# googlegenomics/spark-examples

Hardware: AMD Instinct MI355X
Metric: variants/sec into N×N Gram + PCoA wall-clock, 2504 samples, 1/2/4/8 GPU (higher is better)
Workload: dtype fp4(e2m1)->f32->i32

## Files before the change

### include/pcoa.h

```cpp
#ifndef PCOA_H_
#define PCOA_H_

#include <stddef.h>
#include <stdint.h>

#ifdef __cplusplus
extern "C" {
#endif

#define PCOA_VERSION_MAJOR 0
#define PCOA_VERSION_MINOR 10

typedef struct pcoa_ctx pcoa_ctx;

typedef enum pcoa_status {
  PCOA_OK = 0,
  PCOA_ERR_INVALID_ARG = -1,
  PCOA_ERR_NO_DEVICE = -2,
  PCOA_ERR_HIP = -3,
  PCOA_ERR_OUT_OF_MEMORY = -4,
  PCOA_ERR_INDEX_RANGE = -5,
  PCOA_ERR_RCCL = -6,
  PCOA_ERR_NOT_CONVERGED = -7,
  PCOA_ERR_STATE = -8
// ... 145 lines not shown
  double king_seconds;
  int64_t king_bytes;
  int64_t king_calls;
} pcoa_king_stats;
int pcoa_get_king_stats(pcoa_ctx* plane0, pcoa_king_stats* out, size_t out_size);

#define PCOA_LOADINGS_CENTRE 1u
#define PCOA_LOADINGS_UNIT   2u
int pcoa_loadings_begin(pcoa_ctx* ctx, int32_t num_pc, const double* components ,
                        const double* eigenvalues , uint32_t flags);
int pcoa_loadings_bits(pcoa_ctx* ctx, const uint32_t* bits, int64_t n_variants, int64_t ld_words, int is_device_ptr,
                       double* out , int out_is_device);
int pcoa_loadings_plink_bed(pcoa_ctx* ctx, const uint8_t* bed_rows, int64_t n_variants, int64_t row_bytes, int ref_is_a1,
                            int is_device_ptr, double* out, int out_is_device);
int pcoa_loadings_operator(pcoa_ctx* ctx, int64_t first_variant, int64_t n_variants, double* out, int out_is_device);
int pcoa_loadings_end(pcoa_ctx* ctx);

typedef struct pcoa_loadings_stats {
  int64_t loadings_variants;
  int64_t loadings_bytes;
  double loadings_seconds;
} pcoa_loadings_stats;
int pcoa_get_loadings_stats(pcoa_ctx* ctx, pcoa_loadings_stats* out, size_t out_size);

#define PCOA_LD_MAX_WINDOW 1024
#define PCOA_LD_ACCUMULATE 1u
int pcoa_ld_begin(pcoa_ctx* ctx, int32_t window, double r2_max, uint32_t flags);
int pcoa_ld_bits(pcoa_ctx* ctx, const uint32_t* bits, int64_t n_variants, int64_t ld_words, int is_device_ptr,
                 uint8_t* keep_out , int64_t* n_kept_out );
int pcoa_ld_plink_bed(pcoa_ctx* ctx, const uint8_t* bed_rows, int64_t n_variants, int64_t row_bytes, int ref_is_a1,
                      int is_device_ptr , uint8_t* keep_out, int64_t* n_kept_out);
int pcoa_ld_break(pcoa_ctx* ctx);
int pcoa_ld_end(pcoa_ctx* ctx);

typedef struct pcoa_ld_stats {
  int64_t ld_variants;
  int64_t ld_kept;
  int64_t ld_monomorphic;
  int64_t ld_pairs;
  double ld_count_seconds;
  double ld_band_seconds;
  double ld_resolve_seconds;
  double ld_compact_seconds;
} pcoa_ld_stats;
int pcoa_get_ld_stats(pcoa_ctx* ctx, pcoa_ld_stats* out, size_t out_size);

#define PCOA_LAYOUT_AUTO   0
#define PCOA_LAYOUT_FULL   1
#define PCOA_LAYOUT_STRIPS 2
#define PCOA_LAYOUT_FREE_FRACTION 0.9

int pcoa_plan_layout(int32_t n_samples, int32_t n_engines, const int64_t* free_bytes, int32_t request, int32_t* layout_out,
                     int32_t* col0_out, int32_t* cols_out);

int pcoa_device_memory(int32_t device_ordinal, int64_t* free_out, int64_t* total_out);

int pcoa_compute_strips(pcoa_ctx* const* owners, int32_t n_owners, int32_t num_pc, double* out_components,
                        double* out_eigenvalues, int32_t* nonzero_rows_out);

void pcoa_destroy(pcoa_ctx* ctx);

const char* pcoa_last_error(const pcoa_ctx* ctx);

int pcoa_reset(pcoa_ctx* ctx);

int pcoa_n_samples(const pcoa_ctx* ctx);

int pcoa_set_stream(pcoa_ctx* ctx, void* hip_stream);

int pcoa_sync(pcoa_ctx* ctx);

int pcoa_reserve(pcoa_ctx* ctx, int64_t variants_per_call, int32_t num_pc);


int pcoa_accumulate_calls(pcoa_ctx* ctx, const int32_t* sample_idx, const int64_t* row_offsets,
                          int64_t n_variants);

#define PCOA_CALLS_DEVICE_PTR 1u
#define PCOA_CALLS_HOST_PINNED 2u
#define PCOA_CALLS_ASYNC 4u
int pcoa_accumulate_calls_ex(pcoa_ctx* ctx, const int32_t* sample_idx, const int64_t* row_offsets, int64_t n_variants,
                             uint32_t flags);

int pcoa_accumulate_dense_f32(pcoa_ctx* ctx, const float* x, int64_t n_variants, int64_t ld,
                              int is_device_ptr);

int pcoa_accumulate_dense_u8(pcoa_ctx* ctx, const uint8_t* x, int64_t n_variants, int64_t ld, int is_device_ptr);

int pcoa_accumulate_bits(pcoa_ctx* ctx, const uint32_t* bits, int64_t n_variants, int64_t ld_words,
                         int is_device_ptr);

#define PCOA_BED_HOST_ASYNC 2
int pcoa_accumulate_plink_bed(pcoa_ctx* ctx, const uint8_t* bed_rows, int64_t n_variants, int64_t row_bytes, int ref_is_a1,
                              int is_device_ptr);

int pcoa_accumulate_synthetic(pcoa_ctx* ctx, const pcoa_synth_params* params, int64_t first_variant,
                              int64_t n_variants);

int pcoa_synth_fill_f32(pcoa_ctx* ctx, const pcoa_synth_params* params, int64_t first_variant,
                        int64_t n_variants, float* x_dev, int64_t ld);

int pcoa_gram_finalize(pcoa_ctx* ctx);

int pcoa_gram_allreduce_rccl(pcoa_ctx* ctx, void* nccl_comm);

int pcoa_comm_unique_id(uint8_t out_id[128]);
int pcoa_comm_runtime(char* path_out, int32_t path_cap, int32_t* version_out);
int pcoa_comm_init(pcoa_ctx* ctx, const uint8_t id[128], int32_t rank, int32_t n_ranks,
                   void** comm_out);
int pcoa_comm_destroy(void* nccl_comm);
int pcoa_comm_count(void* nccl_comm, int32_t* count_out);

int pcoa_host_alloc_pinned(size_t bytes, void** out);
int pcoa_host_free_pinned(void* p);

int pcoa_gram_reduce_from(pcoa_ctx* dst, pcoa_ctx* src);

#define PCOA_REDUCE_MAX_ENGINES 16
int pcoa_gram_reduce_peers(pcoa_ctx* const* ctxs, int32_t k, int32_t root_only);

typedef struct pcoa_reduce_peers_stats {
  int64_t reduce_peers_calls;
  double reduce_peers_seconds;
  int64_t reduce_peers_bytes_in;
} pcoa_reduce_peers_stats;
int pcoa_get_reduce_peers_stats(pcoa_ctx* ctx, pcoa_reduce_peers_stats* out, size_t out_size);

int pcoa_gram_export_device_i64(pcoa_ctx* ctx, int64_t* dst_dev);
int pcoa_gram_import_device_i64(pcoa_ctx* ctx, const int64_t* src_dev);

int pcoa_gram_read_i64(pcoa_ctx* ctx, int64_t* out_nxn);

int pcoa_gram_read_block_i64(pcoa_ctx* ctx, int32_t row0, int32_t col0, int32_t rows, int32_t cols, int64_t* out);

int pcoa_gram_load_i64(pcoa_ctx* ctx, const int64_t* in_nxn);


int pcoa_center_read_f64(pcoa_ctx* ctx, double* out_b_nxn, double* out_row_sums, int32_t* out_nonzero_rows,
                         double* out_matrix_mean);

int pcoa_compute(pcoa_ctx* ctx, int32_t num_pc, double* out_components, double* out_eigenvalues,
                 int32_t* out_nonzero_rows);

int pcoa_project(pcoa_ctx* ref, pcoa_ctx* cross, int32_t num_pc, const double* components, const double* eigenvalues,
                 double* out_coords);


int pcoa_get_timings(pcoa_ctx* ctx, pcoa_timings* out);
int pcoa_get_timings_sized(pcoa_ctx* ctx, pcoa_timings* out, size_t out_size);
int pcoa_reset_timings(pcoa_ctx* ctx);

int pcoa_debug_alloc(int32_t device_ordinal, size_t bytes, void** out);
int pcoa_debug_centred_matvec(pcoa_ctx* ctx, const double* x, double* y, int form);
int pcoa_debug_reduce_chunk(int32_t g, int32_t k, int32_t n_samples, int64_t* first_out, int64_t* count_out);
int pcoa_debug_free(void* p);
int pcoa_debug_guard_mode(void);


int pcoa_device_info(pcoa_ctx* ctx, char* name_out, int32_t name_cap, int32_t* cu_count_out);
const char* pcoa_version(void);

#ifdef __cplusplus
}
#endif
#endif
```

### spark-examples_amd/_lib.py

```python
import ctypes
import os

_HERE = os.path.dirname(os.path.abspath(__file__))
LIB_PATH = os.environ.get("PCOA_LIB") or os.path.join(_HERE, "libpcoa_hip.so")

PCOA_OK = 0
PCOA_ERR_INVALID_ARG = -1
PCOA_ERR_NO_DEVICE = -2
PCOA_ERR_HIP = -3
PCOA_ERR_OUT_OF_MEMORY = -4
PCOA_ERR_INDEX_RANGE = -5
PCOA_ERR_RCCL = -6
PCOA_ERR_NOT_CONVERGED = -7
PCOA_ERR_STATE = -8

PCOA_FLAG_DEFAULT = 0
PCOA_FLAG_GRAM_F32_MFMA = 0x1
PCOA_FLAG_GRAM_I8_MFMA = 0x2
PCOA_FLAG_GRAM_FP4_MFMA = 0x4
PCOA_FLAG_NO_SIGN_NORM = 0x10
PCOA_FLAG_EIG_HOUSEHOLDER = 0x20
PCOA_FLAG_EIG_LANCZOS = 0x40
PCOA_FLAG_NO_PIPELINE = 0x80
PCOA_FLAG_OPERAND_FP4 = 0x100
# ... 66 lines not shown
        ("reduce_peers_seconds", ctypes.c_double),
        ("reduce_peers_bytes_in", ctypes.c_int64),
    ]


PCOA_REDUCE_MAX_ENGINES = 16


class PcoaPair(ctypes.Structure):
    _fields_ = [
        ("i", ctypes.c_int32),
        ("j", ctypes.c_int32),
        ("shared", ctypes.c_int64),
    ]


class PcoaPairsStats(ctypes.Structure):
    _fields_ = [
        ("pairs_seconds", ctypes.c_double),
        ("pairs_bytes", ctypes.c_int64),
        ("pairs_calls", ctypes.c_int64),
    ]


PCOA_KING_HET = 0
PCOA_KING_MISSING = 1
PCOA_KING_HET_OR_MISSING = 2
PCOA_KING_HOM_A1 = 3
PCOA_KING_HOM_A2 = 4
PCOA_KING_PLANES = 5


class PcoaKingPair(ctypes.Structure):
    _fields_ = [
        ("i", ctypes.c_int32),
        ("j", ctypes.c_int32),
        ("hethet", ctypes.c_int64),
        ("ibs0", ctypes.c_int64),
        ("het_sum", ctypes.c_int64),
    ]


class PcoaKingStats(ctypes.Structure):
    _fields_ = [
        ("king_seconds", ctypes.c_double),
        ("king_bytes", ctypes.c_int64),
        ("king_calls", ctypes.c_int64),
    ]


class PcoaLdStats(ctypes.Structure):
    _fields_ = [
        ("ld_variants", ctypes.c_int64),
        ("ld_kept", ctypes.c_int64),
        ("ld_monomorphic", ctypes.c_int64),
        ("ld_pairs", ctypes.c_int64),
        ("ld_count_seconds", ctypes.c_double),
        ("ld_band_seconds", ctypes.c_double),
        ("ld_resolve_seconds", ctypes.c_double),
        ("ld_compact_seconds", ctypes.c_double),
    ]


class PcoaLoadingsStats(ctypes.Structure):
    _fields_ = [
        ("loadings_variants", ctypes.c_int64),
        ("loadings_bytes", ctypes.c_int64),
        ("loadings_seconds", ctypes.c_double),
    ]


PCOA_LOADINGS_CENTRE = 1
PCOA_LOADINGS_UNIT = 2
PCOA_LD_MAX_WINDOW = 1024
PCOA_LD_ACCUMULATE = 1


class PcoaSynthParams(ctypes.Structure):
    _fields_ = [
        ("seed", ctypes.c_uint64),
        ("n_pops", ctypes.c_int32),
        ("reserved", ctypes.c_int32),
        ("pop_offsets", ctypes.POINTER(ctypes.c_int32)),
        ("thresholds", ctypes.POINTER(ctypes.c_uint32)),
    ]


_vp = ctypes.c_void_p
_i32 = ctypes.c_int32
_i64 = ctypes.c_int64
_SIGNATURES = [
    ("pcoa_version", ctypes.c_char_p, []),
    ("pcoa_create", ctypes.c_int, [ctypes.POINTER(_vp), _i32, _i32, ctypes.c_uint32]),
    ("pcoa_create_strip", ctypes.c_int, [ctypes.POINTER(_vp), _i32, _i32, _i32, _i32, ctypes.c_uint32]),
    ("pcoa_create_operator", ctypes.c_int, [ctypes.POINTER(_vp), _i32, _i32, ctypes.c_uint32]),
    ("pcoa_create_subset", ctypes.c_int, [ctypes.POINTER(_vp), _vp, _vp, _i32]),
    ("pcoa_similar_pairs", ctypes.c_int, [_vp, ctypes.c_double, _vp, _i64, ctypes.POINTER(_i64), _vp]),
    ("pcoa_get_pairs_stats", ctypes.c_int, [_vp, ctypes.POINTER(PcoaPairsStats), ctypes.c_size_t]),
    ("pcoa_set_similarity", ctypes.c_int, [_vp, _i32]),
    ("pcoa_get_similarity", ctypes.c_int, [_vp, ctypes.POINTER(_i32)]),
    ("pcoa_set_call_companion", ctypes.c_int, [_vp, _vp, _i64]),
    ("pcoa_get_call_companion", ctypes.c_int, [_vp, ctypes.POINTER(_vp), ctypes.POINTER(_i64)]),
    ("pcoa_accumulate_plink_bed_calls", ctypes.c_int, [_vp, _vp, _vp, _i64, _i64, ctypes.c_int, ctypes.c_int]),
    ("pcoa_accumulate_plink_bed_king", ctypes.c_int, [_vp, _vp, _i64, _i64, ctypes.c_int]),
    ("pcoa_king_pairs", ctypes.c_int, [_vp, ctypes.c_double, _vp, _i64, ctypes.POINTER(_i64), ctypes.POINTER(_i64), _vp]),
    ("pcoa_get_king_stats", ctypes.c_int, [_vp, ctypes.POINTER(PcoaKingStats), ctypes.c_size_t]),
    ("pcoa_loadings_begin", ctypes.c_int, [_vp, _i32, _vp, _vp, ctypes.c_uint32]),
    ("pcoa_loadings_bits", ctypes.c_int, [_vp, _vp, _i64, _i64, ctypes.c_int, _vp, ctypes.c_int]),
    ("pcoa_loadings_plink_bed", ctypes.c_int, [_vp, _vp, _i64, _i64, ctypes.c_int, ctypes.c_int, _vp, ctypes.c_int]),
    ("pcoa_loadings_operator", ctypes.c_int, [_vp, _i64, _i64, _vp, ctypes.c_int]),
    ("pcoa_loadings_end", ctypes.c_int, [_vp]),
    ("pcoa_get_loadings_stats", ctypes.c_int, [_vp, ctypes.POINTER(PcoaLoadingsStats), ctypes.c_size_t]),
    ("pcoa_ld_begin", ctypes.c_int, [_vp, _i32, ctypes.c_double, ctypes.c_uint32]),
    ("pcoa_ld_bits", ctypes.c_int, [_vp, _vp, _i64, _i64, ctypes.c_int, _vp, ctypes.POINTER(_i64)]),
    ("pcoa_ld_plink_bed", ctypes.c_int, [_vp, _vp, _i64, _i64, ctypes.c_int, ctypes.c_int, _vp, ctypes.POINTER(_i64)]),
    ("pcoa_ld_break", ctypes.c_int, [_vp]),
    ("pcoa_ld_end", ctypes.c_int, [_vp]),
    ("pcoa_get_ld_stats", ctypes.c_int, [_vp, ctypes.POINTER(PcoaLdStats), ctypes.c_size_t]),
    ("pcoa_operator_info", ctypes.c_int, [_vp, ctypes.POINTER(_i64), ctypes.POINTER(_i64)]),
    ("pcoa_operator_row_sums", ctypes.c_int, [_vp, _vp]),
    ("pcoa_operator_matvec_device", ctypes.c_int, [_vp, _vp, _vp, ctypes.c_int]),
    ("pcoa_create_grm", ctypes.c_int, [ctypes.POINTER(_vp), _i32, _i32, ctypes.c_uint32]),
    ("pcoa_grm_info", ctypes.c_int, [_vp, ctypes.POINTER(_i64), ctypes.POINTER(_i64), ctypes.POINTER(_i64)]),
    ("pcoa_grm_set_min_maf", ctypes.c_int, [_vp, ctypes.c_double]),
    ("pcoa_grm_counts", ctypes.c_int, [_vp, _i64, _i64, _vp]),
    ("pcoa_grm_matvec_device", ctypes.c_int, [_vp, _vp, _vp]),
    ("pcoa_strip_info", ctypes.c_int, [_vp, ctypes.POINTER(_i32), ctypes.POINTER(_i32)]),
    ("pcoa_strip_col_sums", ctypes.c_int, [_vp, _vp]),
    ("pcoa_strip_matvec", ctypes.c_int, [_vp, _vp, _vp, ctypes.c_double, _vp]),
    ("pcoa_strip_set_centering", ctypes.c_int, [_vp, _vp, ctypes.c_double]),
    ("pcoa_strip_matvec_device", ctypes.c_int, [_vp, _vp, _vp]),
    ("pcoa_plan_layout", ctypes.c_int, [_i32, _i32, _vp, _i32, ctypes.POINTER(_i32), _vp, _vp]),
    ("pcoa_device_memory", ctypes.c_int, [_i32, ctypes.POINTER(_i64), ctypes.POINTER(_i64)]),
    ("pcoa_compute_strips", ctypes.c_int, [_vp, _i32, _i32, _vp, _vp, ctypes.POINTER(_i32)]),
    ("pcoa_project", ctypes.c_int, [_vp, _vp, _i32, _vp, _vp, _vp]),
    ("pcoa_destroy", None, [_vp]),
    ("pcoa_last_error", ctypes.c_char_p, [_vp]),
    ("pcoa_reset", ctypes.c_int, [_vp]),
    ("pcoa_n_samples", ctypes.c_int, [_vp]),
    ("pcoa_set_stream", ctypes.c_int, [_vp, _vp]),
    ("pcoa_sync", ctypes.c_int, [_vp]),
    ("pcoa_reserve", ctypes.c_int, [_vp, _i64, _i32]),
    ("pcoa_comm_runtime", ctypes.c_int, [ctypes.c_char_p, _i32, ctypes.POINTER(_i32)]),
    ("pcoa_debug_alloc", ctypes.c_int, [_i32, ctypes.c_size_t, ctypes.POINTER(_vp)]),
    ("pcoa_debug_free", ctypes.c_int, [_vp]),
    ("pcoa_debug_reduce_chunk", ctypes.c_int, [_i32, _i32, _i32, ctypes.POINTER(_i64), ctypes.POINTER(_i64)]),
    ("pcoa_debug_guard_mode", ctypes.c_int, []),
    ("pcoa_accumulate_calls", ctypes.c_int, [_vp, _vp, _vp, _i64]),
    ("pcoa_gram_reduce_from", ctypes.c_int, [_vp, _vp]),
    ("pcoa_gram_reduce_peers", ctypes.c_int, [_vp, _i32, _i32]),
    ("pcoa_get_reduce_peers_stats", ctypes.c_int, [_vp, ctypes.POINTER(PcoaReducePeersStats), ctypes.c_size_t]),
    ("pcoa_lanczos_with_matvec", ctypes.c_int, [_vp, ctypes.c_int32, _vp, _vp, _vp, _vp, ctypes.POINTER(ctypes.c_int32)]),
    ("pcoa_debug_centred_matvec", ctypes.c_int, [_vp, _vp, _vp, ctypes.c_int]),
    ("pcoa_host_alloc_pinned", ctypes.c_int, [ctypes.c_size_t, ctypes.POINTER(ctypes.c_void_p)]),
    ("pcoa_host_free_pinned", ctypes.c_int, [_vp]),
    ("pcoa_accumulate_plink_bed", ctypes.c_int, [_vp, _vp, _i64, _i64, ctypes.c_int, ctypes.c_int]),
    ("pcoa_accumulate_calls_ex", ctypes.c_int, [_vp, _vp, _vp, _i64, ctypes.c_uint32]),
    ("pcoa_accumulate_dense_f32", ctypes.c_int, [_vp, _vp, _i64, _i64, ctypes.c_int]),
    ("pcoa_accumulate_dense_u8", ctypes.c_int, [_vp, _vp, _i64, _i64, ctypes.c_int]),
    ("pcoa_accumulate_bits", ctypes.c_int, [_vp, _vp, _i64, _i64, ctypes.c_int]),
    ("pcoa_accumulate_synthetic", ctypes.c_int, [_vp, ctypes.POINTER(PcoaSynthParams), _i64, _i64]),
    ("pcoa_synth_fill_f32", ctypes.c_int, [_vp, ctypes.POINTER(PcoaSynthParams), _i64, _i64, _vp, _i64]),
    ("pcoa_gram_finalize", ctypes.c_int, [_vp]),
    ("pcoa_gram_allreduce_rccl", ctypes.c_int, [_vp, _vp]),
    ("pcoa_comm_unique_id", ctypes.c_int, [_vp]),
    ("pcoa_comm_init", ctypes.c_int, [_vp, _vp, _i32, _i32, ctypes.POINTER(_vp)]),
    ("pcoa_comm_destroy", ctypes.c_int, [_vp]),
    ("pcoa_comm_count", ctypes.c_int, [_vp, ctypes.POINTER(_i32)]),
    ("pcoa_gram_export_device_i64", ctypes.c_int, [_vp, _vp]),
    ("pcoa_gram_import_device_i64", ctypes.c_int, [_vp, _vp]),
    ("pcoa_gram_read_i64", ctypes.c_int, [_vp, _vp]),
    ("pcoa_gram_read_block_i64", ctypes.c_int, [_vp, _i32, _i32, _i32, _i32, _vp]),
    ("pcoa_gram_load_i64", ctypes.c_int, [_vp, _vp]),
    ("pcoa_center_read_f64", ctypes.c_int, [_vp, _vp, _vp, ctypes.POINTER(_i32), ctypes.POINTER(ctypes.c_double)]),
    ("pcoa_compute", ctypes.c_int, [_vp, _i32, _vp, _vp, ctypes.POINTER(_i32)]),
    ("pcoa_get_timings", ctypes.c_int, [_vp, ctypes.POINTER(PcoaTimings)]),
    ("pcoa_get_timings_sized", ctypes.c_int, [_vp, ctypes.POINTER(PcoaTimings), ctypes.c_size_t]),
    ("pcoa_reset_timings", ctypes.c_int, [_vp]),
    ("pcoa_device_info", ctypes.c_int, [_vp, ctypes.c_char_p, _i32, ctypes.POINTER(_i32)]),
]
EXPORTED_SYMBOLS = [s[0] for s in _SIGNATURES]

_lib = None


def source_hash():
    import hashlib
    h = hashlib.sha256()
    csrc = os.path.join(_HERE, "csrc")
    files = [os.path.join(csrc, f) for f in sorted(os.listdir(csrc)) if f.endswith((".hip", ".inl", ".h"))]
    files.append(os.path.join(os.path.dirname(_HERE), "include", "pcoa.h"))
    for f in files:
        h.update(os.path.basename(f).encode())
        with open(f, "rb") as fh:
            h.update(fh.read())
    return h.hexdigest()[:16]


def load():
    global _lib
    if _lib is not None:
        return _lib
    if not os.path.exists(LIB_PATH):
        raise ImportError(
            "%s not found: build it with `python -c 'import __graft_entry__ as g; g.build()'` or "
            "`make -C spark-examples_amd/csrc`.  There is no CPU fallback." % LIB_PATH)
    try:
        import torch
    except Exception:
        pass
    lib = ctypes.CDLL(LIB_PATH, mode=ctypes.RTLD_GLOBAL)
    for name, restype, argtypes in _SIGNATURES:
        fn = getattr(lib, name)
        fn.restype = restype
        fn.argtypes = argtypes
    _lib = lib
    return lib
```

### spark-examples_amd/csrc/capi_compute.hip

```cpp
#include <algorithm>
#include <cmath>
#include <cstdio>
#include <string>

#include "pcoa_ctx.h"

using namespace pcoa;

namespace pcoa {

int ensure_workspace(pcoa_ctx* c, int32_t k) {
  const int64_t n = c->n;
  if (!c->ws_ready) {
    HIP_TRY(c, dev_alloc((void**)&c->colmean, sizeof(double) * (size_t)n, c->device));
    HIP_TRY(c, dev_alloc((void**)&c->ws.d, sizeof(double) * (size_t)n, c->device));
    HIP_TRY(c, dev_alloc((void**)&c->ws.e, sizeof(double) * (size_t)n, c->device));
    HIP_TRY(c, dev_alloc((void**)&c->ws.tau, sizeof(double) * (size_t)n, c->device));
    HIP_TRY(c, dev_alloc((void**)&c->ws.q, sizeof(double) * (size_t)n, c->device));
    HIP_TRY(c, dev_alloc((void**)&c->ws.w, sizeof(double) * (size_t)(2 * n), c->device));
    HIP_TRY(c, dev_alloc((void**)&c->ws.scratch, sizeof(double) * (size_t)(6 * n), c->device));
    HIP_TRY(c, dev_alloc((void**)&c->ws.iscratch, sizeof(int32_t) * (size_t)(2 * n + 64), c->device));
    HIP_TRY(c, dev_alloc((void**)&c->row_sums, sizeof(double) * (size_t)n, c->device));
    HIP_TRY(c, dev_alloc((void**)&c->stats, sizeof(double) * (size_t)(2 + n), c->device));
    HIP_TRY(c, dev_alloc((void**)&c->nz, sizeof(int32_t) * 4, c->device));
// ... 58 lines not shown
  c->lanczos_steps = steps;
  if (steps_out) *steps_out = steps;
  if (!conv)
    return fail(c, PCOA_ERR_NOT_CONVERGED, "Lanczos did not reach a verified residual (tiny spectral gaps?); there is no dense "
                                           "fallback for an operator the engine does not hold");
  c->eig_method = 1;
  c->eig_dense_form = 0;
  HIP_TRY(c, launch_backtransform(c->ws, n, num_pc, (c->flags & PCOA_FLAG_NO_SIGN_NORM) ? 0 : 1, 0, c->out_dev, c->stream));
  HIP_TRY(c, hipMemcpyAsync(out_components, c->out_dev, sizeof(double) * (size_t)num_pc * (size_t)n, hipMemcpyDeviceToHost,
                            c->stream));
  HIP_TRY(c, hipStreamSynchronize(c->stream));
  for (size_t i = 0; i < (size_t)num_pc * (size_t)n; ++i)
    if (!std::isfinite(out_components[i])) return fail(c, PCOA_ERR_NOT_CONVERGED, "non-finite eigenvector entry");
  if (out_eigenvalues)
    for (int32_t t = 0; t < num_pc; ++t) out_eigenvalues[t] = sel[(size_t)t];
  return PCOA_OK;
}

}

namespace {

int project_engine_state(pcoa_ctx* report, pcoa_ctx* c, const char* who, int rc) {
  if (rc == PCOA_ERR_INDEX_RANGE || rc == PCOA_ERR_INVALID_ARG) rc = PCOA_ERR_STATE;
  return fail(report, rc, std::string("project: ") + who + ": " + c->last_error);
}

int compute_strips_small(pcoa_ctx* const* owners, int32_t n_owners, int32_t num_pc, double* out_components,
                         double* out_eigenvalues, int32_t* nonzero_rows_out) {
  pcoa_ctx* lead = owners[0];
  const int32_t n = lead->n;
  std::vector<int64_t> s((size_t)n * (size_t)n), part;
  for (int32_t i = 0; i < n_owners; ++i) {
    pcoa_ctx* o = owners[i];
    part.assign((size_t)n * (size_t)o->s_cols, 0);
    const int rc = pcoa_gram_read_i64(o, part.data());
    if (rc != PCOA_OK) return fail(lead, rc, "compute_strips: owner " + std::to_string(i) + ": " + o->last_error);
    for (int32_t r = 0; r < n; ++r)
      for (int32_t j = 0; j < o->s_cols; ++j) s[(size_t)r * n + o->strip_col0 + j] = part[(size_t)r * o->s_cols + j];
  }
  pcoa_ctx* tmp = nullptr;
  int rc = pcoa_create(&tmp, n, lead->device, lead->flags);
  if (rc != PCOA_OK) return fail(lead, rc, std::string("compute_strips: temporary engine: ") + pcoa_last_error(nullptr));
  rc = pcoa_gram_load_i64(tmp, s.data());
  if (rc == PCOA_OK) rc = pcoa_compute(tmp, num_pc, out_components, out_eigenvalues, nonzero_rows_out);
  if (rc != PCOA_OK) lead->last_error = "compute_strips: temporary engine: " + tmp->last_error;
  pcoa_destroy(tmp);
  (void)hipSetDevice(lead->device);
  return rc;
}

}

extern "C" {

int pcoa_center_read_f64(pcoa_ctx* c, double* out_b, double* out_row_sums, int32_t* out_nonzero_rows,
                         double* out_matrix_mean) {
  CHECK_CTX(c);
  NOT_ON_OPERATOR(c, "pcoa_center_read_f64");
  if (c->is_strip) return fail(c, PCOA_ERR_STATE, "a strip owner holds N x cols of S: use pcoa_strip_col_sums / pcoa_strip_matvec");
  int rc = finalize_impl(c);
  if (rc != PCOA_OK) return rc;
  if ((rc = check_device_flags(c)) != PCOA_OK) return rc;
  rc = ensure_workspace(c, 1);
  if (rc != PCOA_OK) return rc;
  if (out_b && (rc = ensure_b(c)) != PCOA_OK) return rc;
  const size_t n = (size_t)c->n;
  {
    ScopedTimer t(c, T_CENTER);
    if (measured(c)) {
      if ((rc = measure_centre(c, false, out_b ? c->ws.a : nullptr)) != PCOA_OK) return rc;
    } else {
      HIP_TRY(c, launch_center(c->s32, c->s64, c->n, c->row_sums, c->stats, c->nz, out_b ? c->ws.a : nullptr,
                               c->stream));
    }
  }
  if (out_b) HIP_TRY(c, hipMemcpyAsync(out_b, c->ws.a, sizeof(double) * n * n, hipMemcpyDeviceToHost, c->stream));
  if (out_row_sums)
    HIP_TRY(c, hipMemcpyAsync(out_row_sums, c->row_sums, sizeof(double) * n, hipMemcpyDeviceToHost, c->stream));
  HIP_TRY(c, hipMemcpyAsync(c->hw->st, c->stats, 2 * sizeof(double), hipMemcpyDeviceToHost, c->stream));
  HIP_TRY(c, hipMemcpyAsync(&c->hw->nz, c->nz, sizeof(int32_t), hipMemcpyDeviceToHost, c->stream));
  HIP_TRY(c, hipStreamSynchronize(c->stream));
  if (out_nonzero_rows) *out_nonzero_rows = c->hw->nz;
  if (out_matrix_mean) *out_matrix_mean = c->hw->st[1];
  return PCOA_OK;
}

int pcoa_compute(pcoa_ctx* c, int32_t num_pc, double* out_components, double* out_eigenvalues,
                 int32_t* out_nonzero_rows) {
  CHECK_CTX(c);
  const int32_t n = c->n;
  if (num_pc <= 0 || num_pc > n) {
    char buf[128];
    std::snprintf(buf, sizeof(buf), "num_pc = %d out of range (0, n = %d]", num_pc, n);
    return fail(c, PCOA_ERR_INVALID_ARG, buf);
  }
  if (!out_components) return fail(c, PCOA_ERR_INVALID_ARG, "out_components is NULL");
  if (c->is_grm) return grm_compute(c, num_pc, out_components, out_eigenvalues, out_nonzero_rows);
  if (c->is_operator) return operator_compute(c, num_pc, out_components, out_eigenvalues, out_nonzero_rows);
  if (c->is_strip)
    return fail(c, PCOA_ERR_STATE, "a strip owner holds N x cols of S: the eigensolve over strips is driven by the host "
                                   "(pcoa_strip_col_sums / pcoa_strip_matvec; spark-examples_amd/strips.py)");
  int rc = finalize_impl(c);
  if (rc != PCOA_OK) return rc;
  rc = check_device_flags(c);
  if (rc != PCOA_OK) return rc;
  rc = ensure_workspace(c, num_pc);
  if (rc != PCOA_OK) return rc;

  struct WallEvents {
    pcoa_ctx* c;
    hipEvent_t w0, w1;
    ~WallEvents() {
      if (w0) c->pool.push_back(w0);
      if (w1) c->pool.push_back(w1);
    }
  } wall{c, get_event(c), get_event(c)};
  hipEvent_t w0 = wall.w0, w1 = wall.w1;
  if (w0) (void)hipEventRecord(w0, c->stream);

  const bool force_householder = (c->flags & PCOA_FLAG_EIG_HOUSEHOLDER) != 0;
  const bool force_lanczos = (c->flags & PCOA_FLAG_EIG_LANCZOS) != 0;
  const bool try_lanczos = !force_householder && n >= 32;
  const bool explicit_b = !try_lanczos || debug_knobs().explicit_center != 0;
  if (explicit_b && (rc = ensure_b(c)) != PCOA_OK) return rc;
  const int sym_min = debug_knobs().symv_sym_min_n > 0 ? debug_knobs().symv_sym_min_n : 16384;
  const bool sym_form = !explicit_b && !c->s64 && n >= sym_min && (n & 3) == 0;
  if (sym_form && (rc = ensure(c, &c->sym_part, &c->sym_part_cap, (int64_t)symv_sym_workspace_doubles(n))) != PCOA_OK) return rc;
  const bool measured = pcoa::measured(c);
  {
    ScopedTimer t(c, T_CENTER);
    if (measured) {
      if ((rc = measure_centre(c, sym_form, explicit_b ? c->ws.a : nullptr)) != PCOA_OK) return rc;
    } else {
      if (sym_form)
        HIP_TRY(c, launch_row_sums_sym(c->s32, n, c->sym_part, c->row_sums, reinterpret_cast<int64_t*>(c->stats + 2), c->stream));
      HIP_TRY(c, launch_center(c->s32, c->s64, n, c->row_sums, c->stats, c->nz, explicit_b ? c->ws.a : nullptr,
                               c->stream, sym_form));
      HIP_TRY(c, launch_col_means(c->row_sums, n, c->colmean, c->stream));
    }
  }
  c->ws.s32 = c->s32;
  c->ws.s64 = c->s64;
  c->ws.colmean = c->colmean;
  c->ws.stats = c->stats;
  bool b_ready = explicit_b;
  std::vector<double> sel((size_t)num_pc);
  bool have_vectors = false;
  c->eig_method = 0;
  c->eig_dense_form = 0;
  c->lanczos_steps = 0;
  if (try_lanczos) {
    const int32_t mmax = std::min<int32_t>(n, 512);
    const int64_t need = (int64_t)lanczos_workspace_doubles(n, num_pc, mmax);
    rc = ensure(c, &c->lanczos_ws, &c->lanczos_cap, need);
    if (rc != PCOA_OK) return rc;
    int conv = 0, steps = 0;
    {
      ScopedTimer t(c, T_LANCZOS);
      EigWorkspace wl = c->ws;
      if (!b_ready) wl.a = nullptr;
      wl.sym_part = (sym_form && !wl.a) ? c->sym_part : nullptr;
      c->matvec_form = wl.a ? 2 : wl.sym_part ? 1 : 0;
      wl.band_only = (c->flags & PCOA_FLAG_EIG_BAND) != 0;
      if (measured) measure_bind(c, &wl);
      int band = 0;
      HIP_TRY(c, lanczos_topk(wl, c->lanczos_ws, n, num_pc, mmax, 1e-11, sel.data(), &conv, &steps, c->stream, nullptr, &band));
      c->lanczos_block_steps = band;
    }
    c->lanczos_steps = steps;
    if (conv) {
      have_vectors = true;
      c->eig_method = 1;
    } else if (force_lanczos) {
      return fail(c, PCOA_ERR_NOT_CONVERGED, "Lanczos did not reach a verified residual (PCOA_FLAG_EIG_LANCZOS set)");
    } else if (n > 16384) {
      return fail(c, PCOA_ERR_NOT_CONVERGED,
                  "Lanczos did not reach a verified residual and the dense O(N^3) fallback is disabled above "
                  "N = 16384 (set PCOA_FLAG_EIG_HOUSEHOLDER to force it)");
    }
  }
  if (!have_vectors) {
    c->eig_method = 2;
    if (!b_ready) {
      if ((rc = ensure_b(c)) != PCOA_OK) return rc;
      ScopedTimer t(c, T_CENTER);
      if (measured) {
        if ((rc = measure_b(c, c->ws.a)) != PCOA_OK) return rc;
      } else {
        HIP_TRY(c, launch_center(c->s32, c->s64, n, c->row_sums, c->stats, c->nz, c->ws.a, c->stream));
      }
      b_ready = true;
    }
    {
      ScopedTimer t(c, T_TRIDIAG);
      HIP_TRY(c, launch_tridiagonalize(c->ws, n, c->stream, &c->eig_dense_form));
    }
    std::vector<int32_t> idx;
    for (int32_t t = 0; t < num_pc; ++t) idx.push_back(n - 1 - t);
    for (int32_t t = 0; t < num_pc; ++t)
      if (t < n - num_pc) idx.push_back(t);
    std::vector<double> cand(idx.size());
    {
      ScopedTimer t(c, T_EIG);
      HIP_TRY(c, launch_bisect(c->ws, n, idx.data(), (int32_t)idx.size(), c->ws.lam, c->stream, &c->eig_dense_form));
      HIP_TRY(c, hipMemcpyAsync(cand.data(), c->ws.lam, sizeof(double) * cand.size(), hipMemcpyDeviceToHost,
                                c->stream));
    }
    HIP_TRY(c, hipStreamSynchronize(c->stream));
    std::vector<int> order(cand.size());
    for (size_t i = 0; i < order.size(); ++i) order[i] = (int)i;
    std::stable_sort(order.begin(), order.end(), [&](int a, int b) {
      const double fa = std::fabs(cand[a]), fb = std::fabs(cand[b]);
      if (fa != fb) return fa > fb;
      return cand[a] > cand[b];
    });
    for (int32_t t = 0; t < num_pc; ++t) {
      if (!std::isfinite(cand[order[t]])) return fail(c, PCOA_ERR_NOT_CONVERGED, "non-finite eigenvalue");
      sel[(size_t)t] = cand[order[t]];
    }
    {
      ScopedTimer t(c, T_EIG);
      HIP_TRY(c, launch_inverse_iteration(c->ws, n, sel.data(), num_pc, c->stream, &c->eig_dense_form));
    }
  }
  {
    ScopedTimer t(c, T_BACK);
    HIP_TRY(c, launch_backtransform(c->ws, n, num_pc, (c->flags & PCOA_FLAG_NO_SIGN_NORM) ? 0 : 1,
                                    have_vectors ? 0 : 1, c->out_dev, c->stream, have_vectors ? nullptr : &c->eig_dense_form));
  }
  HIP_TRY(c, hipMemcpyAsync(out_components, c->out_dev, sizeof(double) * (size_t)num_pc * (size_t)n,
                            hipMemcpyDeviceToHost, c->stream));
  HIP_TRY(c, hipMemcpyAsync(&c->hw->nz, c->nz, sizeof(int32_t), hipMemcpyDeviceToHost, c->stream));
  if (w1) (void)hipEventRecord(w1, c->stream);
  HIP_TRY(c, hipStreamSynchronize(c->stream));
  if (w0 && w1) {
    float ms = 0.f;
    if (hipEventElapsedTime(&ms, w0, w1) == hipSuccess) c->compute_total = (double)ms * 1e-3;
  }
  for (int32_t t = 0; t < num_pc; ++t) {
    for (int32_t i = 0; i < n; ++i)
      if (!std::isfinite(out_components[(size_t)t * n + i]))
        return fail(c, PCOA_ERR_NOT_CONVERGED, "non-finite eigenvector entry");
  }
  if (out_eigenvalues)
    for (int32_t t = 0; t < num_pc; ++t) out_eigenvalues[t] = sel[(size_t)t];
  if (out_nonzero_rows) *out_nonzero_rows = c->hw->nz;
  return PCOA_OK;
}

int pcoa_lanczos_with_matvec(pcoa_ctx* c, int32_t num_pc, pcoa_matvec_fn fn, void* user, double* out_components,
                             double* out_eigenvalues, int32_t* steps_out) {
  CHECK_CTX(c);
  NOT_ON_GRM(c, "pcoa_lanczos_with_matvec");
  const int32_t n = c->n;
  if (!fn || !out_components) return fail(c, PCOA_ERR_INVALID_ARG, "fn or out_components is NULL");
  if (num_pc <= 0 || num_pc > n) return fail(c, PCOA_ERR_INVALID_ARG, "num_pc must be in (0, n]");
  if (n < 32) return fail(c, PCOA_ERR_INVALID_ARG, "the Lanczos path needs N >= 32");
  LanczosMatvec mv = [&](const double* v, double* y) { return fn(user, v, y); };
  return lanczos_over(c, num_pc, mv, out_components, out_eigenvalues, steps_out);
}

int pcoa_strip_info(const pcoa_ctx* c, int32_t* col0_out, int32_t* cols_out) {
  if (!c) return fail(nullptr, PCOA_ERR_INVALID_ARG, "ctx is NULL");
  if (col0_out) *col0_out = c->strip_col0;
  if (cols_out) *cols_out = c->s_cols;
  return c->is_strip ? 1 : 0;
}

int pcoa_strip_col_sums(pcoa_ctx* c, double* out_cols) {
  CHECK_CTX(c);
  if (!c->is_strip) return fail(c, PCOA_ERR_STATE, "not a strip owner (pcoa_create_strip)");
  if (!out_cols) return fail(c, PCOA_ERR_INVALID_ARG, "out_cols is NULL");
  int rc = finalize_impl(c);
  if (rc != PCOA_OK) return rc;
  if ((rc = check_device_flags(c)) != PCOA_OK) return rc;
  const int64_t need = strip_ws_doubles(c->n, c->s_cols);
  if ((rc = ensure(c, &c->strip_ws, &c->strip_ws_cap, need)) != PCOA_OK) return rc;
  {
    ScopedTimer t(c, T_CENTER);
    HIP_TRY(c, launch_strip_col_sums(c->s32, c->s64, c->n, c->s_cols, c->strip_ws, c->stream));
  }
  HIP_TRY(c, hipMemcpyAsync(out_cols, c->strip_ws, sizeof(double) * (size_t)c->s_cols, hipMemcpyDeviceToHost, c->stream));
  HIP_TRY(c, hipStreamSynchronize(c->stream));
  return PCOA_OK;
}

int pcoa_strip_matvec(pcoa_ctx* c, const double* v, const double* means, double matrix_mean, double* y_out) {
  CHECK_CTX(c);
  if (!c->is_strip) return fail(c, PCOA_ERR_STATE, "not a strip owner (pcoa_create_strip)");
  if (!v || !means || !y_out) return fail(c, PCOA_ERR_INVALID_ARG, "v, means or y_out is NULL");
  int rc = finalize_impl(c);
  if (rc != PCOA_OK) return rc;
  if ((rc = check_device_flags(c)) != PCOA_OK) return rc;
  const int64_t need = strip_ws_doubles(c->n, c->s_cols) + 2 * (int64_t)c->n;
  if ((rc = ensure(c, &c->strip_ws, &c->strip_ws_cap, need)) != PCOA_OK) return rc;
  double* v_dev = c->strip_ws + strip_ws_doubles(c->n, c->s_cols);
  double* m_dev = v_dev + c->n;
  HIP_TRY(c, hipMemcpyAsync(v_dev, v, sizeof(double) * (size_t)c->n, hipMemcpyHostToDevice, c->stream));
  HIP_TRY(c, hipMemcpyAsync(m_dev, means, sizeof(double) * (size_t)c->n, hipMemcpyHostToDevice, c->stream));
  {
    ScopedTimer t(c, T_LANCZOS);
    HIP_TRY(c, launch_strip_matvec(c->s32, c->s64, c->n, c->strip_col0, c->s_cols, v_dev, m_dev, matrix_mean, c->strip_ws,
                                   c->stream));
  }
  HIP_TRY(c, hipMemcpyAsync(y_out, c->strip_ws, sizeof(double) * (size_t)c->s_cols, hipMemcpyDeviceToHost, c->stream));
  HIP_TRY(c, hipStreamSynchronize(c->stream));
  return PCOA_OK;
}

int pcoa_strip_set_centering(pcoa_ctx* c, const double* means, double matrix_mean) {
  CHECK_CTX(c);
  if (!c->is_strip) return fail(c, PCOA_ERR_STATE, "not a strip owner (pcoa_create_strip)");
  if (!means) return fail(c, PCOA_ERR_INVALID_ARG, "means is NULL");
  if (!c->strip_means) HIP_TRY(c, dev_alloc((void**)&c->strip_means, sizeof(double) * (size_t)c->n, c->device));
  HIP_TRY(c, hipMemcpyAsync(c->strip_means, means, sizeof(double) * (size_t)c->n, hipMemcpyHostToDevice, c->stream));
  HIP_TRY(c, hipStreamSynchronize(c->stream));
// ... 228 lines not shown
    int64_t* to_i64 = local ? rs_i64 + c->strip_col0 : reinterpret_cast<int64_t*>(c->strip_ws + strip_ws_doubles(n, c->s_cols));
    double* to_f64 = local ? lead->row_sums + c->strip_col0 : c->strip_ws + strip_ws_doubles(n, c->s_cols) + n;
    {
      ScopedTimer t(c, T_CENTER);
      const hipError_t e = launch_strip_col_sums_to(c->s32, c->s64, n, c->s_cols, c->strip_ws, to_i64, to_f64, c->stream);
      if (e != hipSuccess) return owner_failed(i, hip_fail(c, e, "strip column sums"));
    }
    if (!local) {
      hipError_t e = hipMemcpyPeerAsync(rs_i64 + c->strip_col0, lead->device, to_i64, c->device, sizeof(int64_t) * (size_t)c->s_cols,
                                        c->stream);
      if (e == hipSuccess)
        e = hipMemcpyPeerAsync(lead->row_sums + c->strip_col0, lead->device, to_f64, c->device, sizeof(double) * (size_t)c->s_cols,
                               c->stream);
      if (e != hipSuccess) return owner_failed(i, hip_fail(c, e, "peer copy of the column sums"));
    }
  }
  for (int32_t i = 0; i < n_owners; ++i) {
    pcoa_ctx* c = owners[i];
    (void)hipSetDevice(c->device);
    const hipError_t e = hipStreamSynchronize(c->stream);
    if (e != hipSuccess) return owner_failed(i, hip_fail(c, e, "column sums"));
  }
  (void)hipSetDevice(lead->device);
  {
    ScopedTimer t(lead, T_CENTER);
    HIP_TRY(lead, launch_center(nullptr, nullptr, n, lead->row_sums, lead->stats, lead->nz, nullptr, lead->stream, true));
    HIP_TRY(lead, launch_col_means(lead->row_sums, n, lead->colmean, lead->stream));
  }
  double st[2] = {0, 0};
  HIP_TRY(lead, hipMemcpyAsync(st, lead->stats, sizeof(st), hipMemcpyDeviceToHost, lead->stream));
  HIP_TRY(lead, hipMemcpyAsync(&lead->hw->nz, lead->nz, sizeof(int32_t), hipMemcpyDeviceToHost, lead->stream));
  for (int32_t i = 0; i < n_owners; ++i) {
    pcoa_ctx* c = owners[i];
    if (c->device == lead->device)
      HIP_TRY(lead, hipMemcpyAsync(c->strip_means, lead->colmean, sizeof(double) * (size_t)n, hipMemcpyDeviceToDevice, lead->stream));
    else
      HIP_TRY(lead, hipMemcpyPeerAsync(c->strip_means, c->device, lead->colmean, lead->device, sizeof(double) * (size_t)n, lead->stream));
  }
  HIP_TRY(lead, hipStreamSynchronize(lead->stream));
  const double matrix_mean = st[1];
  for (int32_t i = 0; i < n_owners; ++i) {
    owners[i]->strip_matrix_mean = matrix_mean;
    owners[i]->strip_centering_set = true;
  }

  struct Events {
    std::vector<hipEvent_t> ev;
    ~Events() { for (hipEvent_t e : ev) if (e) (void)hipEventDestroy(e); }
  } evs;
  evs.ev.assign((size_t)n_owners + 1, nullptr);
  for (int32_t i = 0; i <= n_owners; ++i) {
    const int dev = i == 0 ? lead->device : owners[i - 1]->device;
    (void)hipSetDevice(dev);
    const hipError_t e = hipEventCreateWithFlags(&evs.ev[(size_t)i], hipEventDisableTiming);
    if (e != hipSuccess) {
      (void)hipSetDevice(lead->device);
      return hip_fail(lead, e, "hipEventCreateWithFlags");
    }
  }
  (void)hipSetDevice(lead->device);
  std::string mv_error;
  LanczosMatvec mv = [&](const double* v, double* y) -> int {
    auto bad = [&](hipError_t e, int32_t i, const char* what) {
      mv_error = "compute_strips: owner " + std::to_string(i) + ": " + what + ": " + hipGetErrorString(e);
      (void)hipSetDevice(lead->device);
      return 1;
    };
    hipError_t e = hipEventRecord(evs.ev[0], lead->stream);
    if (e != hipSuccess) return bad(e, 0, "hipEventRecord");
    for (int32_t i = 0; i < n_owners; ++i) {
      pcoa_ctx* c = owners[i];
      const bool local = c->device == lead->device;
      if ((e = hipSetDevice(c->device)) != hipSuccess) return bad(e, i, "hipSetDevice");
      if ((e = hipStreamWaitEvent(c->stream, evs.ev[0], 0)) != hipSuccess) return bad(e, i, "hipStreamWaitEvent");
      const double* vo = v;
      double* dst = y + c->strip_col0;
      double* const spare = c->strip_ws + strip_ws_doubles(n, c->s_cols);
      if (!local) {
        if ((e = hipMemcpyPeerAsync(spare, c->device, v, lead->device, sizeof(double) * (size_t)n, c->stream)) != hipSuccess)
          return bad(e, i, "peer copy of v");
        vo = spare;
        if (!peer[(size_t)i]) dst = spare + n;
      }
      if ((e = launch_strip_matvec_to(c->s32, c->s64, n, c->strip_col0, c->s_cols, vo, c->strip_means, matrix_mean, c->strip_ws,
                                      dst, c->stream)) != hipSuccess)
        return bad(e, i, "strip mat-vec");
      if (!local && !peer[(size_t)i] &&
          (e = hipMemcpyPeerAsync(y + c->strip_col0, lead->device, dst, c->device, sizeof(double) * (size_t)c->s_cols,
                                  c->stream)) != hipSuccess)
        return bad(e, i, "peer copy of the piece");
      if ((e = hipEventRecord(evs.ev[(size_t)i + 1], c->stream)) != hipSuccess) return bad(e, i, "hipEventRecord");
    }
    if ((e = hipSetDevice(lead->device)) != hipSuccess) return bad(e, 0, "hipSetDevice");
    for (int32_t i = 0; i < n_owners; ++i)
      if ((e = hipStreamWaitEvent(lead->stream, evs.ev[(size_t)i + 1], 0)) != hipSuccess) return bad(e, i, "hipStreamWaitEvent");
    return 0;
  };
  int32_t steps = 0;
  rc = lanczos_over(lead, num_pc, mv, out_components, out_eigenvalues, &steps);
  if (rc != PCOA_OK && !mv_error.empty()) lead->last_error = mv_error;
  if (rc != PCOA_OK) return rc;
  if (nonzero_rows_out) *nonzero_rows_out = lead->hw->nz;
  lead->compute_total = wall_now() - t0;
  return PCOA_OK;
}

int pcoa_debug_centred_matvec(pcoa_ctx* c, const double* x, double* y, int form) {
  CHECK_CTX(c);
  if (!x || !y) return fail(c, PCOA_ERR_INVALID_ARG, "x or y is NULL");
  if (form < 0 || form > 2) return fail(c, PCOA_ERR_INVALID_ARG, "form must be 0, 1 or 2");
  const bool upper_triangle_form = form == 1;
  NOT_ON_OPERATOR(c, "pcoa_debug_centred_matvec");
  if (c->is_strip) return fail(c, PCOA_ERR_STATE, "not available on a strip owner");
  int rc = finalize_impl(c);
  if (rc != PCOA_OK) return rc;
  if ((rc = check_device_flags(c)) != PCOA_OK) return rc;
  if ((rc = ensure_workspace(c, 1)) != PCOA_OK) return rc;
  const int32_t n = c->n;
  EigWorkspace wl = c->ws;
  wl.a = nullptr;
  wl.s32 = c->s32;
  wl.s64 = c->s64;
  wl.colmean = c->colmean;
  wl.stats = c->stats;
  wl.sym_part = nullptr;
  if (upper_triangle_form) {
    if (c->s64 || (n & 3)) return fail(c, PCOA_ERR_STATE, "the upper-triangle form needs N % 4 == 0 and no int64 part");
    if ((rc = ensure(c, &c->sym_part, &c->sym_part_cap, (int64_t)symv_sym_workspace_doubles(n))) != PCOA_OK) return rc;
    wl.sym_part = c->sym_part;
    if (!measured(c))
      HIP_TRY(c, launch_row_sums_sym(c->s32, n, c->sym_part, c->row_sums, reinterpret_cast<int64_t*>(c->stats + 2), c->stream));
  }
  if (form == 2) {
    if ((rc = ensure_b(c)) != PCOA_OK) return rc;
    wl.a = c->ws.a;
  }
  if (measured(c)) {
    if ((rc = measure_centre(c, upper_triangle_form, wl.a)) != PCOA_OK) return rc;
    measure_bind(c, &wl);
  } else {
    HIP_TRY(c, launch_center(c->s32, c->s64, n, c->row_sums, c->stats, c->nz, wl.a, c->stream, upper_triangle_form));
    HIP_TRY(c, launch_col_means(c->row_sums, n, c->colmean, c->stream));
  }
  double* xd = c->ws.q;
  double* yd = c->ws.w;
  HIP_TRY(c, hipMemcpyAsync(xd, x, sizeof(double) * (size_t)n, hipMemcpyHostToDevice, c->stream));
  launch_centred_matvec(wl, n, xd, yd, c->stream);
  HIP_TRY(c, hipGetLastError());
  HIP_TRY(c, hipMemcpyAsync(y, yd, sizeof(double) * (size_t)n, hipMemcpyDeviceToHost, c->stream));
  HIP_TRY(c, hipStreamSynchronize(c->stream));
  return PCOA_OK;
}

}
```

### spark-examples_amd/csrc/eig.hip

```cpp
#include <cfloat>
#include <type_traits>
#include <algorithm>
#include <cmath>

#include "pcoa_internal.h"

namespace pcoa {
namespace {

constexpr int HW_T = 1024;

__device__ __forceinline__ double wave_sum(double v) {
#pragma unroll
  for (int o = 32; o > 0; o >>= 1) v += __shfl_down(v, o, 64);
  return v;
}
__device__ __forceinline__ double wave_max(double v) {
#pragma unroll
  for (int o = 32; o > 0; o >>= 1) v = fmax(v, __shfl_down(v, o, 64));
  return v;
}
__device__ __forceinline__ double wave_min(double v) {
#pragma unroll
  for (int o = 32; o > 0; o >>= 1) v = fmin(v, __shfl_down(v, o, 64));
// ... 527 lines not shown
  const int lane = threadIdx.x & 63, wave = threadIdx.x >> 6;
  const int slice = blockIdx.x, vec = blockIdx.y;
  const int s0 = blk * BT;
  const int c0 = slice * 256, c1 = (c0 + 256 < n) ? c0 + 256 : n;
  const double* zc = z + (int64_t)vec * n;
  for (int i = wave; i < BT; i += 4) {
    double acc = 0.0;
    if (s0 + i < nref) {
      const double* vi = a + (int64_t)(s0 + i) * n;
      for (int c = c0 + lane; c < c1; c += 64)
        if (c > s0 + i) acc += vi[c] * zc[c];
    }
    acc = wave_sum(acc);
    if (lane == 0) ypart[((int64_t)slice * k + vec) * BT + i] = acc;
  }
}

__global__ __launch_bounds__(256) void wy_apply_kernel(const double* __restrict__ a, int n, int nref, int blk, int nslices,
                                                       const double* __restrict__ t, const double* __restrict__ ypart,
                                                       double* __restrict__ z, int k) {
  __shared__ double y[BT], ty[BT];
  const int slice = blockIdx.x, vec = blockIdx.y;
  const int s0 = blk * BT;
  if (threadIdx.x < BT) {
    double acc = 0.0;
    for (int sl = 0; sl < nslices; ++sl) acc += ypart[((int64_t)sl * k + vec) * BT + threadIdx.x];
    y[threadIdx.x] = acc;
  }
  __syncthreads();
  if (threadIdx.x < BT) {
    const double* tb = t + (int64_t)blk * BT * BT;
    double acc = 0.0;
    for (int c = threadIdx.x; c < BT; ++c) acc += tb[threadIdx.x * BT + c] * y[c];
    ty[threadIdx.x] = acc;
  }
  __syncthreads();
  const int c = slice * 256 + threadIdx.x;
  if (c >= n) return;
  double* zc = z + (int64_t)vec * n;
  double acc = 0.0;
#pragma unroll 8
  for (int i = 0; i < BT; ++i)
    if (s0 + i < nref && c > s0 + i) acc += a[(int64_t)(s0 + i) * n + c] * ty[i];
  zc[c] -= acc;
}

}

hipError_t launch_tridiagonalize(const EigWorkspace& ws, int32_t n, hipStream_t stream, int32_t* form) {
  if (n <= 0) return hipErrorInvalidValue;
  if (n == 1) {
    hipLaunchKernelGGL(tridiag_hw_kernel, dim3(1), dim3(HW_T), 0, stream, ws.a, n, 0, ws.d, ws.e, ws.tau, ws.q,
                       ws.w);
    return hipGetLastError();
  }
  const size_t lds_full = 3 * (size_t)n * sizeof(double);
  int kf = 0;
  if (n >= 8 && lds_full <= 160 * 1024 - 1024) {
    if (lds_full > 64 * 1024) {
      static bool raised = false;
      if (!raised) {
        hipError_t err = hipFuncSetAttribute(reinterpret_cast<const void*>(tridiag_fused_kernel),
                                             hipFuncAttributeMaxDynamicSharedMemorySize, 160 * 1024 - 1024);
        if (err != hipSuccess) return err;
        raised = true;
      }
    }
    if (form) *form |= EIG_FORM_FUSED | (lds_full > 64 * 1024 ? EIG_FORM_FUSED_BIG_LDS : 0);
    kf = n - 2;
    double* qb[2] = {ws.w, ws.w + n};
    double* vb[2] = {ws.scratch, ws.scratch + n};
    for (int k = 0; k < kf; ++k) {
      const int rows = n - k - 1;
      int nb = (rows + FT / 64 - 1) / (FT / 64);
      if (nb > 256) nb = 256;
      nb = (nb + 7) / 8 * 8;
      const size_t lds = 3 * (size_t)(n - k) * sizeof(double);
      hipLaunchKernelGGL(tridiag_fused_kernel, dim3((unsigned)nb), dim3(FT), lds, stream, ws.a, n, k, ws.d, ws.e, ws.tau,
                         qb[(k + 1) & 1], qb[k & 1], vb[(k + 1) & 1], vb[k & 1]);
    }
    hipError_t err = hipMemcpyAsync(ws.a + (int64_t)(kf - 1) * n + kf, vb[(kf - 1) & 1] + kf, sizeof(double) * (size_t)(n - kf),
                                    hipMemcpyDeviceToDevice, stream);
    if (err != hipSuccess) return err;
    err = hipMemcpyAsync(ws.q, qb[(kf - 1) & 1], sizeof(double) * (size_t)n, hipMemcpyDeviceToDevice, stream);
    if (err != hipSuccess) return err;
  }
  if (form && kf == 0) *form |= EIG_FORM_TWO_KERNEL;
  for (int k = kf; k <= n - 2; ++k) {
    const int hw_threads = HW_T;
    hipLaunchKernelGGL(tridiag_hw_kernel, dim3(1), dim3(hw_threads), 0, stream, ws.a, n, k, ws.d, ws.e, ws.tau,
                       ws.q, ws.w);
    if (k <= n - 3) {
      const int rows = n - k - 1;
      hipLaunchKernelGGL(tridiag_update_kernel, dim3((unsigned)((rows + 3) / 4)), dim3(256), 0, stream, ws.a, n,
                         k, ws.w, ws.q);
    }
  }
  return hipGetLastError();
}

hipError_t launch_bisect(const EigWorkspace& ws, int32_t n, const int32_t* idx_host, int32_t count,
                         double* lam_out_dev, hipStream_t stream, int32_t* form) {
  if (count <= 0) return hipSuccess;
  hipError_t err = hipMemcpyAsync(ws.iscratch, idx_host, sizeof(int32_t) * count, hipMemcpyHostToDevice, stream);
  if (err != hipSuccess) return err;
  const size_t lds_full = sizeof(double) * (32 + 2 * (size_t)n);
  const int use_lds = lds_full <= 64 * 1024;
  const size_t lds = use_lds ? lds_full : sizeof(double) * 32;
  if (form && use_lds) *form |= EIG_FORM_BISECT_LDS;
  hipLaunchKernelGGL(bisect_kernel, dim3((unsigned)count), dim3(256), lds, stream, ws.d, ws.e, n, ws.iscratch,
                     lam_out_dev, use_lds);
  return hipGetLastError();
}

namespace {
hipError_t invit_lds_bytes(int32_t n, size_t* lds_out) {
  const size_t lds = (size_t)n * (5 * sizeof(double) + sizeof(int)) + 16;
  const bool use_lds = lds <= 150 * 1024;
  if (use_lds && lds > 64 * 1024) {
    static bool raised = false;
    if (!raised) {
      hipError_t err = hipFuncSetAttribute(reinterpret_cast<const void*>(invit_kernel),
                                           hipFuncAttributeMaxDynamicSharedMemorySize, 160 * 1024);
      if (err != hipSuccess) return err;
      raised = true;
    }
  }
  *lds_out = use_lds ? lds : 0;
  return hipSuccess;
}
}

hipError_t launch_inverse_iteration(const EigWorkspace& ws, int32_t n, const double* lam_sel_host, int32_t k,
                                    hipStream_t stream, int32_t* form) {
  hipError_t err = hipMemcpyAsync(ws.lam, lam_sel_host, sizeof(double) * k, hipMemcpyHostToDevice, stream);
  if (err != hipSuccess) return err;
  size_t lds = 0;
  if ((err = invit_lds_bytes(n, &lds)) != hipSuccess) return err;
  const int use_lds = lds > 0;
  bool separate = use_lds && k > 1;
  if (separate) {
    double big = 0.0;
    for (int c = 0; c < k; ++c) big = std::max(big, std::fabs(lam_sel_host[c]));
    for (int c = 0; c < k && separate; ++c)
      for (int p = 0; p < c; ++p)
        if (std::fabs(lam_sel_host[c] - lam_sel_host[p]) <= 1e-2 * big) { separate = false; break; }
  }
  if (form) *form |= (use_lds ? EIG_FORM_INVIT_LDS : 0) | (separate ? EIG_FORM_INVIT_PER_VECTOR : 0);
  hipLaunchKernelGGL(invit_kernel, dim3(separate ? (unsigned)k : 1u), dim3(64), lds, stream, ws.d, ws.e, n,
                     ws.lam, k, ws.z, ws.scratch, ws.iscratch, use_lds);
  return hipGetLastError();
}

hipError_t launch_inverse_iteration_dev(const EigWorkspace& ws, int32_t n, int32_t k, hipStream_t stream) {
  size_t lds = 0;
  hipError_t err = invit_lds_bytes(n, &lds);
  if (err != hipSuccess) return err;
  hipLaunchKernelGGL(invit_kernel, dim3(1), dim3(64), lds, stream, ws.d, ws.e, n, ws.lam, k, ws.z, ws.scratch,
                     ws.iscratch, lds > 0 ? 1 : 0);
  return hipGetLastError();
}

hipError_t launch_backtransform(const EigWorkspace& ws, int32_t n, int32_t k, int sign_normalize,
                                int apply_reflectors, double* out_dev, hipStream_t stream, int32_t* form) {
  const int nref = n - 2;
  if (apply_reflectors && ws.wy != nullptr && nref >= 4 * BT) {
    const int nblk = (nref + BT - 1) / BT;
    const int nslices = (n + 255) / 256;
    double* g = ws.wy;
    double* t = g + (int64_t)nblk * BT * BT;
    double* ypart = t + (int64_t)nblk * BT * BT;
    hipLaunchKernelGGL(wy_gram_kernel, dim3(BT * BT / 4, (unsigned)nblk), dim3(256), 0, stream, ws.a, n, nref, g);
    hipLaunchKernelGGL(wy_tfactor_kernel, dim3((unsigned)nblk), dim3(64), 0, stream, g, ws.tau, nref, t);
    for (int blk = nblk - 1; blk >= 0; --blk) {
      hipLaunchKernelGGL(wy_dots_kernel, dim3((unsigned)nslices, (unsigned)k), dim3(256), 0, stream, ws.a, n, nref, blk, ws.z,
                         k, ypart);
      hipLaunchKernelGGL(wy_apply_kernel, dim3((unsigned)nslices, (unsigned)k), dim3(256), 0, stream, ws.a, n, nref, blk,
                         nslices, t, ypart, ws.z, k);
    }
    apply_reflectors = 0;
    if (form) *form |= EIG_FORM_WY_BACKTRANSFORM;
  }
  hipLaunchKernelGGL(backtransform_kernel, dim3((unsigned)k), dim3(HW_T), 0, stream, ws.a, n, ws.tau, ws.z,
                     sign_normalize, apply_reflectors, out_dev);
  return hipGetLastError();
}

size_t wy_workspace_doubles(int32_t n, int32_t k) {
  const int64_t nblk = ((int64_t)n - 2 + BT - 1) / BT;
  const int64_t nslices = ((int64_t)n + 255) / 256;
  return (size_t)(std::max<int64_t>(nblk, 1) * 2 * BT * BT + nslices * k * BT);
}

}
```

### spark-examples_amd/csrc/eig_lanczos.hip

```cpp
#include <algorithm>
#include <cfloat>
#include <cstdio>
#include <cstdlib>

#include "pcoa_internal.h"
#include "symv_shared.h"

namespace pcoa {
namespace {

__device__ __forceinline__ double block_sum(double v, double* red) {
  v = wave_sum(v);
  const int w = threadIdx.x >> 6;
  const int nw = (blockDim.x + 63) >> 6;
  __syncthreads();
  if ((threadIdx.x & 63) == 0) red[w] = v;
  __syncthreads();
  if (threadIdx.x < 64) {
    double t = ((int)threadIdx.x < nw) ? red[threadIdx.x] : 0.0;
    t = wave_sum(t);
    if (threadIdx.x == 0) red[16] = t;
  }
  __syncthreads();
  return red[16];
}

__global__ __launch_bounds__(1024) void lanczos_init_kernel(double* __restrict__ v0, int n, uint32_t salt = 0u) {
  __shared__ double red[24];
  double part = 0.0;
  for (int i = threadIdx.x; i < n; i += 1024) {
    uint32_t s = (uint32_t)(i + 1) * 2654435761u + 12345u + salt * 0x9E3779B9u;
    s = s * 1103515245u + 12345u;
    s ^= s >> 15;
    s = s * 1103515245u + 12345u;
    const double x = (double)(s >> 8) * (1.0 / 8388608.0) - 1.0;
    v0[i] = x;
    part += x * x;
  }
  const double nrm2 = block_sum(part, red);
  const double rn = 1.0 / sqrt(nrm2);
  for (int i = threadIdx.x; i < n; i += 1024) v0[i] *= rn;
}

__global__ __launch_bounds__(256) void symv_kernel(const double* __restrict__ a, int n,
                                                   const double* __restrict__ x, double* __restrict__ y) {
  const int lane = threadIdx.x & 63;
  const int i = blockIdx.x * 4 + (threadIdx.x >> 6);
  if (i >= n) return;
  const double* row = a + (int64_t)i * n;
  auto quad = [&](int j, double* out) {
    const double2 lo = *reinterpret_cast<const double2*>(row + j), hi = *reinterpret_cast<const double2*>(row + j + 2);
    out[0] = lo.x; out[1] = lo.y; out[2] = hi.x; out[3] = hi.y;
  };
  auto one = [&](int j) -> double { return row[j]; };
  const double acc = row_dot(quad, one, x, n, lane);
  if (lane == 0) y[i] = acc;
}

template <bool HAS64>
__global__ __launch_bounds__(256) void symv_centered_kernel(const int32_t* __restrict__ s32,
                                                            const int64_t* __restrict__ s64, int n,
                                                            const double* __restrict__ cm,
                                                            const double* __restrict__ stats,
                                                            const double* __restrict__ x, double* __restrict__ y) {
  const int lane = threadIdx.x & 63;
  const int i = blockIdx.x * 4 + (threadIdx.x >> 6);
  if (i >= n) return;
  const int64_t base = (int64_t)i * n;
  const double row_mean = cm[i];
  const double mmean = stats[1];
  auto centre = [&](double data, double col_mean) -> double {
#pragma clang fp contract(off)
    double t = data - row_mean;
    t = t - col_mean;
    t = t + mmean;
    return t;
  };
  auto quad = [&](int j, double* out) {
    const int4 s = *reinterpret_cast<const int4*>(s32 + base + j);
    double d0 = (double)s.x, d1 = (double)s.y, d2 = (double)s.z, d3 = (double)s.w;
    if (HAS64) {
      const longlong2 l = *reinterpret_cast<const longlong2*>(s64 + base + j);
      const longlong2 h = *reinterpret_cast<const longlong2*>(s64 + base + j + 2);
      d0 = (double)((int64_t)s.x + l.x); d1 = (double)((int64_t)s.y + l.y);
      d2 = (double)((int64_t)s.z + h.x); d3 = (double)((int64_t)s.w + h.y);
    }
    const double2 ca = *reinterpret_cast<const double2*>(cm + j), cb = *reinterpret_cast<const double2*>(cm + j + 2);
    out[0] = centre(d0, ca.x); out[1] = centre(d1, ca.y); out[2] = centre(d2, cb.x); out[3] = centre(d3, cb.y);
  };
  auto one = [&](int j) -> double {
    const double data = HAS64 ? (double)((int64_t)s32[base + j] + s64[base + j]) : (double)s32[base + j];
    return centre(data, cm[j]);
  };
  const double acc = row_dot(quad, one, x, n, lane);
  if (lane == 0) y[i] = acc;
}



template <bool DIAG, bool EDGE>
__device__ __forceinline__ void symv_sym_tile_body(const int32_t* __restrict__ s32, int n, int nb,
                                                   const double* __restrict__ cm, const double mmean,
                                                   const double* __restrict__ x, double* __restrict__ part, int bi, int bj,
                                                   double* xs, double* ms, double (*rs)[SYT]) {
  const int lane = threadIdx.x & 63, wave = __builtin_amdgcn_readfirstlane(threadIdx.x >> 6);
  const int wr = wave >> 1, wc = wave & 1;
  const int i0 = bi * SYT, j0 = bj * SYT;
  const int jw = j0 + 512 * wc + 4 * lane;
  const int rows = EDGE ? min(SYT, n - i0) : SYT;
  for (int r = threadIdx.x; r < SYT; r += 256) {
    const bool in = !EDGE || i0 + r < n;
    xs[r] = in ? x[i0 + r] : 0.0;
    ms[r] = in ? cm[i0 + r] : 0.0;
  }
  double xj[8], mj[8], cacc[8];
#pragma unroll
  for (int q = 0; q < 2; ++q)
#pragma unroll
    for (int e = 0; e < 4; ++e) {
      const int j = jw + 256 * q + e;
      const bool in = !EDGE || j < n;
      xj[4 * q + e] = in ? x[j] : 0.0;
      mj[4 * q + e] = in ? cm[j] : 0.0;
      cacc[4 * q + e] = 0.0;
    }
  __syncthreads();
  const int32_t* base = s32 + (int64_t)i0 * n + jw;
  auto load_row = [&](int r, int4 (&v)[2]) {
    const int32_t* rowp = base + (int64_t)r * n;
#pragma unroll
    for (int q = 0; q < 2; ++q) {
      if (EDGE) {
        const bool in = r < rows && jw + 256 * q < n;
        v[q] = in ? *reinterpret_cast<const int4*>(rowp + 256 * q) : make_int4(0, 0, 0, 0);
      } else {
        v[q] = *reinterpret_cast<const int4*>(rowp + 256 * q);
      }
    }
  };
  auto use_row = [&](int r, const int4 (&v)[2]) {
    const int i = i0 + r;
    const double xi = xs[r], mi = ms[r];
    double racc = 0.0;
#pragma unroll
    for (int q = 0; q < 2; ++q) {
      const int sv[4] = {v[q].x, v[q].y, v[q].z, v[q].w};
#pragma unroll
      for (int e = 0; e < 4; ++e) {
        const int j = jw + 256 * q + e;
        const double d = (double)sv[e];
        double bij, bji;
        {
#pragma clang fp contract(off)
          bij = d - mi;
          bij = bij - mj[4 * q + e];
          bij = bij + mmean;
          bji = d - mj[4 * q + e];
          bji = bji - mi;
          bji = bji + mmean;
        }
        if (DIAG) {
          const bool in = !EDGE || j < n;
          racc += (j >= i && in) ? bij * xj[4 * q + e] : 0.0;
          cacc[4 * q + e] += (j > i && in) ? bji * xi : 0.0;
        } else if (EDGE) {
          racc += j < n ? bij * xj[4 * q + e] : 0.0;
          cacc[4 * q + e] += j < n ? bji * xi : 0.0;
        } else {
          racc += bij * xj[4 * q + e];
          cacc[4 * q + e] += bji * xi;
        }
      }
    }
    racc = wave_sum_to_lane63(racc);
    if (lane == 63) rs[wc][r] = racc;
#pragma unroll
    for (int c = 0; c < 8; ++c) asm volatile("" : "+v"(cacc[c]));
    __builtin_amdgcn_sched_barrier(0);
  };
  int4 buf[SYNB][2];
  const int nr = rows > wr ? (rows - wr + 1) / 2 : 0;
#pragma unroll
  for (int b = 0; b < SYNB; ++b)
    if (b < nr) load_row(wr + 2 * b, buf[b]);
  int k = 0;
  for (; k + 2 * SYNB <= nr; k += SYNB) {
#pragma unroll
    for (int b = 0; b < SYNB; ++b) {
      use_row(wr + 2 * (k + b), buf[b]);
      load_row(wr + 2 * (k + b + SYNB), buf[b]);
    }
  }
#pragma unroll
  for (int b = 0; b < SYNB; ++b)
    if (k + b < nr) {
      use_row(wr + 2 * (k + b), buf[b]);
      if (k + b + SYNB < nr) load_row(wr + 2 * (k + b + SYNB), buf[b]);
    }
  k += SYNB;
#pragma unroll
  for (int b = 0; b < SYNB; ++b)
    if (k + b < nr) use_row(wr + 2 * (k + b), buf[b]);
  double* ptile = part + sym_tile_index(bi, bj, nb) * SYP;
  double* pcol = ptile + 2 * SYT + wr * SYT + 512 * wc + 4 * lane;
#pragma unroll
  for (int q = 0; q < 2; ++q) {
    *reinterpret_cast<double2*>(pcol + 256 * q) = make_double2(cacc[4 * q], cacc[4 * q + 1]);
    *reinterpret_cast<double2*>(pcol + 256 * q + 2) = make_double2(cacc[4 * q + 2], cacc[4 * q + 3]);
  }
  __syncthreads();
  for (int r = threadIdx.x; r < SYT; r += 256) {
    ptile[r] = r < rows ? rs[0][r] : 0.0;
    ptile[SYT + r] = r < rows ? rs[1][r] : 0.0;
  }
}

__global__ __launch_bounds__(256) __attribute__((amdgpu_num_vgpr(64)))
void symv_sym_tiles_kernel(const int32_t* __restrict__ s32, int n, int nb, int nbi,
                           const double* __restrict__ cm, const double* __restrict__ stats,
                           const double* __restrict__ x, double* __restrict__ part) {
  __shared__ double xs[SYT], ms[SYT];
  __shared__ double rs[2][SYT];
  const double mmean = stats[1];
  int t = blockIdx.x;
  const int edge = nb - nbi;
  if (t < edge) {
    symv_sym_tile_body<true, true>(s32, n, nb, cm, mmean, x, part, nb - 1, nb - 1, xs, ms, rs);
    return;
  }
  t -= edge;
  if (t < nbi) {
    symv_sym_tile_body<true, false>(s32, n, nb, cm, mmean, x, part, t, t, xs, ms, rs);
    return;
  }
  t -= nbi;
  if (t < edge * (nb - 1)) {
    symv_sym_tile_body<false, true>(s32, n, nb, cm, mmean, x, part, t, nb - 1, xs, ms, rs);
    return;
  }
  t -= edge * (nb - 1);
  int bi = 0;
  while (t >= nbi - 1 - bi) {
    t -= nbi - 1 - bi;
    ++bi;
  }
  symv_sym_tile_body<false, false>(s32, n, nb, cm, mmean, x, part, bi, bi + 1 + t, xs, ms, rs);
}

// ... 16 lines not shown
template <int CTRL, int ROW_MASK>
__device__ __forceinline__ int64_t dpp_add_i64(int64_t v) {
  const int lo = (int)(uint32_t)v, hi = (int)(uint32_t)((uint64_t)v >> 32);
  const uint32_t l2 = (uint32_t)__builtin_amdgcn_update_dpp(0, lo, CTRL, ROW_MASK, 0xF, false);
  const uint32_t h2 = (uint32_t)__builtin_amdgcn_update_dpp(0, hi, CTRL, ROW_MASK, 0xF, false);
  return v + (int64_t)(((uint64_t)h2 << 32) | l2);
}
__device__ __forceinline__ int64_t wave_sum_i64_to_lane63(int64_t v) {
  v = dpp_add_i64<0xB1, 0xF>(v);
  v = dpp_add_i64<0x4E, 0xF>(v);
  v = dpp_add_i64<0x141, 0xF>(v);
  v = dpp_add_i64<0x140, 0xF>(v);
  v = dpp_add_i64<0x142, 0xA>(v);
  v = dpp_add_i64<0x143, 0xC>(v);
  return v;
}

__global__ __launch_bounds__(256) void rowsums_sym_tiles_kernel(const int32_t* __restrict__ s32, int n, int nb,
                                                                int64_t* __restrict__ part) {
  __shared__ int64_t rs[2][SYT];
  const int lane = threadIdx.x & 63, wave = __builtin_amdgcn_readfirstlane(threadIdx.x >> 6);
  const int wr = wave >> 1, wc = wave & 1;
  int t = blockIdx.x, bi = 0;
  while (t >= nb - bi) {
    t -= nb - bi;
    ++bi;
  }
  const int bj = bi + t;
  const bool diag = bi == bj;
  const int i0 = bi * SYT, j0 = bj * SYT;
  const int jw = j0 + 512 * wc + 4 * lane;
  const int rows = min(SYT, n - i0);
  const bool full = j0 + SYT <= n;
  int64_t cacc[8];
#pragma unroll
  for (int c = 0; c < 8; ++c) cacc[c] = 0;
  const int32_t* base = s32 + (int64_t)i0 * n + jw;
  auto load_row = [&](int r, int4 (&v)[2]) {
    const int32_t* rowp = base + (int64_t)r * n;
#pragma unroll
    for (int q = 0; q < 2; ++q)
      v[q] = (full || (r < rows && jw + 256 * q < n)) ? *reinterpret_cast<const int4*>(rowp + 256 * q) : make_int4(0, 0, 0, 0);
  };
  auto use_row = [&](int r, const int4 (&v)[2]) {
    const int i = i0 + r;
    int64_t racc = 0;
#pragma unroll
    for (int q = 0; q < 2; ++q) {
      const int sv[4] = {v[q].x, v[q].y, v[q].z, v[q].w};
#pragma unroll
      for (int e = 0; e < 4; ++e) {
        const int j = jw + 256 * q + e;
        racc += (!diag || j >= i) ? sv[e] : 0;
        cacc[4 * q + e] += (!diag || j > i) ? sv[e] : 0;
      }
    }
    racc = wave_sum_i64_to_lane63(racc);
    if (lane == 63) rs[wc][r] = racc;
  };
  int4 buf[SYNB][2];
  const int nr = rows > wr ? (rows - wr + 1) / 2 : 0;
#pragma unroll
  for (int b = 0; b < SYNB; ++b)
    if (b < nr) load_row(wr + 2 * b, buf[b]);
  int k = 0;
  for (; k + 2 * SYNB <= nr; k += SYNB) {
#pragma unroll
    for (int b = 0; b < SYNB; ++b) {
      use_row(wr + 2 * (k + b), buf[b]);
      load_row(wr + 2 * (k + b + SYNB), buf[b]);
    }
  }
#pragma unroll
  for (int b = 0; b < SYNB; ++b)
    if (k + b < nr) {
      use_row(wr + 2 * (k + b), buf[b]);
      if (k + b + SYNB < nr) load_row(wr + 2 * (k + b + SYNB), buf[b]);
    }
  k += SYNB;
#pragma unroll
  for (int b = 0; b < SYNB; ++b)
    if (k + b < nr) use_row(wr + 2 * (k + b), buf[b]);
  int64_t* ptile = part + sym_tile_index(bi, bj, nb) * SYP;
  int64_t* pcol = ptile + 2 * SYT + wr * SYT + 512 * wc + 4 * lane;
#pragma unroll
  for (int q = 0; q < 2; ++q)
#pragma unroll
    for (int e = 0; e < 4; ++e) pcol[256 * q + e] = cacc[4 * q + e];
  __syncthreads();
  for (int r = threadIdx.x; r < SYT; r += 256) {
    ptile[r] = r < rows ? rs[0][r] : 0;
    ptile[SYT + r] = r < rows ? rs[1][r] : 0;
  }
}

__global__ __launch_bounds__(256) void rowsums_sym_gather_kernel(const int64_t* __restrict__ part, int n, int nb,
                                                                 double* __restrict__ row_sums, int64_t* __restrict__ row_sums_i64) {
  const int i = blockIdx.x * 256 + threadIdx.x;
  if (i >= n) return;
  const int bi = i / SYT, r = i - bi * SYT;
  int64_t acc = 0;
  for (int bj = bi; bj < nb; ++bj) {
    const int64_t* t = part + sym_tile_index(bi, bj, nb) * SYP;
    acc += t[r] + t[SYT + r];
  }
  for (int bk = 0; bk <= bi; ++bk) {
    const int64_t* t = part + sym_tile_index(bk, bi, nb) * SYP + 2 * SYT;
    acc += t[r] + t[SYT + r];
  }
  row_sums_i64[i] = acc;
  row_sums[i] = (double)acc;
}

size_t symv_sym_workspace_doubles_impl(int n) {
  const int64_t nb = (n + SYT - 1) / SYT;
  return (size_t)(nb * (nb + 1) / 2) * (size_t)SYP;
}

void launch_symv(const EigWorkspace& ws, int n, const double* x, double* y, hipStream_t stream) {
  const unsigned rows4 = (unsigned)((n + 3) / 4);
  if (ws.a) {
    hipLaunchKernelGGL(symv_kernel, dim3(rows4), dim3(256), 0, stream, ws.a, n, x, y);
  } else if (ws.measure != PCOA_SIMILARITY_SHARED) {
    (void)launch_measure_symv(ws, n, x, y, stream);
  } else if (ws.comp_q32) {
    (void)launch_complete_symv(ws, n, x, y, stream);
  } else if (ws.s64) {
    hipLaunchKernelGGL(symv_centered_kernel<true>, dim3(rows4), dim3(256), 0, stream, ws.s32, ws.s64, n, ws.colmean,
                       ws.stats, x, y);
  } else if (ws.sym_part && (n & 3) == 0) {
    const int nb = (n + SYT - 1) / SYT;
    const int nbi = n / SYT;
    hipLaunchKernelGGL(symv_sym_tiles_kernel, dim3((unsigned)((int64_t)nb * (nb + 1) / 2)), dim3(256), 0, stream, ws.s32, n, nb, nbi,
                       ws.colmean, ws.stats, x, ws.sym_part);
    hipLaunchKernelGGL(symv_sym_gather_kernel, dim3((unsigned)((n + 255) / 256)), dim3(256), 0, stream, ws.sym_part, n, nb, y);
  } else {
    hipLaunchKernelGGL(symv_centered_kernel<false>, dim3(rows4), dim3(256), 0, stream, ws.s32, ws.s64, n, ws.colmean,
                       ws.stats, x, y);
  }
}

__global__ __launch_bounds__(256) void cgs_dots_kernel(const double* __restrict__ v, int n,
                                                       const double* __restrict__ w, double* __restrict__ h) {
  __shared__ double red[24];
  const double* vp = v + (int64_t)blockIdx.x * n;
  double part = 0.0;
  for (int i = threadIdx.x; i < n; i += 256) part += vp[i] * w[i];
  const double t = block_sum(part, red);
  if (threadIdx.x == 0) h[blockIdx.x] = t;
}

constexpr int kMaxKrylov = 512;

__global__ __launch_bounds__(256) void cgs_update_dots_kernel(const double* __restrict__ v, int n, int count,
                                                              const double* __restrict__ h, double* __restrict__ w,
                                                              double* __restrict__ part) {
  __shared__ double red[4][kMaxKrylov + 8];
  const int i = blockIdx.x * 256 + threadIdx.x;
  const int lane = threadIdx.x & 63, wave = threadIdx.x >> 6;
  const bool in = i < n;
  const int ic = in ? i : n - 1;
  double acc = 0.0;
  for (int p = 0; p < count; ++p) acc += h[p] * v[(int64_t)p * n + ic];
  const double wi = in ? w[ic] - acc : 0.0;
  if (in) w[i] = wi;
  for (int q = 0; q < count; ++q) {
    const double t = wave_sum(v[(int64_t)q * n + ic] * wi);
    if (lane == 0) red[wave][q] = t;
  }
  __syncthreads();
  for (int q = threadIdx.x; q < count; q += 256)
    part[(int64_t)blockIdx.x * count + q] = (red[0][q] + red[1][q]) + (red[2][q] + red[3][q]);
}

__global__ __launch_bounds__(256) void cgs_update_norm_kernel(const double* __restrict__ v, int n, int count,
                                                              const double* __restrict__ part, int nb,
                                                              double* __restrict__ w, double* __restrict__ h2,
                                                              double* __restrict__ pnorm) {
  __shared__ double hs[kMaxKrylov + 8];
  __shared__ double red[24];
  for (int q = threadIdx.x; q < count; q += 256) {
    double t = 0.0;
    for (int b = 0; b < nb; ++b) t += part[(int64_t)b * count + q];
    hs[q] = t;
    if (blockIdx.x == 0) h2[q] = t;
  }
  __syncthreads();
  const int i = blockIdx.x * 256 + threadIdx.x;
  double wi = 0.0;
  if (i < n) {
    double acc = 0.0;
    for (int p = 0; p < count; ++p) acc += hs[p] * v[(int64_t)p * n + i];
    wi = w[i] - acc;
    w[i] = wi;
  }
  const double t = block_sum(wi * wi, red);
  if (threadIdx.x == 0) pnorm[blockIdx.x] = t;
}

__global__ __launch_bounds__(1024) void lanczos_finish_kernel(double* __restrict__ v, int n, int j,
                                                              const double* __restrict__ w,
                                                              const double* __restrict__ pnorm, int nb,
                                                              const double* __restrict__ h1,
                                                              const double* __restrict__ h2,
                                                              double* __restrict__ alpha, double* __restrict__ beta) {
  __shared__ double red[24];
  double part = 0.0;
  for (int b = threadIdx.x; b < nb; b += 1024) part += pnorm[b];
  const double nrm = sqrt(block_sum(part, red));
  const double rn = (nrm > 0.0) ? 1.0 / nrm : 0.0;
  double* vn = v + (int64_t)(j + 1) * n;
  for (int i = threadIdx.x; i < n; i += 1024) vn[i] = w[i] * rn;
  if (threadIdx.x == 0) {
    alpha[j] = h1[j] + h2[j];
    beta[j] = nrm;
  }
}

__global__ __launch_bounds__(64) void ritz_select_kernel(const double* __restrict__ cand, int count, int k,
                                                         double* __restrict__ sel) {
  if (threadIdx.x != 0) return;
  auto before = [&](int a, int b) {
    const double fa = fabs(cand[a]), fb = fabs(cand[b]);
    if (fa != fb) return fa > fb;
    if (cand[a] != cand[b]) return cand[a] > cand[b];
    return a < b;
  };
  int prev = -1;
  for (int t = 0; t < k && t < count; ++t) {
    int best = -1;
    for (int c = 0; c < count; ++c) {
      if (prev >= 0 && !before(prev, c)) continue;
      if (best < 0 || before(c, best)) best = c;
    }
    if (best < 0) break;
    sel[t] = cand[best];
    prev = best;
  }
}

__global__ __launch_bounds__(64) void ritz_collect_kernel(const double* __restrict__ beta, const double* __restrict__ z,
                                                          int m, int k, double* __restrict__ rec) {
  if (threadIdx.x == 0) rec[0] = beta[m - 1];
  for (int t = threadIdx.x; t < k; t += 64) rec[1 + t] = z[(int64_t)t * m + (m - 1)];
}

__global__ __launch_bounds__(256) void ritz_kernel(const double* __restrict__ v, int n, int m,
                                                   const double* __restrict__ y, double* __restrict__ u) {
  const int i = blockIdx.x * 256 + threadIdx.x;
  const int c = blockIdx.y;
  if (i >= n) return;
  const double* yc = y + (int64_t)c * m;
  double acc = 0.0;
  for (int p = 0; p < m; ++p) acc += yc[p] * v[(int64_t)p * n + i];
  u[(int64_t)c * n + i] = acc;
}

__global__ __launch_bounds__(1024) void residual_kernel(const double* __restrict__ bu, const double* __restrict__ u,
                                                        int n, const double* __restrict__ theta,
                                                        double* __restrict__ res) {
  __shared__ double red[24];
  const int c = blockIdx.x;
  const double th = theta[c];
  double pr = 0.0, pu = 0.0;
  for (int i = threadIdx.x; i < n; i += 1024) {
    const double ui = u[(int64_t)c * n + i];
    const double r = bu[(int64_t)c * n + i] - th * ui;
    pr += r * r;
    pu += ui * ui;
  }
  const double r2 = block_sum(pr, red);
  const double u2 = block_sum(pu, red);
  if (threadIdx.x == 0) res[c] = (u2 > 0.0) ? sqrt(r2 / u2) : DBL_MAX;
}

__global__ __launch_bounds__(1024) void band_finish_kernel(double* __restrict__ v, int n, int dst, const double* __restrict__ w,
                                                           const double* __restrict__ pnorm, int nb, const double* __restrict__ h1,
                                                           const double* __restrict__ h2, int cnt, double* __restrict__ hcol,
                                                           double* __restrict__ out2) {
  __shared__ double red[24];
  double part = 0.0;
  for (int b = threadIdx.x; b < nb; b += 1024) part += pnorm[b];
  const double nrm2 = block_sum(part, red);
  double hp = 0.0;
  for (int i = threadIdx.x; i < cnt; i += 1024) {
    const double h = h1[i] + h2[i];
    hcol[i] = h;
    hp += h * h;
  }
  const double h2sum = block_sum(hp, red);
  const double nrm = sqrt(nrm2);
  const double rn = (nrm > 0.0) ? 1.0 / nrm : 0.0;
  double* vn = v + (int64_t)dst * n;
  for (int i = threadIdx.x; i < n; i += 1024) vn[i] = w[i] * rn;
  if (threadIdx.x == 0) {
    hcol[cnt] = nrm;
    out2[0] = nrm;
    out2[1] = sqrt(h2sum + nrm2);
  }
}

__global__ __launch_bounds__(64) void band_restart_h_kernel(double* __restrict__ hfull, int mcap, int p, const double* __restrict__ theta) {
  for (int t = threadIdx.x; t < p; t += 64) hfull[(int64_t)t * mcap + t] = theta[t];
}

__global__ __launch_bounds__(256) void band_gather_kernel(const double* __restrict__ hfull, int mcap, int J, double* __restrict__ a) {
  const int t = blockIdx.x * 256 + threadIdx.x;
  if (t >= J * J) return;
  const int i = t / J, j = t - i * J;
  a[t] = (i <= j) ? hfull[(int64_t)j * mcap + i] : hfull[(int64_t)i * mcap + j];
}

}

size_t symv_sym_workspace_doubles(int32_t n) { return symv_sym_workspace_doubles_impl(n); }
hipError_t launch_row_sums_sym(const int32_t* s32, int32_t n, double* sym_part, double* row_sums, int64_t* row_sums_i64,
                               hipStream_t stream) {
  const int nb = (n + SYT - 1) / SYT;
  int64_t* part = reinterpret_cast<int64_t*>(sym_part);
  hipLaunchKernelGGL(rowsums_sym_tiles_kernel, dim3((unsigned)((int64_t)nb * (nb + 1) / 2)), dim3(256), 0, stream, s32, n, nb, part);
  hipLaunchKernelGGL(rowsums_sym_gather_kernel, dim3((unsigned)((n + 255) / 256)), dim3(256), 0, stream, part, n, nb, row_sums,
                     row_sums_i64);
  return hipGetLastError();
}
hipError_t launch_symv_sym_gather(const double* sym_part, int32_t n, double* y, hipStream_t stream) {
  const int nb = (n + SYT - 1) / SYT;
  hipLaunchKernelGGL(symv_sym_gather_kernel, dim3((unsigned)((n + 255) / 256)), dim3(256), 0, stream, sym_part, n, nb, y);
  return hipGetLastError();
}
void launch_centred_matvec(const EigWorkspace& ws, int32_t n, const double* x, double* y, hipStream_t stream) { launch_symv(ws, n, x, y, stream); }

size_t lanczos_workspace_doubles(int32_t n, int32_t k, int32_t mmax) {
  const size_t nb = ((size_t)n + 255) / 256;
  const size_t mcap = (size_t)mmax + 1;
  const size_t pmax = 2 * ((size_t)k + 2);
  const size_t band = 2 * mcap * mcap + 12 * mcap + 2 * pmax * mcap + 4 * pmax + 32;
  return (size_t)(mmax + 1) * n + (size_t)n + (size_t)k * n + 4 * (size_t)(mmax + 2) + 4 * (size_t)k + 16 +
         nb * (size_t)(mmax + 2) + band;
}

namespace {
hipError_t lanczos_band(const EigWorkspace& ws, double* lz, int32_t n, int32_t k, int32_t mmax, double tol, double* lam_sel_host,
                        int* converged, int* band_steps_out, hipStream_t stream, const LanczosMatvec* mv);
inline int band_pmax(int k) { return 2 * (k + 2); }
hipError_t lanczos_single(const EigWorkspace& ws, double* lz, int32_t n, int32_t k, int32_t mmax, double tol,
                          double* lam_sel_host, int* converged, int* steps_out, hipStream_t stream, const LanczosMatvec* mv);
}

hipError_t lanczos_topk(const EigWorkspace& ws, double* lz, int32_t n, int32_t k, int32_t mmax, double tol,
                        double* lam_sel_host, int* converged, int* steps_out, hipStream_t stream, const LanczosMatvec* mv,
                        int* band_steps_out) {
  if (band_steps_out) *band_steps_out = 0;
  const bool band_only = debug_knobs().lanczos_band == 2 || ws.band_only;
  hipError_t e1 = band_only ? hipSuccess : lanczos_single(ws, lz, n, k, mmax, tol, lam_sel_host, converged, steps_out, stream, mv);
  if (band_only) *converged = 0;
  if (e1 != hipSuccess || *converged || debug_knobs().lanczos_band == 0) return e1;
  return lanczos_band(ws, lz, n, k, mmax, tol, lam_sel_host, converged, band_steps_out, stream, mv);
}

namespace {
hipError_t lanczos_single(const EigWorkspace& ws, double* lz, int32_t n, int32_t k, int32_t mmax, double tol,
                          double* lam_sel_host, int* converged, int* steps_out, hipStream_t stream, const LanczosMatvec* mv) {
  auto matvec = [&](const double* v, double* y) -> hipError_t {
    if (!mv) {
      launch_symv(ws, n, v, y, stream);
      return hipSuccess;
    }
    hipError_t e = hipStreamSynchronize(stream);
    if (e != hipSuccess) return e;
    return (*mv)(v, y) == 0 ? hipSuccess : hipErrorUnknown;
  };
  *converged = 0;
  if (steps_out) *steps_out = 0;
  if (mmax > n) mmax = n;
  if (mmax > kMaxKrylov) mmax = kMaxKrylov;
  if (mmax < k + 2 || n < 8) return hipSuccess;
  const unsigned nb = (unsigned)((n + 255) / 256);
  double* V = lz;
  double* w = V + (size_t)(mmax + 1) * n;
  double* bu = w + n;
  double* alpha = bu + (size_t)k * n;
  double* beta = alpha + (mmax + 2);
  double* h1 = beta + (mmax + 2);
  double* h2 = h1 + (mmax + 2);
  double* rec = h2 + (mmax + 2);
  double* part = rec + (4 * (size_t)k + 16);
  double* pnorm = part + (size_t)nb * (mmax + 1);

  EigWorkspace small = ws;
  small.d = alpha;
  small.e = beta;

  hipLaunchKernelGGL(lanczos_init_kernel, dim3(1), dim3(1024), 0, stream, V, n);
  int next_check = 12;
  if (next_check < k + 2) next_check = k + 2;
  if (next_check > mmax) next_check = mmax;
  std::vector<double> cand, pageable;
  std::vector<int32_t> idx;
  double est_prev = 0.0;
  for (int j = 0; j < mmax; ++j) {
    const double* vj = V + (size_t)j * n;
    const int cnt = j + 1;
    {
      const hipError_t em = matvec(vj, w);
      if (em != hipSuccess) return em;
    }
    hipLaunchKernelGGL(cgs_dots_kernel, dim3((unsigned)cnt), dim3(256), 0, stream, V, n, w, h1);
    hipLaunchKernelGGL(cgs_update_dots_kernel, dim3(nb), dim3(256), 0, stream, V, n, cnt, h1, w, part);
    hipLaunchKernelGGL(cgs_update_norm_kernel, dim3(nb), dim3(256), 0, stream, V, n, cnt, part, (int)nb, w, h2, pnorm);
    hipLaunchKernelGGL(lanczos_finish_kernel, dim3(1), dim3(1024), 0, stream, V, n, j, w, pnorm, (int)nb, h1, h2, alpha,
                       beta);
    const int m = j + 1;
    if (m != next_check && m != mmax) continue;
    next_check = (m < 24) ? m + 4 : (m < 64) ? m + 8 : m + m / 2;
    if (next_check > mmax) next_check = mmax;
    if (steps_out) *steps_out = m;

    idx.clear();
    for (int t = 0; t <= k && t < m; ++t) idx.push_back(m - 1 - t);
    for (int t = 0; t <= k; ++t)
      if (t < m - 1 - k) idx.push_back(t);
    const int nc = (int)idx.size();
    double* rec_beta = rec + nc;
    double* rec_res = rec_beta + 1 + k;
    hipError_t e = launch_bisect(small, m, idx.data(), nc, rec, stream);
    if (e != hipSuccess) return e;
    hipLaunchKernelGGL(ritz_select_kernel, dim3(1), dim3(64), 0, stream, rec, nc, k, ws.lam);
    if ((e = launch_inverse_iteration_dev(small, m, k, stream)) != hipSuccess) return e;
    hipLaunchKernelGGL(ritz_collect_kernel, dim3(1), dim3(64), 0, stream, beta, ws.z, m, k, rec_beta);
    hipLaunchKernelGGL(ritz_kernel, dim3(nb, (unsigned)k), dim3(256), 0, stream, V, n, m, ws.z, bu);
    if ((e = hipMemcpyAsync(ws.z, bu, sizeof(double) * (size_t)k * n, hipMemcpyDeviceToDevice, stream)) != hipSuccess)
      return e;
    for (int t = 0; t < k; ++t) {
      const hipError_t em = matvec(ws.z + (size_t)t * n, bu + (size_t)t * n);
      if (em != hipSuccess) return em;
    }
    hipLaunchKernelGGL(residual_kernel, dim3((unsigned)k), dim3(1024), 0, stream, bu, ws.z, n, ws.lam, rec_res);
    const size_t rec_count = (size_t)nc + 1 + 2 * (size_t)k;
    double* hrec = ws.host_rec;
    if (!hrec || rec_count > ws.host_rec_cap) {
      pageable.resize(rec_count);
      hrec = pageable.data();
    }
    if ((e = hipMemcpyAsync(hrec, rec, sizeof(double) * rec_count, hipMemcpyDeviceToHost, stream)) != hipSuccess) return e;
    if ((e = hipStreamSynchronize(stream)) != hipSuccess) return e;
    cand.assign(hrec, hrec + nc);
    const double beta_m = hrec[nc];
    const double* ylast = hrec + nc + 1;
    const double* hres = ylast + k;

    std::vector<int> order(cand.size());
    for (size_t i = 0; i < order.size(); ++i) order[i] = (int)i;
    std::stable_sort(order.begin(), order.end(), [&](int a, int b) {
      const double fa = fabs(cand[a]), fb = fabs(cand[b]);
      if (fa != fb) return fa > fb;
      return cand[a] > cand[b];
    });
    double scale = 0.0;
    for (double c : cand) scale = fmax(scale, fabs(c));
    for (int t = 0; t < k; ++t) lam_sel_host[t] = cand[order[t]];
    if (!(scale > 0.0) || !std::isfinite(scale)) return hipSuccess;
    std::vector<double> gap((size_t)k);
    for (int t = 0; t < k; ++t) {
      double g = DBL_MAX;
      for (size_t c2 = 0; c2 < cand.size(); ++c2)
        if ((int)c2 != order[t]) g = fmin(g, fabs(cand[c2] - lam_sel_host[t]));
      gap[(size_t)t] = g;
    }
    auto accept = [&](double r, int t) { return r <= tol * scale && (r <= 1e-8 * gap[(size_t)t] || r <= 1e-13 * scale); };
    bool ok = true;
    for (int t = 0; t < k; ++t) ok = ok && accept(fabs(beta_m * ylast[t]), t);
    const bool breakdown = beta_m <= 1e-14 * scale;
    bool verified = true;
    for (int t = 0; t < k; ++t) verified = verified && std::isfinite(hres[t]) && accept(hres[t] * 0.125, t);
    if (!ok && !breakdown) {
      if (m == mmax) return hipSuccess;
      double est_now = 0.0;
      for (int t = 0; t < k; ++t) est_now = fmax(est_now, fabs(beta_m * ylast[t]) / scale);
      const bool stalled = m >= 128 && est_prev > 0.0 && est_now > 0.25 * est_prev;
      est_prev = est_now;
      if (stalled) return hipSuccess;
      continue;
    }
    if (verified) {
      *converged = 1;
      return hipGetLastError();
    }
    if (breakdown || m == mmax) return hipSuccess;
  }
  return hipGetLastError();
}

hipError_t lanczos_band(const EigWorkspace& ws, double* lz, int32_t n, int32_t k, int32_t mmax, double tol, double* lam_sel_host,
                        int* converged, int* band_steps_out, hipStream_t stream, const LanczosMatvec* mv) {
  auto matvec = [&](const double* v, double* y) -> hipError_t {
    if (!mv) {
      launch_symv(ws, n, v, y, stream);
      return hipSuccess;
    }
    hipError_t e = hipStreamSynchronize(stream);
    if (e != hipSuccess) return e;
    return (*mv)(v, y) == 0 ? hipSuccess : hipErrorUnknown;
  };
  *converged = 0;
  if (mmax > n) mmax = n;
  if (mmax > kMaxKrylov) mmax = kMaxKrylov;
  const int ma = mmax;
  if (debug_knobs().lanczos_band_mmax > 0 && debug_knobs().lanczos_band_mmax < mmax) mmax = debug_knobs().lanczos_band_mmax;
  const int bw0 = std::min<int>(k + 2, n);
  const int pk = std::min<int>(2 * bw0, band_pmax(k));
  if (mmax < 4 * pk + 2 || n < 8) return hipSuccess;
  const unsigned nb = (unsigned)((n + 255) / 256);
  const int mcap = ma + 1;
  double* V = lz;
  double* w = V + (size_t)(ma + 1) * n;
  double* bu = w + n;
  double* alpha = bu + (size_t)k * n;
  double* beta = alpha + (ma + 2);
  double* h1 = beta + (ma + 2);
  double* h2 = h1 + (ma + 2);
  double* rec0 = h2 + (ma + 2);
  double* part = rec0 + (4 * (size_t)k + 16);
  double* pnorm = part + (size_t)nb * (ma + 1);
  double* hfull = pnorm + nb;
  double* hdense = hfull + (size_t)mcap * mcap;
  double* hd = hdense + (size_t)mcap * mcap;
  double* he = hd + mcap;
  double* htau = he + mcap;
  double* hq = htau + mcap;
  double* hw = hq + mcap;
  double* hscr = hw + 2 * (size_t)mcap;
  double* hout = hscr + 6 * (size_t)mcap;
  double* hz = hout + (size_t)band_pmax(k) * mcap;
  double* rec = hz + (size_t)band_pmax(k) * mcap;
  double* out2 = rec + (3 * (size_t)band_pmax(k) + 8);
  double* hlam = out2 + 2;

  EigWorkspace hs = ws;
  hs.a = hdense; hs.d = hd; hs.e = he; hs.tau = htau; hs.q = hq; hs.w = hw; hs.scratch = hscr; hs.wy = nullptr;
  hs.z = hz; hs.lam = hlam;

  std::vector<double> pageable;
  auto read_back = [&](const double* src, size_t count, double** host) -> hipError_t {
    double* hrec = ws.host_rec;
    if (!hrec || count > ws.host_rec_cap) {
      pageable.resize(count);
      hrec = pageable.data();
    }
    hipError_t e = hipMemcpyAsync(hrec, src, sizeof(double) * count, hipMemcpyDeviceToHost, stream);
    if (e != hipSuccess) return e;
    if ((e = hipStreamSynchronize(stream)) != hipSuccess) return e;
    *host = hrec;
    return hipSuccess;
  };
  hipError_t e = hipMemsetAsync(hfull, 0, sizeof(double) * (size_t)mcap * mcap, stream);
  if (e != hipSuccess) return e;

  hipLaunchKernelGGL(lanczos_init_kernel, dim3(1), dim3(1024), 0, stream, V, n, 0u);
  int cnt = 1;
  for (int t = 1; t < bw0; ++t) {
    hipLaunchKernelGGL(lanczos_init_kernel, dim3(1), dim3(1024), 0, stream, w, n, (uint32_t)t);
    hipLaunchKernelGGL(cgs_dots_kernel, dim3((unsigned)cnt), dim3(256), 0, stream, V, n, w, h1);
    hipLaunchKernelGGL(cgs_update_dots_kernel, dim3(nb), dim3(256), 0, stream, V, n, cnt, h1, w, part);
    hipLaunchKernelGGL(cgs_update_norm_kernel, dim3(nb), dim3(256), 0, stream, V, n, cnt, part, (int)nb, w, h2, pnorm);
    hipLaunchKernelGGL(lanczos_finish_kernel, dim3(1), dim3(1024), 0, stream, V, n, cnt - 1, w, pnorm, (int)nb, h1, h2, alpha, beta);
    cnt += 1;
  }
  double anorm = 0.0;
  int next_check = std::max(12, 3 * bw0);
  std::vector<double> cand;
  std::vector<int32_t> idx;
  const int cap = mmax - pk;
  const int64_t budget = 40LL * mmax;
  int64_t columns = 0;
  int j = 0;
  for (;;) {
    {
      const hipError_t em = matvec(V + (size_t)j * n, w);
      if (em != hipSuccess) return em;
    }
    columns += 1;
    hipLaunchKernelGGL(cgs_dots_kernel, dim3((unsigned)cnt), dim3(256), 0, stream, V, n, w, h1);
    hipLaunchKernelGGL(cgs_update_dots_kernel, dim3(nb), dim3(256), 0, stream, V, n, cnt, h1, w, part);
    hipLaunchKernelGGL(cgs_update_norm_kernel, dim3(nb), dim3(256), 0, stream, V, n, cnt, part, (int)nb, w, h2, pnorm);
    const bool room = cnt < cap;
    hipLaunchKernelGGL(band_finish_kernel, dim3(1), dim3(1024), 0, stream, V, n, cnt, w, pnorm, (int)nb, h1, h2, cnt,
                       hfull + (size_t)j * mcap, out2);
    double* h2v = nullptr;
    if ((e = read_back(out2, 2, &h2v)) != hipSuccess) return e;
    const double nrm = h2v[0];
    anorm = fmax(anorm, h2v[1]);
    if (!std::isfinite(nrm) || !std::isfinite(anorm)) return hipSuccess;
    if (room && nrm > 1e-9 * anorm) cnt += 1;
    const int J = j + 1;
    j += 1;
    if (band_steps_out) *band_steps_out = (int)std::min<int64_t>(columns, 0x7fffffff);
    const bool exhausted = (J == cnt);
    const bool full = !exhausted && cnt >= cap && J + bw0 >= cnt;
    const bool out_of_budget = columns >= budget;
    const bool last = exhausted || out_of_budget;
    if (J != next_check && !last && !full) continue;
    if (J < k + 2 && !exhausted) continue;
    next_check = (J < 64) ? J + 8 : J + J / 4;

    if (J < 2) return hipSuccess;
    hipLaunchKernelGGL(band_gather_kernel, dim3((unsigned)((J * J + 255) / 256)), dim3(256), 0, stream, hfull, mcap, J, hdense);
    if ((e = launch_tridiagonalize(hs, J, stream)) != hipSuccess) return e;
    const int kk = std::min(k, J);
    const int pw = full ? std::min(pk, J - 1) : kk;
    idx.clear();
    for (int t = 0; t <= pw && t < J; ++t) idx.push_back(J - 1 - t);
    for (int t = 0; t <= pw; ++t)
      if (t < J - 1 - pw) idx.push_back(t);
    const int nc = (int)idx.size();
    double* rec_res = rec + nc;
    if ((e = launch_bisect(hs, J, idx.data(), nc, rec, stream)) != hipSuccess) return e;
    hipLaunchKernelGGL(ritz_select_kernel, dim3(1), dim3(64), 0, stream, rec, nc, pw, hlam);
    if ((e = launch_inverse_iteration_dev(hs, J, pw, stream)) != hipSuccess) return e;
    if ((e = launch_backtransform(hs, J, pw, 0, 1, hout, stream)) != hipSuccess) return e;
    hipLaunchKernelGGL(ritz_kernel, dim3(nb, (unsigned)kk), dim3(256), 0, stream, V, n, J, hout, bu);
    if ((e = hipMemcpyAsync(ws.z, bu, sizeof(double) * (size_t)kk * n, hipMemcpyDeviceToDevice, stream)) != hipSuccess) return e;
    for (int t = 0; t < kk; ++t) {
      const hipError_t em = matvec(ws.z + (size_t)t * n, bu + (size_t)t * n);
      if (em != hipSuccess) return em;
    }
    hipLaunchKernelGGL(residual_kernel, dim3((unsigned)kk), dim3(1024), 0, stream, bu, ws.z, n, hlam, rec_res);
    double* hrec = nullptr;
    if ((e = read_back(rec, (size_t)nc + kk, &hrec)) != hipSuccess) return e;
    cand.assign(hrec, hrec + nc);
    const double* hres = hrec + nc;
    std::vector<int> order(cand.size());
    for (size_t i = 0; i < order.size(); ++i) order[i] = (int)i;
    std::stable_sort(order.begin(), order.end(), [&](int a, int b) {
      const double fa = fabs(cand[a]), fb = fabs(cand[b]);
      if (fa != fb) return fa > fb;
      return cand[a] > cand[b];
    });
    double scale = 0.0;
    for (double c : cand) scale = fmax(scale, fabs(c));
    if (!(scale > 0.0) || !std::isfinite(scale)) return hipSuccess;
    if (kk < k) return hipSuccess;
    for (int t = 0; t < k; ++t) lam_sel_host[t] = cand[order[t]];
    bool tight = true, loose = true;
    for (int t = 0; t < k; ++t) {
      double g = DBL_MAX;
      for (size_t c2 = 0; c2 < cand.size(); ++c2)
        if ((int)c2 != order[t]) g = fmin(g, fabs(cand[c2] - lam_sel_host[t]));
      const double r = hres[t];
      const bool fin = std::isfinite(r);
      loose = loose && fin && r * 0.125 <= tol * scale;
      tight = tight && fin && r * 0.125 <= tol * scale && (r * 0.125 <= 1e-8 * g || r <= 1e-13 * scale);
    }
    if (tight || (last && loose)) {
      *converged = 1;
      return hipGetLastError();
    }
    if (last) return hipSuccess;
    if (!full) continue;

    hipLaunchKernelGGL(ritz_kernel, dim3(nb, (unsigned)pw), dim3(256), 0, stream, V, n, J, hout, V + (size_t)cnt * n);
    const int carry = cnt - J;
    if ((e = hipMemcpyAsync(V, V + (size_t)cnt * n, sizeof(double) * (size_t)pw * n, hipMemcpyDeviceToDevice, stream)) != hipSuccess) return e;
    if (carry > 0 &&
        (e = hipMemcpyAsync(V + (size_t)pw * n, V + (size_t)J * n, sizeof(double) * (size_t)carry * n, hipMemcpyDeviceToDevice, stream)) != hipSuccess)
      return e;
    if ((e = hipMemsetAsync(hfull, 0, sizeof(double) * (size_t)mcap * mcap, stream)) != hipSuccess) return e;
    hipLaunchKernelGGL(band_restart_h_kernel, dim3(1), dim3(64), 0, stream, hfull, mcap, pw, hlam);
    cnt = pw + carry;
    j = pw;
    next_check = j + std::max(8, 2 * bw0);
  }
}

}

}
```

### spark-examples_amd/csrc/pcoa_capi.hip

```cpp
#include <cstdio>
#include <cstring>
#include <new>

#include "pcoa_ctx.h"

using namespace pcoa;

namespace {

thread_local std::string g_create_error;

int64_t knob_limit(int64_t x, int64_t dflt) { return (x > 0 && x < dflt) ? x : dflt; }

}

namespace pcoa {

int fail(pcoa_ctx* c, int code, const std::string& msg) {
  if (c) c->last_error = msg; else g_create_error = msg;
  return code;
}

int hip_fail(pcoa_ctx* c, hipError_t e, const char* what) {
  std::string m = std::string(what) + ": " + hipGetErrorString(e);
// ... 99 lines not shown
  }
  {
    const int64_t by_mem = (((int64_t)4 << 30) / gram_packed_npad(n_samples)) / 1536 * 1536;
    c->pack_chunk = std::max<int64_t>(1536, std::min<int64_t>(c->pack_chunk, by_mem));
  }
  if (knobs.pack_chunk > 0 && knobs.pack_chunk <= ((int64_t)1 << 24)) c->pack_chunk = knobs.pack_chunk;
  c->max_launch = knob_limit(knobs.max_launch, kMaxLaunchVariants);
  c->fold_threshold = knob_limit(knobs.fold_threshold, kFoldThreshold);
  auto bail = [&](hipError_t err, const char* what) {
    int rc = hip_fail(c, err, what);
    g_create_error = c->last_error;
    pcoa_destroy(c);
    return rc;
  };
  if ((e = hipSetDevice(device_ordinal)) != hipSuccess) return bail(e, "hipSetDevice");
  hipDeviceProp_t prop;
  if ((e = hipGetDeviceProperties(&prop, device_ordinal)) != hipSuccess) return bail(e, "hipGetDeviceProperties");
  c->num_cu = prop.multiProcessorCount > 0 ? prop.multiProcessorCount : 256;
  std::snprintf(c->dev_name, sizeof(c->dev_name), "%s (%s)", prop.name, prop.gcnArchName);
  if ((e = hipStreamCreateWithFlags(&c->own_stream, hipStreamNonBlocking)) != hipSuccess)
    return bail(e, "hipStreamCreate");
  c->stream = c->own_stream;
  if (strip && !c->use_i8) {
    pcoa_destroy(c);
    return fail(nullptr, PCOA_ERR_INVALID_ARG, "a strip owner needs a packed-operand engine (PCOA_GRAM_KERNEL=f32 is set)");
  }
  const size_t nn = s_count(c);
  if (!op) {
    if ((e = dev_alloc((void**)&c->s32, sizeof(int32_t) * nn, c->device)) != hipSuccess) return bail(e, "allocation of S");
    if (zero_s && (e = hipMemsetAsync(c->s32, 0, sizeof(int32_t) * nn, c->stream)) != hipSuccess) return bail(e, "memset(S)");
  }
  if ((e = dev_alloc((void**)&c->zeros, 4096, c->device)) != hipSuccess) return bail(e, "allocation of the zero page");
  if ((e = hipMemsetAsync(c->zeros, 0, 4096, c->stream)) != hipSuccess) return bail(e, "memset(zeros)");
  if ((e = dev_alloc((void**)&c->err_flag, 16, c->device)) != hipSuccess) return bail(e, "allocation of the flag words");
  if ((e = hipMemsetAsync(c->err_flag, 0, 16, c->stream)) != hipSuccess) return bail(e, "memset(flag)");
  if ((e = hipHostMalloc((void**)&c->hw, sizeof(pcoa_ctx::HostWords), hipHostMallocDefault)) != hipSuccess)
    return bail(e, "hipHostMalloc(landing words)");
  std::memset(c->hw, 0, sizeof(pcoa_ctx::HostWords));
  if ((e = hipStreamSynchronize(c->stream)) != hipSuccess) return bail(e, "hipStreamSynchronize");
  *out = c;
  return PCOA_OK;
}

namespace pcoa {
int create_full_engine_unfilled(pcoa_ctx** out, int32_t n_samples, int32_t device_ordinal, uint32_t flags) {
  return create_impl(out, n_samples, device_ordinal, flags, 0, -1, false, false);
}
int create_grm_engine(pcoa_ctx** out, int32_t n_samples, int32_t device_ordinal, uint32_t flags) {
  return create_impl(out, n_samples, device_ordinal, flags, 0, -1, true, true, true);
}
}

extern "C" {

const char* pcoa_version(void) { return "pcoa_hip 0.10 (gfx950)"; }

int pcoa_create(pcoa_ctx** out, int32_t n_samples, int32_t device_ordinal, uint32_t flags) {
  return create_impl(out, n_samples, device_ordinal, flags, 0, -1);
}

int pcoa_create_strip(pcoa_ctx** out, int32_t n_samples, int32_t col0, int32_t cols, int32_t device_ordinal,
                      uint32_t flags) {
  if (cols < 0) return fail(nullptr, PCOA_ERR_INVALID_ARG, "cols must be positive");
  return create_impl(out, n_samples, device_ordinal, flags, col0, cols);
}

int pcoa_create_operator(pcoa_ctx** out, int32_t n_samples, int32_t device_ordinal, uint32_t flags) {
  return create_impl(out, n_samples, device_ordinal, flags, 0, -1, true);
}

void pcoa_destroy(pcoa_ctx* c) {
  if (!c) return;
  (void)hipSetDevice(c->device);
  if (c->stream) (void)hipStreamSynchronize(c->stream);
  if (c->pack_stream) (void)hipStreamSynchronize(c->pack_stream);
  if (c->gram_stream) (void)hipStreamSynchronize(c->gram_stream);
  if (c->csr_stream) (void)hipStreamSynchronize(c->csr_stream);
  for (auto& p : c->pending) { (void)hipEventDestroy(p.a); (void)hipEventDestroy(p.b); }
  for (auto& ev : c->pool) (void)hipEventDestroy(ev);
  for (auto& b : c->fb) {
    if (b.packed) (void)hipEventDestroy(b.packed);
    if (b.consumed) (void)hipEventDestroy(b.consumed);
    if (b.p) dev_free(b.p);
  }
  if (c->ev_fork) (void)hipEventDestroy(c->ev_fork);
  for (StagingRing* r : {&c->cs, &c->bs, &c->ts}) staging_destroy(*r);
  if (c->csr_stream) (void)hipStreamDestroy(c->csr_stream);
  if (c->csr_flag) dev_free(c->csr_flag);
  if (c->csr_flag_host) (void)hipHostFree(c->csr_flag_host);
  if (c->fb_flags_host) (void)hipHostFree(c->fb_flags_host);
  if (c->hw) (void)hipHostFree(c->hw);
  if (c->ws.host_rec) (void)hipHostFree(c->ws.host_rec);
  void* bufs[] = {c->s32, c->s64, c->s64_spare, c->narrow_flag, c->zeros, c->err_flag, c->tile, c->csr_idx, c->csr_offs, c->thr_dev,
                  c->sample_pop, c->measure_diag, c->measure_q, c->xfer, c->coll, c->fb_flags, c->strip_ws, c->strip_means, c->proj_ws, c->pack_buf, c->lanczos_ws, c->sym_part, c->ws.a, c->ws.d, c->ws.e, c->ws.tau, c->ws.q, c->ws.w, c->ws.lam,
                  c->ws.z, c->ws.wy, c->ws.scratch, c->ws.iscratch, c->row_sums, c->colmean, c->stats, c->nz,
                  c->out_dev};
  for (void* b : bufs)
    if (b) dev_free(b);
  operator_destroy(c);
  grm_destroy(c);
  loadings_destroy(c);
  ld_destroy(c);
  complete_destroy(c);
  king_destroy(c);
  if (c->pack_stream) (void)hipStreamDestroy(c->pack_stream);
  if (c->gram_stream) (void)hipStreamDestroy(c->gram_stream);
  if (c->own_stream) (void)hipStreamDestroy(c->own_stream);
  delete c;
}

const char* pcoa_last_error(const pcoa_ctx* c) { return c ? c->last_error.c_str() : g_create_error.c_str(); }

int pcoa_n_samples(const pcoa_ctx* c) { return c ? c->n : PCOA_ERR_INVALID_ARG; }

int pcoa_set_stream(pcoa_ctx* c, void* hip_stream) {
  CHECK_CTX(c);
  int rc = fp4_flush(c);
  if (rc != PCOA_OK) return rc;
  HIP_TRY(c, hipStreamSynchronize(c->stream));
  drain_events(c, true);
  c->stream = hip_stream ? (hipStream_t)hip_stream : c->own_stream;
  return PCOA_OK;
}

int pcoa_sync(pcoa_ctx* c) {
  CHECK_CTX(c);
  int rc = fp4_sync_point(c);
  if (rc != PCOA_OK) return rc;
  HIP_TRY(c, hipStreamSynchronize(c->stream));
  return PCOA_OK;
}

int pcoa_reserve(pcoa_ctx* c, int64_t variants_per_call, int32_t num_pc) {
  CHECK_CTX(c);
  if (variants_per_call < 0 || num_pc < 0 || num_pc > c->n)
    return fail(c, PCOA_ERR_INVALID_ARG, "reserve: variants_per_call < 0 or num_pc outside [0, n]");
  if (c->is_operator) return operator_reserve(c, num_pc);
  int rc = PCOA_OK;
  if (variants_per_call > 0 && c->use_i8 && c->packed_mode != 2) {
    if ((rc = fp4_setup(c)) != PCOA_OK) return rc;
    const int64_t chunk = std::min(std::min(variants_per_call, c->max_launch), c->pack_chunk);
    for (int bi = 0; bi < c->fb_count; ++bi) {
      pcoa_ctx::Fp4Buf& b = c->fb[bi];
      if (b.kb > 0 || b.launched) continue;
      const int64_t kb = kb_of(c, chunk);
      if (b.cap_kb >= std::max(kb, chunk >= ((int64_t)1 << 18) ? fp4_target_kb(c) : kb)) continue;
      if ((rc = fp4_grow(c, bi, kb, chunk)) != PCOA_OK) return rc;
    }
  }
  if (num_pc > 0 && !c->is_strip) {
    if ((rc = ensure_workspace(c, num_pc)) != PCOA_OK) return rc;
    if (c->n >= 32 && !(c->flags & PCOA_FLAG_EIG_HOUSEHOLDER)) {
      const int32_t mmax = std::min<int32_t>(c->n, 512);
      if ((rc = ensure(c, &c->lanczos_ws, &c->lanczos_cap, (int64_t)lanczos_workspace_doubles(c->n, num_pc, mmax))) != PCOA_OK)
        return rc;
    } else if ((rc = ensure_b(c)) != PCOA_OK) {
      return rc;
    }
  }
  HIP_TRY(c, hipStreamSynchronize(c->stream));
  return PCOA_OK;
}

int pcoa_reset(pcoa_ctx* c) {
  CHECK_CTX(c);
  int rc = fp4_discard(c);
  if (rc != PCOA_OK) return rc;
  ld_drop_tail(c);
  if (c->is_operator) return operator_reset(c);
  const size_t nn = s_count(c);
  HIP_TRY(c, hipMemsetAsync(c->s32, 0, sizeof(int32_t) * nn, c->stream));
  if (c->s64) HIP_TRY(c, hipMemsetAsync(c->s64, 0, sizeof(int64_t) * nn, c->stream));
  HIP_TRY(c, hipMemsetAsync(c->err_flag, 0, 16, c->stream));
  c->variants_in_s32 = 0;
  c->dirty = false;
  c->strip_centering_set = false;
  return PCOA_OK;
}

int pcoa_get_timings_sized(pcoa_ctx* c, pcoa_timings* out_user, size_t out_size) {
  CHECK_CTX(c);
  if (!out_user || out_size < sizeof(double)) return fail(c, PCOA_ERR_INVALID_ARG, "out is NULL or out_size too small");
  int rc0 = fp4_sync_point(c);
  if (rc0 != PCOA_OK) return rc0;
  drain_events(c, true);
  pcoa_timings full;
  pcoa_timings* out = &full;
  std::memset(out, 0, sizeof(*out));
  out->gram_kernel_seconds = c->tsec[T_GRAM];
  out->gram_kernel_launches = c->gram_launches;
  out->gram_variants = c->gram_variants;
  out->gram_flops = c->gram_flops;
  out->gram_bytes = c->gram_bytes;
  out->densify_seconds = c->tsec[T_DENSIFY];
  out->synth_seconds = c->tsec[T_SYNTH];
  out->finalize_seconds = c->tsec[T_FINALIZE];
  out->center_seconds = c->tsec[T_CENTER];
  out->tridiag_seconds = c->tsec[T_TRIDIAG];
  out->eig_seconds = c->tsec[T_EIG];
  out->backtransform_seconds = c->tsec[T_BACK];
  out->compute_total_seconds = c->compute_total;
  out->gram_kernel_kind = c->gram_kind;
  out->lanczos_seconds = c->tsec[T_LANCZOS];
  out->eig_method = c->eig_method;
  out->lanczos_steps = c->lanczos_steps;
  out->fp4_fallbacks = c->fp4_fallbacks;
  out->lockstep_launches = c->lockstep_launches;
  out->pipeline_launches = c->pipeline_launches;
  out->evensplit_launches = c->evensplit_launches;
  out->operand_bits = !c->use_i8 ? 32 : c->gram_kind == 2 ? 8 : c->op_fmt == 2 ? 1 : 4;
  {
    const int ls = c->pipe_ok ? gram_lockstep_splitk(c->n, c->pipe_gram_cus) : 0;
    int wgs = ls > 0 ? gram_lockstep_workgroups(c->n, ls) : 0;
    if (c->pipe_ok && c->op_fmt == 2 && !(c->coreside && c->coreside_mode == 2)) wgs = c->pipe_gram_cus;
    out->pipeline_pre_pass_cus = c->pipe_ok ? (c->coreside ? c->num_cu : c->num_cu - wgs) : 0;
    out->pipeline_contraction_cus = wgs;
  }
  out->pack_seconds = c->tsec[T_PACK];
  out->pack_launches = c->pack_launches;
  out->pack_bytes = c->pack_bytes;
  out->csr_stage_seconds = c->csr_stage_s;
  out->csr_wait_seconds = c->csr_wait_s;
  out->csr_fast_chunks = c->csr_fast_chunks;
  out->csr_redo_chunks = c->csr_redo_chunks;
  out->allreduce_seconds = c->tsec[T_ALLREDUCE];
  out->allreduce_calls = c->allreduce_calls;
  out->comm_ranks = c->comm_ranks;
  out->allreduce_int32 = c->allreduce_int32;
  out->matvec_form = c->matvec_form;
  out->gram_i64_live = c->s64 ? 1 : 0;
  out->reduce_int32_calls = c->reduce_i32_calls;
  out->narrowed_to_int32 = c->narrowed;
  out->lanczos_block_steps = c->lanczos_block_steps;
  out->eig_dense_form = c->eig_dense_form;
  out->operator_products = c->op_products;
  out->operator_matvec_seconds = c->tsec[T_OPERATOR];
  out->operator_store_bytes = operator_store_bytes(c);
  out->subset_seconds = c->tsec[T_SUBSET];
  out->subset_bytes = c->subset_bytes;
  std::memcpy(out_user, out, std::min(out_size, sizeof(full)));
  return PCOA_OK;
}

int pcoa_get_reduce_peers_stats(pcoa_ctx* c, pcoa_reduce_peers_stats* out_user, size_t out_size) {
  CHECK_CTX(c);
  if (!out_user || out_size < sizeof(int64_t)) return fail(c, PCOA_ERR_INVALID_ARG, "out is NULL or out_size too small");
  int rc0 = fp4_sync_point(c);
  if (rc0 != PCOA_OK) return rc0;
  drain_events(c, true);
  pcoa_reduce_peers_stats full;
  std::memset(&full, 0, sizeof(full));
  full.reduce_peers_calls = c->reduce_peers_calls;
  full.reduce_peers_seconds = c->tsec[T_REDUCE_PEERS];
  full.reduce_peers_bytes_in = c->reduce_peers_bytes_in;
  std::memcpy(out_user, &full, std::min(out_size, sizeof(full)));
  return PCOA_OK;
}

static_assert(offsetof(pcoa_timings, csr_stage_seconds) == PCOA_TIMINGS_R03_BYTES, "the r03 prefix of pcoa_timings is frozen");
int pcoa_get_timings(pcoa_ctx* c, pcoa_timings* out) { return pcoa_get_timings_sized(c, out, PCOA_TIMINGS_R03_BYTES); }

int pcoa_reset_timings(pcoa_ctx* c) {
  CHECK_CTX(c);
  int rc0 = fp4_sync_point(c);
  if (rc0 != PCOA_OK) return rc0;
  drain_events(c, true);
  for (double& t : c->tsec) t = 0;
  c->csr_stage_s = c->csr_wait_s = 0;
  c->csr_fast_chunks = c->csr_redo_chunks = 0;
  c->allreduce_calls = 0;
  c->reduce_i32_calls = c->narrowed = 0;
  c->gram_launches = 0;
  c->gram_variants = 0;
  c->gram_flops = c->gram_bytes = 0;
  c->compute_total = 0;
  c->pack_launches = 0;
  c->pack_bytes = 0;
  c->lockstep_launches = 0;
  c->pipeline_launches = 0;
  c->evensplit_launches = 0;
  c->op_products = 0;
  c->subset_bytes = 0;
  c->pairs_bytes = c->pairs_calls = 0;
  c->king_bytes = c->king_calls = 0;
  c->ld_variants = c->ld_bytes = 0;
  c->ldp_seen = c->ldp_kept = c->ldp_mono = c->ldp_pairs = 0;
  c->reduce_peers_calls = c->reduce_peers_bytes_in = 0;
  return PCOA_OK;
}

int pcoa_device_info(pcoa_ctx* c, char* name_out, int32_t name_cap, int32_t* cu_count_out) {
  CHECK_CTX(c);
  if (name_out && name_cap > 0) {
    std::strncpy(name_out, c->dev_name, (size_t)name_cap - 1);
    name_out[name_cap - 1] = 0;
  }
  if (cu_count_out) *cu_count_out = c->num_cu;
  return PCOA_OK;
}

}
```

### spark-examples_amd/csrc/pcoa_internal.h

```cpp
#ifndef PCOA_INTERNAL_H_
#define PCOA_INTERNAL_H_

#include <hip/hip_runtime.h>
#include <stdint.h>

#include <functional>
#include <string>
#include <vector>

#include "pcoa.h"

namespace pcoa {

constexpr int kWave = 64;
constexpr int kNumXcd = 8;

struct DebugKnobs {
  int gram_kernel = -1;
  int64_t pack_chunk = 0;
  int64_t max_launch = 0;
  int64_t fold_threshold = 0;
  int pipeline = -1;
  int explicit_center = 0;
  int lockstep = -1;
// ... 83 lines not shown
hipError_t launch_symmetrize_i32(int32_t* s32, int32_t n, hipStream_t stream);
hipError_t launch_fold_i32_to_i64(int32_t* s32, int64_t* s64, int64_t count, hipStream_t stream);
hipError_t launch_export_i64(const int32_t* s32, const int64_t* s64_or_null, int64_t* dst, int64_t count,
                             hipStream_t stream);
hipError_t launch_plink_bed_to_bits(const uint8_t* bed, int64_t row_bytes, int64_t nv, int32_t n, int64_t words, int ref_a1,
                                    uint32_t* bits, hipStream_t stream);
hipError_t launch_add_i64(int64_t* dst, const int64_t* src, int64_t count, hipStream_t stream);
hipError_t launch_add_i32(int32_t* dst, const int32_t* src, int64_t count, hipStream_t stream);
hipError_t launch_narrow_i64_to_i32(const int64_t* s64, int32_t* s32, int64_t count, int32_t* flag, hipStream_t stream);
hipError_t launch_synth_fill_f32(uint64_t seed, const uint32_t* thresholds_dev, const int32_t* sample_pop_dev,
                                 int32_t n_pops, int64_t first_variant, int64_t nv, int32_t n, float* x_dev,
                                 int64_t ld, hipStream_t stream);

hipError_t launch_synth_kbits(uint64_t seed, const uint32_t* thresholds_dev, const int32_t* sample_pop_dev, int32_t n_pops,
                              int64_t first_variant, int64_t nv, int32_t n, int32_t npad, int8_t* p, int64_t nblk_out,
                              hipStream_t stream);

constexpr int32_t kSubsetTileCols = 1024;
constexpr int32_t kSubsetBandRows = 32;
hipError_t launch_subset_gather_i32(const int32_t* src, int32_t n, const int32_t* keep_dev, int32_t m, int32_t* dst,
                                    hipStream_t stream);
hipError_t launch_subset_gather_i64(const int64_t* src, int32_t n, const int32_t* keep_dev, int32_t m, int64_t* dst,
                                    hipStream_t stream);

constexpr int32_t kPairsTileCols = 1024;
constexpr int32_t kPairsBandRows = 32;
constexpr int32_t kPairsMaxSamples = 1 << 30;
int32_t pairs_tiles(int32_t n);
int64_t pairs_count_pass_entries(int32_t n);
hipError_t launch_pairs_diag(const int32_t* s32, const int64_t* s64_or_null, int32_t n, int64_t* diag, hipStream_t stream);
hipError_t launch_pairs_count(const int32_t* s32, const int64_t* s64_or_null, int32_t n, const int64_t* diag, double x,
                              int32_t* cnt, hipStream_t stream);
hipError_t launch_pairs_scan(int32_t* cnt, int32_t n, int64_t* rowoff, hipStream_t stream);
hipError_t launch_pairs_write(const int32_t* s32, const int64_t* s64_or_null, int32_t n, const int64_t* diag, double x,
                              const int32_t* prefix, const int64_t* rowoff, int64_t capacity, pcoa_pair* out,
                              unsigned long long* entries_read, hipStream_t stream);

struct KingMatrices { const int32_t* p[PCOA_KING_PLANES]; };
struct KingPlaneRows { uint32_t* p[PCOA_KING_PLANES]; };
constexpr int kKingFlagV = 0, kKingFlagIbs0 = 1, kKingFlagHetSum = 2, kKingFlagSHm = 3, kKingFlagWords = 4;
hipError_t launch_plink_bed_to_king_planes(const uint8_t* bed, int64_t row_bytes, int64_t nv, int32_t n, int64_t words,
                                           const KingPlaneRows& out, hipStream_t stream);
hipError_t launch_king_diag(const KingMatrices& g, int32_t n, int64_t* h, int64_t* hm, int64_t* v, int32_t* flag, hipStream_t stream);
hipError_t launch_king_count(const KingMatrices& g, int32_t n, const int64_t* h, const int64_t* hm, const int64_t* v, double x,
                             int32_t* cnt, int32_t* flag, hipStream_t stream);
hipError_t launch_king_write(const KingMatrices& g, int32_t n, const int64_t* h, const int64_t* hm, const int64_t* v, double x,
                             const int32_t* prefix, const int64_t* rowoff, int64_t capacity, pcoa_king_pair* out,
                             unsigned long long* entries_read, hipStream_t stream);

constexpr int32_t kOperatorRangeRows = 512;
constexpr int32_t kOperatorSegmentAlign = 2048;
constexpr int32_t kOperatorGroupWords = 256;
int32_t operator_pitch_words(int32_t n);
int32_t operator_groups(int32_t n);
hipError_t launch_operator_append(const uint32_t* src, int64_t ld_words, int64_t nv, int32_t n, uint32_t* dst, hipStream_t stream);
hipError_t launch_operator_xv(const uint32_t* seg, int32_t rows, int32_t n, const double* v, double* tpart, int64_t vstride,
                              hipStream_t stream);
hipError_t launch_operator_combine_t(const double* tpart, int64_t vstride, int32_t n, int64_t rows, double* t, hipStream_t stream);
hipError_t launch_operator_xt_f64(const uint32_t* seg, int32_t rows, int32_t n, const double* t, double* ypart, hipStream_t stream);
hipError_t launch_operator_xt_i64(const uint32_t* seg, int32_t rows, int32_t n, const int32_t* cnt, int64_t* ipart,
                                  hipStream_t stream);
hipError_t launch_operator_popcount(const uint32_t* seg, int32_t rows, int32_t n, int32_t* cnt, hipStream_t stream);
hipError_t launch_operator_dots(const double* v, const double* means, int32_t n, double* dots, hipStream_t stream);
hipError_t launch_operator_finish(const double* ypart, int32_t nranges, int32_t n, const double* means, const double* stats,
                                  const double* dots, int centred, double* y, hipStream_t stream);
hipError_t launch_operator_row_sums_finish(const int64_t* ipart, int32_t nranges, int32_t n, int64_t* rs_i64, double* rs_f64,
                                           hipStream_t stream);

constexpr int32_t kGrmRangeRows = 512;
constexpr int32_t kGrmSegmentAlign = 2048;
constexpr int32_t kGrmGroupWords = 256;
int32_t grm_pitch_words(int32_t n);
int32_t grm_groups(int32_t n);
hipError_t launch_grm_append(const uint8_t* src, int64_t row_bytes, int64_t nv, int32_t n, int swap, uint32_t* dst, hipStream_t stream);
hipError_t launch_grm_counts(const uint32_t* seg, int32_t rows, int32_t n, int32_t* cnt, hipStream_t stream);
hipError_t launch_grm_weights(const int32_t* cnt, int64_t rows, double min_maf, double* mu, double* d, int32_t* used,
                              unsigned long long* mprime, hipStream_t stream);
hipError_t launch_grm_ax(const uint32_t* seg, int32_t rows, int32_t n, const double* mu, const double* x, double* tpart,
                         int64_t vstride, hipStream_t stream);
hipError_t launch_grm_combine_t(const double* tpart, int64_t vstride, int32_t n, int64_t rows, const double* mu, const double* d,
                                double* t, double* s, hipStream_t stream);
hipError_t launch_grm_at(const uint32_t* seg, int32_t rows, int32_t n, const double* t, const double* s, double* ypart,
                         hipStream_t stream);
hipError_t launch_grm_called(const uint32_t* seg, int32_t rows, int32_t n, const int32_t* used, int32_t* ipart, hipStream_t stream);
hipError_t launch_grm_finish(const double* ypart, int32_t nranges, int32_t n, const unsigned long long* mprime, double* y,
                             hipStream_t stream);
hipError_t launch_grm_called_finish(const int32_t* ipart, int32_t nranges, int32_t n, int32_t* nz, hipStream_t stream);

int32_t loadings_lanes(int32_t n);
int loadings_chunk(int32_t remaining);
hipError_t launch_loadings(const uint32_t* bits, int64_t nv, int64_t ld_words, int32_t n, const double* u, int64_t ustride, int32_t k,
                           const double* div, double* out, int32_t num_pc, hipStream_t stream);

int32_t ld_band_tile_rows();
int32_t ld_band_chunk_words();
hipError_t launch_ld_count(const uint32_t* rows, int64_t ld, int64_t vc, int32_t n, uint32_t* wb_rows, int32_t* cnt_rows,
                           hipStream_t stream);
hipError_t launch_ld_band(const uint32_t* wb, const int32_t* cnt, int64_t vc, int32_t n, int32_t window, int32_t tail, double t,
                          uint32_t* ex, hipStream_t stream);
hipError_t launch_ld_resolve(const uint32_t* ex, const int32_t* cnt_rows, int64_t vc, int32_t n, int32_t window, int64_t g0,
                             uint32_t* flags, uint32_t* kbits, hipStream_t stream);
hipError_t launch_ld_scan(const uint32_t* kbits, int64_t g0, const int32_t* cnt_rows, int64_t vc, int32_t n, uint8_t* keep,
                          int32_t* pos, int64_t* out2, hipStream_t stream);
hipError_t launch_ld_gather(const uint32_t* wb_rows, const uint8_t* keep, const int32_t* pos, int64_t vc, int32_t n, uint32_t* out,
                            hipStream_t stream);

hipError_t launch_col_means(const double* row_sums, int32_t n, double* cm, hipStream_t stream);
hipError_t launch_center(const int32_t* s32, const int64_t* s64_or_null, int32_t n, double* row_sums,
                         double* stats, int32_t* nz, double* b, hipStream_t stream, bool row_sums_done = false);

int64_t strip_ws_doubles(int32_t n, int32_t cols);
hipError_t launch_strip_col_sums(const int32_t* s32, const int64_t* s64_or_null, int32_t n, int32_t cols, double* ws,
                                 hipStream_t stream);
hipError_t launch_strip_matvec(const int32_t* s32, const int64_t* s64_or_null, int32_t n, int32_t col0, int32_t cols,
                               const double* v, const double* means, double matrix_mean, double* ws, hipStream_t stream);
hipError_t launch_strip_col_sums_to(const int32_t* s32, const int64_t* s64_or_null, int32_t n, int32_t cols, double* ws,
                                    int64_t* out_i64, double* out_f64, hipStream_t stream);
hipError_t launch_strip_matvec_to(const int32_t* s32, const int64_t* s64_or_null, int32_t n, int32_t col0, int32_t cols,
                                  const double* v, const double* means, double matrix_mean, double* ws, double* y_out,
                                  hipStream_t stream);

int64_t project_ws_doubles(int32_t n_ref, int32_t cols, int32_t k);
int project_chunk(int32_t remaining);
hipError_t launch_project(const int32_t* s32, const int64_t* s64_or_null, int32_t n_ref, int32_t cols, const double* colsum,
                          const double* means, double matrix_mean, const double* u, int32_t k, const double* lam, double* ws,
                          double* out, hipStream_t stream);

constexpr int32_t EIG_FORM_FUSED = 1;
constexpr int32_t EIG_FORM_FUSED_BIG_LDS = 2;
constexpr int32_t EIG_FORM_TWO_KERNEL = 4;
constexpr int32_t EIG_FORM_BISECT_LDS = 8;
constexpr int32_t EIG_FORM_INVIT_LDS = 16;
constexpr int32_t EIG_FORM_INVIT_PER_VECTOR = 32;
constexpr int32_t EIG_FORM_WY_BACKTRANSFORM = 64;
struct EigWorkspace {
  double* a;
  double* d;
  double* e;
  double* tau;
  double* q;
  double* w;
  double* lam;
  double* z;
  double* scratch;
  int32_t* iscratch;
  double* wy;
  double* host_rec = nullptr;
  size_t host_rec_cap = 0;
  const int32_t* s32;
  const int64_t* s64;
  const double* colmean;
  const double* stats;
  double* sym_part = nullptr;
  bool band_only = false;
  int measure = 0;
  const int64_t* diag = nullptr;
  const double* qcos = nullptr;
  const int32_t* comp_q32 = nullptr;
  const int64_t* comp_c = nullptr;
  int64_t comp_v = 0;
};
size_t symv_sym_workspace_doubles(int32_t n);
hipError_t launch_row_sums_sym(const int32_t* s32, int32_t n, double* sym_part, double* row_sums, int64_t* row_sums_i64,
                               hipStream_t stream);
void launch_centred_matvec(const EigWorkspace& ws, int32_t n, const double* x, double* y, hipStream_t stream);
hipError_t launch_symv_sym_gather(const double* sym_part, int32_t n, double* y, hipStream_t stream);

hipError_t launch_measure_diag(const int32_t* s32, const int64_t* s64_or_null, int32_t n, int kind, int64_t* diag, double* q,
                               hipStream_t stream);
hipError_t launch_measure_row_sums(const int32_t* s32, const int64_t* s64_or_null, int32_t n, int kind, const int64_t* diag,
                                   const double* q, double* ones, double* row_sums, hipStream_t stream);
hipError_t launch_measure_row_sums_sym(const int32_t* s32, int32_t n, int kind, const int64_t* diag, const double* q,
                                       double* ones, double* sym_part, double* row_sums, hipStream_t stream);
hipError_t launch_measure_stats(const double* row_sums, int32_t n, double* stats, int32_t* nz, hipStream_t stream);
hipError_t launch_measure_center(const int32_t* s32, const int64_t* s64_or_null, int32_t n, int kind, const int64_t* diag,
                                 const double* q, const double* cm, const double* stats, double* b, hipStream_t stream);
hipError_t launch_measure_symv(const EigWorkspace& ws, int32_t n, const double* x, double* y, hipStream_t stream);

hipError_t launch_complete_diag(const int32_t* q32, int32_t n, int64_t v, int64_t* c, int32_t* flag, hipStream_t stream);
hipError_t launch_complete_row_sums(const int32_t* s32, const int64_t* s64_or_null, const int32_t* q32, int32_t n, const int64_t* c,
                                    int64_t v, double* ones, double* row_sums, hipStream_t stream);
hipError_t launch_complete_row_sums_sym(const int32_t* s32, const int32_t* q32, int32_t n, const int64_t* c, int64_t v, double* ones,
                                        double* sym_part, double* row_sums, hipStream_t stream);
hipError_t launch_complete_center(const int32_t* s32, const int64_t* s64_or_null, const int32_t* q32, int32_t n, const int64_t* c,
                                  int64_t v, const double* cm, const double* stats, double* b, hipStream_t stream);
hipError_t launch_complete_symv(const EigWorkspace& ws, int32_t n, const double* x, double* y, hipStream_t stream);
hipError_t launch_plink_bed_to_bits_pair(const uint8_t* bed, int64_t row_bytes, int64_t nv, int32_t n, int64_t words, int ref_a1,
                                         uint32_t* bits, uint32_t* miss, hipStream_t stream);
hipError_t launch_tridiagonalize(const EigWorkspace& ws, int32_t n, hipStream_t stream, int32_t* form = nullptr);
hipError_t launch_bisect(const EigWorkspace& ws, int32_t n, const int32_t* idx_host, int32_t count,
                         double* lam_out_dev, hipStream_t stream, int32_t* form = nullptr);
hipError_t launch_inverse_iteration(const EigWorkspace& ws, int32_t n, const double* lam_sel_host, int32_t k,
                                    hipStream_t stream, int32_t* form = nullptr);
hipError_t launch_inverse_iteration_dev(const EigWorkspace& ws, int32_t n, int32_t k, hipStream_t stream);
size_t wy_workspace_doubles(int32_t n, int32_t k);
hipError_t launch_backtransform(const EigWorkspace& ws, int32_t n, int32_t k, int sign_normalize,
                                int apply_reflectors, double* out_dev, hipStream_t stream, int32_t* form = nullptr);

size_t lanczos_workspace_doubles(int32_t n, int32_t k, int32_t mmax);
typedef std::function<int(const double*, double*)> LanczosMatvec;
hipError_t lanczos_topk(const EigWorkspace& ws, double* lz, int32_t n, int32_t k, int32_t mmax, double tol,
                        double* lam_sel_host, int* converged, int* steps_out, hipStream_t stream,
                        const LanczosMatvec* mv = nullptr, int* band_steps_out = nullptr);

}

#endif
```

### spark-examples_amd/engine.py

```python
import ctypes

import numpy as np

from . import _lib as L


class PcoaError(RuntimeError):
    def __init__(self, code, message):
        RuntimeError.__init__(self, "pcoa error %d: %s" % (code, message))
        self.code = code


class IndexRangeError(PcoaError, IndexError):
    """A callset index outside [0, N): the reference throws NoSuchElementException /
    IndexOutOfBounds here (VariantsPca.scala:59, :188)."""


def _ptr(a):
    return ctypes.c_void_p(a.ctypes.data)


_BITS_ROWS = (np.uint32, "int32", "bits must be 2-D [variants][words]")
_BED_ROWS = (np.uint8, "uint8", "rows must be [variants][row_bytes]")

# ... 147 lines not shown

    def accumulate_callsets(self, callsets):
        offs = np.zeros(len(callsets) + 1, dtype=np.int64)
        for v, c in enumerate(callsets):
            offs[v + 1] = offs[v] + len(c)
        idx = np.fromiter((i for c in callsets for i in c), dtype=np.int32, count=int(offs[-1]))
        self.accumulate_calls(idx, offs)

    def accumulate_dense(self, x, n_variants=None, ld=None):
        if hasattr(x, "data_ptr") and getattr(x, "is_cuda", False):
            import torch
            assert x.dtype == torch.float32 and x.dim() == 2 and x.stride(1) == 1
            nv = int(x.shape[0]) if n_variants is None else int(n_variants)
            ldv = int(x.stride(0)) if ld is None else int(ld)
            self._keepalive.append(x)
            torch.cuda.current_stream(x.device).synchronize()
            self._check(self._lib.pcoa_accumulate_dense_f32(self._ctx, ctypes.c_void_p(x.data_ptr()), nv, ldv, 1))
            return
        a = np.ascontiguousarray(x, dtype=np.float32)
        if a.ndim != 2:
            raise ValueError("x must be 2-D [variants][samples]")
        nv = a.shape[0] if n_variants is None else int(n_variants)
        ldv = a.shape[1] if ld is None else int(ld)
        self._check(self._lib.pcoa_accumulate_dense_f32(self._ctx, _ptr(a), nv, ldv, 0))

    def accumulate_dense_u8(self, x, n_variants=None, ld=None):
        if hasattr(x, "data_ptr") and getattr(x, "is_cuda", False):
            import torch
            assert x.dtype == torch.uint8 and x.dim() == 2 and x.stride(1) == 1
            nv = int(x.shape[0]) if n_variants is None else int(n_variants)
            ldv = int(x.stride(0)) if ld is None else int(ld)
            self._keepalive.append(x)
            torch.cuda.current_stream(x.device).synchronize()
            self._check(self._lib.pcoa_accumulate_dense_u8(self._ctx, ctypes.c_void_p(x.data_ptr()), nv, ldv, 1))
            return
        a = np.ascontiguousarray(x, dtype=np.uint8)
        if a.ndim != 2:
            raise ValueError("x must be 2-D [variants][samples]")
        nv = a.shape[0] if n_variants is None else int(n_variants)
        ldv = a.shape[1] if ld is None else int(ld)
        self._check(self._lib.pcoa_accumulate_dense_u8(self._ctx, _ptr(a), nv, ldv, 0))

    def accumulate_bits(self, bits, n_variants=None, ld_words=None):
        ptr, nv, ldv, dev, keep = _rows_arg(bits, *_BITS_ROWS)
        if dev:
            self._keepalive.append(keep)
        self._check(self._lib.pcoa_accumulate_bits(self._ctx, ptr, nv if n_variants is None else int(n_variants),
                                                   ldv if ld_words is None else int(ld_words), int(dev)))

    def accumulate_plink_bed(self, rows, ref_is_a1=False, asynchronous=False):
        ptr, nv, stride, source = self._bed_arg(rows, asynchronous)
        self._check(self._lib.pcoa_accumulate_plink_bed(self._ctx, ptr, nv, stride, int(bool(ref_is_a1)), source))

    def _bed_arg(self, rows, asynchronous):
        ptr, nv, stride, dev, keep = _rows_arg(rows, *_BED_ROWS, pinned=asynchronous)
        if dev:
            self._keepalive.append(keep)
        return ptr, nv, stride, L.PCOA_BED_HOST_ASYNC if asynchronous else int(dev)

    def accumulate_plink_bed_calls(self, rows, companion, ref_is_a1=False, asynchronous=False):
        ptr, nv, stride, source = self._bed_arg(rows, asynchronous)
        self._check(self._lib.pcoa_accumulate_plink_bed_calls(self._ctx, companion._ctx, ptr, nv, stride, int(bool(ref_is_a1)), source))

    def accumulate_dense_device_ptr(self, ptr, n_variants, ld):
        self._check(self._lib.pcoa_accumulate_dense_f32(self._ctx, ctypes.c_void_p(int(ptr)), int(n_variants),
                                                        int(ld), 1))

    def _synth_params(self, seed, pop_offsets, thresholds):
        po = np.ascontiguousarray(pop_offsets, dtype=np.int32)
        th = np.ascontiguousarray(thresholds, dtype=np.uint32)
        p = L.PcoaSynthParams()
        p.seed = int(seed)
        p.n_pops = int(po.size - 1)
        p.pop_offsets = po.ctypes.data_as(ctypes.POINTER(ctypes.c_int32))
        p.thresholds = th.ctypes.data_as(ctypes.POINTER(ctypes.c_uint32))
        return p, (po, th)

    def accumulate_synthetic(self, seed, pop_offsets, thresholds, first_variant):
        th = np.asarray(thresholds)
        p, keep = self._synth_params(seed, pop_offsets, th)
        self._check(self._lib.pcoa_accumulate_synthetic(self._ctx, ctypes.byref(p), int(first_variant),
                                                        int(th.shape[0])))
        del keep

    def synth_fill(self, seed, pop_offsets, thresholds, first_variant, x_dev_ptr, ld):
        th = np.asarray(thresholds)
        p, keep = self._synth_params(seed, pop_offsets, th)
        self._check(self._lib.pcoa_synth_fill_f32(self._ctx, ctypes.byref(p), int(first_variant), int(th.shape[0]),
                                                  ctypes.c_void_p(int(x_dev_ptr)), int(ld)))
        del keep

    def finalize(self):
        self._check(self._lib.pcoa_gram_finalize(self._ctx))

    def gram(self):
        out = np.zeros((self.n, self.cols), dtype=np.int64)
        self._check(self._lib.pcoa_gram_read_i64(self._ctx, _ptr(out)))
        return out

    def gram_block(self, row0, col0, rows, cols):
        out = np.zeros((int(rows), int(cols)), dtype=np.int64)
        self._check(self._lib.pcoa_gram_read_block_i64(self._ctx, int(row0), int(col0), int(rows), int(cols), _ptr(out)))
        return out

    def load_gram(self, s):
        a = np.ascontiguousarray(s, dtype=np.int64)
        if a.shape != (self.n, self.cols):
            raise ValueError("expected an %d x %d matrix" % (self.n, self.cols))
        self._check(self._lib.pcoa_gram_load_i64(self._ctx, _ptr(a)))

    def lanczos(self, matvec, num_pc, max_steps=512, tol=1e-11, first_check=12, trace=None):
        import torch
        n, k = self.n, int(num_pc)
        dev = torch.device("cuda", self.device)

        class _Ptr(object):
            def __init__(self, addr):
                self.__cuda_array_interface__ = {"shape": (n,), "typestr": "<f8", "data": (int(addr), False), "version": 2}

        failure = []

        def call(_user, v_ptr, y_ptr):
            try:
                v = torch.as_tensor(_Ptr(v_ptr), device=dev)
                y = torch.as_tensor(_Ptr(y_ptr), device=dev)
                y.copy_(matvec(v))
                torch.cuda.current_stream(dev).synchronize()
                return 0
            except BaseException as exc:
                failure.append(exc)
                return 1

        cb = L.MATVEC_FN(call)
        comps = np.zeros((k, n), dtype=np.float64)
        lam = np.zeros(k, dtype=np.float64)
        steps = ctypes.c_int32(0)
        rc = self._lib.pcoa_lanczos_with_matvec(self._ctx, k, cb, None, _ptr(comps), _ptr(lam), ctypes.byref(steps))
        if failure:
            raise failure[0]
        if trace is not None:
            trace.append((int(steps.value), lam.copy(), None))
        if rc == L.PCOA_ERR_NOT_CONVERGED:
            raise RuntimeError("Lanczos over strips did not reach a verified residual in %d steps (tiny spectral gaps?); there "
                               "is no dense fallback for a matrix tiled across GPUs" % int(steps.value))
        self._check(rc)
        return np.ascontiguousarray(comps.T), lam

    def debug_centred_matvec(self, x, form):
        x = np.ascontiguousarray(x, dtype=np.float64)
        y = np.zeros(self.n, dtype=np.float64)
        self._check(self._lib.pcoa_debug_centred_matvec(self._ctx, _ptr(x), _ptr(y), int(form)))
        return y

    def reduce_from(self, other):
        self._check(self._lib.pcoa_gram_reduce_from(self._ctx, other._ctx))

    def subset(self, keep):
        idx = np.ascontiguousarray(keep, dtype=np.int32)
        if idx.ndim != 1:
            raise ValueError("keep must be one-dimensional")
        ctx = ctypes.c_void_p()
        self._check(self._lib.pcoa_create_subset(ctypes.byref(ctx), self._ctx, _ptr(idx) if idx.size else None, int(idx.size)))
        sub = object.__new__(PcoaEngine)
        sub._lib, sub._ctx = self._lib, ctx
        sub.strip, sub.operator = None, False
        sub.n = sub.cols = int(idx.size)
        sub.device = self.device
        sub._keepalive = []
        return sub

    PAIR_DTYPE = np.dtype([("i", np.int32), ("j", np.int32), ("shared", np.int64)])

    def similar_pairs(self, min_jaccard, capacity=1 << 20):
        cap = int(capacity)
        pairs = np.zeros(max(cap, 0), dtype=self.PAIR_DTYPE)
        diag = np.zeros(self.n, dtype=np.int64)
        found = ctypes.c_int64(0)
        self._check(self._lib.pcoa_similar_pairs(self._ctx, float(min_jaccard), _ptr(pairs) if cap > 0 else None, cap,
                                                 ctypes.byref(found), _ptr(diag)))
        n_found = int(found.value)
        return pairs[:min(n_found, cap)], n_found, diag

    KING_PAIR_DTYPE = np.dtype([("i", np.int32), ("j", np.int32), ("hethet", np.int64), ("ibs0", np.int64),
                                ("het_sum", np.int64)])

    @staticmethod
    def _king_planes(planes):
        planes = list(planes) if planes is not None else None
        if planes is not None and len(planes) != L.PCOA_KING_PLANES:
            raise ValueError("planes must be %d engines (het, missing, het_or_missing, hom_a1, hom_a2)" % L.PCOA_KING_PLANES)
        lib = L.load()
        if planes is None:
            return lib, None, None
        arr = (ctypes.c_void_p * L.PCOA_KING_PLANES)(*[p._ctx if p is not None else None for p in planes])
        return lib, planes[0], arr

    @staticmethod
    def _king_check(lib, first, rc):
        if rc != L.PCOA_OK:
            msg = lib.pcoa_last_error(first._ctx if first is not None else None)
            raise PcoaError(rc, msg.decode() if msg else "")

    @staticmethod
    def accumulate_plink_bed_king(planes, rows, asynchronous=False):
        lib, first, arr = PcoaEngine._king_planes(planes)
        if first is not None:
            ptr, nv, stride, source = first._bed_arg(rows, asynchronous)
        else:
            a = np.ascontiguousarray(rows, dtype=np.uint8)
            ptr, nv, stride, source = _ptr(a), a.shape[0], a.shape[1], 0
        PcoaEngine._king_check(lib, first, lib.pcoa_accumulate_plink_bed_king(arr, ptr, nv, stride, source))

    @staticmethod
    def king_pairs(planes, min_kinship, capacity=1 << 20):
        lib, first, arr = PcoaEngine._king_planes(planes)
        cap = int(capacity)
        pairs = np.zeros(max(cap, 0), dtype=PcoaEngine.KING_PAIR_DTYPE)
        n = first.n if first is not None else 0
        het = np.zeros(n, dtype=np.int64)
        found, v = ctypes.c_int64(0), ctypes.c_int64(0)
        PcoaEngine._king_check(lib, first, lib.pcoa_king_pairs(arr, float(min_kinship), _ptr(pairs) if cap > 0 else None, cap,
                                                                ctypes.byref(found), ctypes.byref(v), _ptr(het) if n else None))
        n_found = int(found.value)
        return pairs[:min(n_found, cap)], n_found, int(v.value), het

    def king_stats(self):
        k = L.PcoaKingStats()
        self._check(self._lib.pcoa_get_king_stats(self._ctx, ctypes.byref(k), ctypes.sizeof(k)))
        return dict((f[0], getattr(k, f[0])) for f in L.PcoaKingStats._fields_)

    SIMILARITY_KINDS = {"shared": 0, "jaccard": 1, "cosine": 2}

    def set_similarity(self, kind):
        if isinstance(kind, str):
            if kind not in self.SIMILARITY_KINDS:
                raise ValueError("similarity kind must be one of shared, jaccard, cosine, not %r" % (kind,))
            kind = self.SIMILARITY_KINDS[kind]
        self._check(self._lib.pcoa_set_similarity(self._ctx, int(kind)))

    def get_similarity(self):
        kind = ctypes.c_int32(-1)
        self._check(self._lib.pcoa_get_similarity(self._ctx, ctypes.byref(kind)))
        return dict((v, k) for k, v in self.SIMILARITY_KINDS.items())[int(kind.value)]

    def set_call_companion(self, other, n_variants=0):
        self._check(self._lib.pcoa_set_call_companion(self._ctx, other._ctx if other is not None else None, int(n_variants)))
        self._companion = other

    def get_call_companion(self):
        ctx, v = ctypes.c_void_p(), ctypes.c_int64(0)
        self._check(self._lib.pcoa_get_call_companion(self._ctx, ctypes.byref(ctx), ctypes.byref(v)))
        if not ctx.value:
            return None, 0
        mine = getattr(self, "_companion", None)
        if mine is not None and mine._ctx is not None and mine._ctx.value == ctx.value:
            return mine, int(v.value)
        view = object.__new__(PcoaEngine)
        view._lib, view._ctx, view._borrowed = self._lib, ctx, True
        view.strip, view.operator = None, False
        view.n = view.cols = self.n
        view.device = self.device
        view._keepalive = []
        return view, int(v.value)

    def export_device(self, dst_ptr):
        self._check(self._lib.pcoa_gram_export_device_i64(self._ctx, ctypes.c_void_p(int(dst_ptr))))

    def import_device(self, src_ptr):
        self._check(self._lib.pcoa_gram_import_device_i64(self._ctx, ctypes.c_void_p(int(src_ptr))))

    def comm_unique_id(self):
        buf = (ctypes.c_uint8 * 128)()
        self._check(self._lib.pcoa_comm_unique_id(ctypes.cast(buf, ctypes.c_void_p)))
        return bytes(buf)

    def comm_init(self, unique_id, rank, n_ranks):
        buf = (ctypes.c_uint8 * 128).from_buffer_copy(unique_id)
        comm = ctypes.c_void_p()
        self._check(self._lib.pcoa_comm_init(self._ctx, ctypes.cast(buf, ctypes.c_void_p), int(rank), int(n_ranks),
                                             ctypes.byref(comm)))
        return comm

    def comm_runtime(self):
        buf = ctypes.create_string_buffer(1024)
        ver = ctypes.c_int32(0)
        self._check(self._lib.pcoa_comm_runtime(buf, 1024, ctypes.byref(ver)))
        return buf.value.decode(), int(ver.value)

    def comm_destroy(self, comm):
        self._check(self._lib.pcoa_comm_destroy(comm))

    def comm_count(self, comm):
        n = ctypes.c_int32(0)
        self._check(self._lib.pcoa_comm_count(comm, ctypes.byref(n)))
        return int(n.value)

    def allreduce_rccl(self, comm):
        self._check(self._lib.pcoa_gram_allreduce_rccl(self._ctx, comm))

    def strip_col_sums(self):
        out = np.zeros(self.cols, dtype=np.float64)
        self._check(self._lib.pcoa_strip_col_sums(self._ctx, _ptr(out)))
        return out

    def strip_matvec(self, v, means, matrix_mean):
        v = np.ascontiguousarray(v, dtype=np.float64)
# ... 318 lines not shown
```

Before: 467.4 million.

## Fuse Lanczos matvec with normalization and replace Ritz bisection with one tridiag kernel

Adds a fused Lanczos step kernel that combines the matvec with normalization of the previous vector, the alpha partial dot and the first CGS projection dots. The CGS update kernel gains a fused variant that finishes the alpha reduction itself. The Ritz extraction's bisection, selection, inverse iteration and collect kernels are replaced by a single LDS-resident tridiagonal eigensolver kernel that uses DPP wave reductions, and the extra device-to-device copy of Ritz vectors is dropped. The aim is fewer kernel launches and fewer passes over memory per Lanczos step, at the cost of more workspace and more complex kernels. This touches only the PCoA eigen stage, so its share of total wall-clock time is probably small.

```diff
diff --git a/include/pcoa.h b/include/pcoa.h
--- a/include/pcoa.h
+++ b/include/pcoa.h
@@ -321,6 +321,9 @@
 
 int pcoa_debug_alloc(int32_t device_ordinal, size_t bytes, void** out);
 int pcoa_debug_centred_matvec(pcoa_ctx* ctx, const double* x, double* y, int form);
+int pcoa_debug_ritz_candidates(int32_t m, int32_t k);
+int pcoa_debug_ritz_tridiag(pcoa_ctx* ctx, const double* d, const double* e, int32_t m, int32_t k, double* cand_out, double* sel_out,
+                            double* y_out);
 int pcoa_debug_reduce_chunk(int32_t g, int32_t k, int32_t n_samples, int64_t* first_out, int64_t* count_out);
 int pcoa_debug_free(void* p);
 int pcoa_debug_guard_mode(void);
diff --git a/spark-examples_amd/_lib.py b/spark-examples_amd/_lib.py
--- a/spark-examples_amd/_lib.py
+++ b/spark-examples_amd/_lib.py
@@ -242,6 +242,8 @@
     ("pcoa_get_reduce_peers_stats", ctypes.c_int, [_vp, ctypes.POINTER(PcoaReducePeersStats), ctypes.c_size_t]),
     ("pcoa_lanczos_with_matvec", ctypes.c_int, [_vp, ctypes.c_int32, _vp, _vp, _vp, _vp, ctypes.POINTER(ctypes.c_int32)]),
     ("pcoa_debug_centred_matvec", ctypes.c_int, [_vp, _vp, _vp, ctypes.c_int]),
+    ("pcoa_debug_ritz_candidates", ctypes.c_int, [ctypes.c_int32, ctypes.c_int32]),
+    ("pcoa_debug_ritz_tridiag", ctypes.c_int, [_vp, _vp, _vp, ctypes.c_int32, ctypes.c_int32, _vp, _vp, _vp]),
     ("pcoa_host_alloc_pinned", ctypes.c_int, [ctypes.c_size_t, ctypes.POINTER(ctypes.c_void_p)]),
     ("pcoa_host_free_pinned", ctypes.c_int, [_vp]),
     ("pcoa_accumulate_plink_bed", ctypes.c_int, [_vp, _vp, _i64, _i64, ctypes.c_int, ctypes.c_int]),
diff --git a/spark-examples_amd/csrc/capi_compute.hip b/spark-examples_amd/csrc/capi_compute.hip
--- a/spark-examples_amd/csrc/capi_compute.hip
+++ b/spark-examples_amd/csrc/capi_compute.hip
@@ -234,7 +234,8 @@
   c->lanczos_steps = 0;
   if (try_lanczos) {
     const int32_t mmax = std::min<int32_t>(n, 512);
-    const int64_t need = (int64_t)lanczos_workspace_doubles(n, num_pc, mmax);
+    const bool fused_room = !sym_form && !measured;
+    const int64_t need = (int64_t)(lanczos_workspace_doubles(n, num_pc, mmax) + (fused_room ? lanczos_fused_workspace_doubles(n, mmax) : 0));
     rc = ensure(c, &c->lanczos_ws, &c->lanczos_cap, need);
     if (rc != PCOA_OK) return rc;
     int conv = 0, steps = 0;
@@ -245,6 +246,7 @@
       wl.sym_part = (sym_form && !wl.a) ? c->sym_part : nullptr;
       c->matvec_form = wl.a ? 2 : wl.sym_part ? 1 : 0;
       wl.band_only = (c->flags & PCOA_FLAG_EIG_BAND) != 0;
+      wl.lanczos_fused_room = fused_room;
       if (measured) measure_bind(c, &wl);
       int band = 0;
       HIP_TRY(c, lanczos_topk(wl, c->lanczos_ws, n, num_pc, mmax, 1e-11, sel.data(), &conv, &steps, c->stream, nullptr, &band));
@@ -779,4 +781,31 @@
   return PCOA_OK;
 }
 
-}
+int pcoa_debug_ritz_candidates(int32_t m, int32_t k) { return (m >= 1 && k >= 1) ? ritz_tridiag_candidates(m, k) : 0; }
+int pcoa_debug_ritz_tridiag(pcoa_ctx* c, const double* d, const double* e, int32_t m, int32_t k, double* cand_out, double* sel_out,
+                            double* y_out) {
+  CHECK_CTX(c);
+  if (!d || !e || !cand_out || !sel_out || !y_out) return fail(c, PCOA_ERR_INVALID_ARG, "a NULL array");
+  if (k < 1 || m < k + 2 || m > 512) return fail(c, PCOA_ERR_INVALID_ARG, "need 1 <= k, k + 2 <= m <= 512");
+  int rc = check_device_flags(c);
+  if (rc != PCOA_OK) return rc;
+  const int32_t nc = ritz_tridiag_candidates(m, k);
+  const size_t count = 2 * (size_t)m + (size_t)nc + (size_t)k + (size_t)k * m;
+  if ((rc = ensure(c, &c->lanczos_ws, &c->lanczos_cap, (int64_t)count)) != PCOA_OK) return rc;
+  double* dd = c->lanczos_ws;
+  double* de = dd + m;
+  double* dcand = de + m;
+  double* dsel = dcand + nc;
+  double* dy = dsel + k;
+  HIP_TRY(c, hipMemcpyAsync(dd, d, sizeof(double) * (size_t)m, hipMemcpyHostToDevice, c->stream));
+  HIP_TRY(c, hipMemsetAsync(de, 0, sizeof(double) * (size_t)m, c->stream));
+  HIP_TRY(c, hipMemcpyAsync(de, e, sizeof(double) * (size_t)(m - 1), hipMemcpyHostToDevice, c->stream));
+  HIP_TRY(c, ritz_tridiag(dd, de, m, k, dcand, dsel, dy, c->stream));
+  HIP_TRY(c, hipMemcpyAsync(cand_out, dcand, sizeof(double) * (size_t)nc, hipMemcpyDeviceToHost, c->stream));
+  HIP_TRY(c, hipMemcpyAsync(sel_out, dsel, sizeof(double) * (size_t)k, hipMemcpyDeviceToHost, c->stream));
+  HIP_TRY(c, hipMemcpyAsync(y_out, dy, sizeof(double) * (size_t)k * m, hipMemcpyDeviceToHost, c->stream));
+  HIP_TRY(c, hipStreamSynchronize(c->stream));
+  return PCOA_OK;
+}
+
+}
diff --git a/spark-examples_amd/csrc/eig.hip b/spark-examples_amd/csrc/eig.hip
--- a/spark-examples_amd/csrc/eig.hip
+++ b/spark-examples_amd/csrc/eig.hip
@@ -703,15 +703,6 @@
   return hipGetLastError();
 }
 
-hipError_t launch_inverse_iteration_dev(const EigWorkspace& ws, int32_t n, int32_t k, hipStream_t stream) {
-  size_t lds = 0;
-  hipError_t err = invit_lds_bytes(n, &lds);
-  if (err != hipSuccess) return err;
-  hipLaunchKernelGGL(invit_kernel, dim3(1), dim3(64), lds, stream, ws.d, ws.e, n, ws.lam, k, ws.z, ws.scratch,
-                     ws.iscratch, lds > 0 ? 1 : 0);
-  return hipGetLastError();
-}
-
 hipError_t launch_backtransform(const EigWorkspace& ws, int32_t n, int32_t k, int sign_normalize,
                                 int apply_reflectors, double* out_dev, hipStream_t stream, int32_t* form) {
   const int nref = n - 2;
diff --git a/spark-examples_amd/csrc/eig_lanczos.hip b/spark-examples_amd/csrc/eig_lanczos.hip
--- a/spark-examples_amd/csrc/eig_lanczos.hip
+++ b/spark-examples_amd/csrc/eig_lanczos.hip
@@ -42,30 +42,29 @@
   for (int i = threadIdx.x; i < n; i += 1024) v0[i] *= rn;
 }
 
-__global__ __launch_bounds__(256) void symv_kernel(const double* __restrict__ a, int n,
-                                                   const double* __restrict__ x, double* __restrict__ y) {
-  const int lane = threadIdx.x & 63;
-  const int i = blockIdx.x * 4 + (threadIdx.x >> 6);
-  if (i >= n) return;
+__device__ __forceinline__ double symv_row(const double* __restrict__ a, int n, const double* __restrict__ x, int i, int lane) {
   const double* row = a + (int64_t)i * n;
   auto quad = [&](int j, double* out) {
     const double2 lo = *reinterpret_cast<const double2*>(row + j), hi = *reinterpret_cast<const double2*>(row + j + 2);
     out[0] = lo.x; out[1] = lo.y; out[2] = hi.x; out[3] = hi.y;
   };
   auto one = [&](int j) -> double { return row[j]; };
-  const double acc = row_dot(quad, one, x, n, lane);
-  if (lane == 0) y[i] = acc;
-}
-
-template <bool HAS64>
-__global__ __launch_bounds__(256) void symv_centered_kernel(const int32_t* __restrict__ s32,
-                                                            const int64_t* __restrict__ s64, int n,
-                                                            const double* __restrict__ cm,
-                                                            const double* __restrict__ stats,
-                                                            const double* __restrict__ x, double* __restrict__ y) {
+  return row_dot(quad, one, x, n, lane);
+}
+
+__global__ __launch_bounds__(256) void symv_kernel(const double* __restrict__ a, int n,
+                                                   const double* __restrict__ x, double* __restrict__ y) {
   const int lane = threadIdx.x & 63;
   const int i = blockIdx.x * 4 + (threadIdx.x >> 6);
   if (i >= n) return;
+  const double acc = symv_row(a, n, x, i, lane);
+  if (lane == 0) y[i] = acc;
+}
+
+template <bool HAS64>
+__device__ __forceinline__ double symv_centered_row(const int32_t* __restrict__ s32, const int64_t* __restrict__ s64, int n,
+                                                    const double* __restrict__ cm, const double* __restrict__ stats,
+                                                    const double* __restrict__ x, int i, int lane) {
   const int64_t base = (int64_t)i * n;
   const double row_mean = cm[i];
   const double mmean = stats[1];
@@ -92,8 +91,73 @@
     const double data = HAS64 ? (double)((int64_t)s32[base + j] + s64[base + j]) : (double)s32[base + j];
     return centre(data, cm[j]);
   };
-  const double acc = row_dot(quad, one, x, n, lane);
+  return row_dot(quad, one, x, n, lane);
+}
+
+template <bool HAS64>
+__global__ __launch_bounds__(256) void symv_centered_kernel(const int32_t* __restrict__ s32,
+                                                            const int64_t* __restrict__ s64, int n,
+                                                            const double* __restrict__ cm,
+                                                            const double* __restrict__ stats,
+                                                            const double* __restrict__ x, double* __restrict__ y) {
+  const int lane = threadIdx.x & 63;
+  const int i = blockIdx.x * 4 + (threadIdx.x >> 6);
+  if (i >= n) return;
+  const double acc = symv_centered_row<HAS64>(s32, s64, n, cm, stats, x, i, lane);
   if (lane == 0) y[i] = acc;
+}
+
+template <int FORM>
+__global__ __launch_bounds__(256) void lanczos_matvec_fused_kernel(const double* __restrict__ a, const int32_t* __restrict__ s32,
+                                                                   const int64_t* __restrict__ s64, int n,
+                                                                   const double* __restrict__ cm, const double* __restrict__ stats,
+                                                                   int rows4, int j, const double* __restrict__ x,
+                                                                   const double* __restrict__ pnorm, int nb,
+                                                                   double* __restrict__ vj, const double* __restrict__ wrows,
+                                                                   double* __restrict__ wj, double* __restrict__ apart,
+                                                                   const double* __restrict__ h1prev, const double* __restrict__ h2,
+                                                                   double* __restrict__ h1out, double* __restrict__ alpha,
+                                                                   double* __restrict__ beta) {
+  __shared__ double red[24];
+  const int lane = threadIdx.x & 63, wave = threadIdx.x >> 6;
+  double nrm = 1.0, rn = 1.0;
+  if (pnorm) {
+    double t = 0.0;
+    for (int b = lane; b < nb; b += 64) t += pnorm[b];
+    nrm = sqrt(__shfl(wave_sum(t), 0, 64));
+    rn = (nrm > 0.0) ? 1.0 / nrm : 0.0;
+  }
+  if ((int)blockIdx.x >= rows4) {
+    const int p = (int)blockIdx.x - rows4;
+    const double* wp = wrows + (int64_t)p * n;
+    double part = 0.0;
+    for (int i = threadIdx.x; i < n; i += 256) part += wp[i] * (x[i] * rn);
+    const double t = block_sum(part, red);
+    if (threadIdx.x == 0) h1out[p] = t;
+    return;
+  }
+  const int i = blockIdx.x * 4 + wave;
+  double share = 0.0;
+  if (i < n) {
+    double acc;
+    if (FORM == 0) acc = symv_row(a, n, x, i, lane);
+    else acc = symv_centered_row<FORM == 2>(s32, s64, n, cm, stats, x, i, lane);
+    if (lane == 0) {
+      const double vi = x[i] * rn, yi = acc * rn;
+      if (pnorm) vj[i] = vi;
+      wj[i] = yi;
+      share = vi * yi;
+    }
+  }
+  if (lane == 0) red[wave] = share;
+  __syncthreads();
+  if (threadIdx.x == 0) {
+    apart[blockIdx.x] = (red[0] + red[1]) + (red[2] + red[3]);
+    if (blockIdx.x == 0 && pnorm) {
+      alpha[j - 1] = h1prev[j - 1] + h2[j - 1];
+      beta[j - 1] = nrm;
+    }
+  }
 }
 
 
@@ -416,17 +480,30 @@
 
 constexpr int kMaxKrylov = 512;
 
+template <bool FUSED>
 __global__ __launch_bounds__(256) void cgs_update_dots_kernel(const double* __restrict__ v, int n, int count,
-                                                              const double* __restrict__ h, double* __restrict__ w,
-                                                              double* __restrict__ part) {
+                                                              double* h, const double* win, double* w,
+                                                              double* __restrict__ part, const double* __restrict__ apart,
+                                                              int napart) {
   __shared__ double red[4][kMaxKrylov + 8];
   const int i = blockIdx.x * 256 + threadIdx.x;
   const int lane = threadIdx.x & 63, wave = threadIdx.x >> 6;
   const bool in = i < n;
   const int ic = in ? i : n - 1;
   double acc = 0.0;
-  for (int p = 0; p < count; ++p) acc += h[p] * v[(int64_t)p * n + ic];
-  const double wi = in ? w[ic] - acc : 0.0;
+  if (FUSED) {
+    double s = 0.0;
+    for (int b = threadIdx.x; b < napart; b += 256) s += apart[b];
+    const double vlast = v[(int64_t)(count - 1) * n + ic];
+    for (int p = 0; p < count - 1; ++p) acc += h[p] * v[(int64_t)p * n + ic];
+    const double a = block_sum(s, &red[0][0]);
+    __syncthreads();
+    if (blockIdx.x == 0 && threadIdx.x == 0) h[count - 1] = a;
+    acc += a * vlast;
+  } else {
+    for (int p = 0; p < count; ++p) acc += h[p] * v[(int64_t)p * n + ic];
+  }
+  const double wi = in ? win[ic] - acc : 0.0;
   if (in) w[i] = wi;
   for (int q = 0; q < count; ++q) {
     const double t = wave_sum(v[(int64_t)q * n + ic] * wi);
@@ -481,32 +558,321 @@
   }
 }
 
-__global__ __launch_bounds__(64) void ritz_select_kernel(const double* __restrict__ cand, int count, int k,
-                                                         double* __restrict__ sel) {
-  if (threadIdx.x != 0) return;
-  auto before = [&](int a, int b) {
-    const double fa = fabs(cand[a]), fb = fabs(cand[b]);
-    if (fa != fb) return fa > fb;
-    if (cand[a] != cand[b]) return cand[a] > cand[b];
-    return a < b;
-  };
-  int prev = -1;
-  for (int t = 0; t < k && t < count; ++t) {
-    int best = -1;
-    for (int c = 0; c < count; ++c) {
-      if (prev >= 0 && !before(prev, c)) continue;
-      if (best < 0 || before(c, best)) best = c;
-    }
-    if (best < 0) break;
-    sel[t] = cand[best];
-    prev = best;
-  }
-}
-
-__global__ __launch_bounds__(64) void ritz_collect_kernel(const double* __restrict__ beta, const double* __restrict__ z,
-                                                          int m, int k, double* __restrict__ rec) {
-  if (threadIdx.x == 0) rec[0] = beta[m - 1];
-  for (int t = threadIdx.x; t < k; t += 64) rec[1 + t] = z[(int64_t)t * m + (m - 1)];
+constexpr int kRitzThreads = 768;
+
+template <int CTRL, int ROW_MASK>
+__device__ __forceinline__ double dpp_max(double v) {
+  const int lo = __double2loint(v), hi = __double2hiint(v);
+  const int l2 = __builtin_amdgcn_update_dpp(lo, lo, CTRL, ROW_MASK, 0xF, false);
+  const int h2 = __builtin_amdgcn_update_dpp(hi, hi, CTRL, ROW_MASK, 0xF, false);
+  return fmax(v, __hiloint2double(h2, l2));
+}
+__device__ __forceinline__ double wave_max_all(double v) {
+  v = dpp_max<0xB1, 0xF>(v);
+  v = dpp_max<0x4E, 0xF>(v);
+  v = dpp_max<0x141, 0xF>(v);
+  v = dpp_max<0x140, 0xF>(v);
+  v = dpp_max<0x142, 0xA>(v);
+  v = dpp_max<0x143, 0xC>(v);
+  return __hiloint2double(__builtin_amdgcn_readlane(__double2hiint(v), 63), __builtin_amdgcn_readlane(__double2loint(v), 63));
+}
+__device__ __forceinline__ double wave_min_all(double v) { return -wave_max_all(-v); }
+__device__ __forceinline__ void wave_sync() {
+  __builtin_amdgcn_fence(__ATOMIC_SEQ_CST, "workgroup");
+  __builtin_amdgcn_wave_barrier();
+}
+
+size_t ritz_tridiag_lds_bytes(int m, int k, int nc, bool* par_fit) {
+  const size_t fixed = sizeof(double) * (3 * (size_t)m + (size_t)nc + (size_t)k + 40);
+  const size_t per_vec = (size_t)m * (6 * sizeof(double) + sizeof(int));
+  *par_fit = k > 1 && k <= kRitzThreads / 64 && fixed + (size_t)k * per_vec <= 60 * 1024;
+  return fixed + (*par_fit ? (size_t)k : 1) * per_vec;
+}
+
+__global__ __launch_bounds__(kRitzThreads) void ritz_tridiag_kernel(const double* __restrict__ d, const double* __restrict__ e,
+                                                                    int m, int k, int nc, int gs, int par_fit,
+                                                                    double* __restrict__ cand, double* __restrict__ sel,
+                                                                    double* __restrict__ y, const double* __restrict__ beta_src,
+                                                                    double* __restrict__ rec_beta) {
+  extern __shared__ __attribute__((aligned(16))) double ritz_lds[];
+  double* ds = ritz_lds;
+  double* es = ds + m;
+  double* e2s = es + m;
+  double* cands = e2s + m;
+  double* sels = cands + nc;
+  double* red = sels + k;
+  double* vec0 = red + 40;
+  __shared__ double red4[4 * (kRitzThreads / 64)];
+  const int tid = threadIdx.x, lane = tid & 63, wave = tid >> 6;
+  constexpr int NW = kRitzThreads / 64;
+
+  double gl = DBL_MAX, gu = -DBL_MAX, e2max = 0.0, tn = 0.0;
+  for (int i = tid; i < m; i += kRitzThreads) {
+    const double di = d[i];
+    const double el = (i > 0) ? fabs(e[i - 1]) : 0.0;
+    const double er = (i < m - 1) ? fabs(e[i]) : 0.0;
+    gl = fmin(gl, di - el - er);
+    gu = fmax(gu, di + el + er);
+    e2max = fmax(e2max, er * er);
+    tn = fmax(tn, fmax(fabs(di), er));
+    ds[i] = di;
+    es[i] = (i < m - 1) ? e[i] : 0.0;
+    e2s[i] = er * er;
+  }
+  gl = -wave_max_all(-gl);
+  gu = wave_max_all(gu);
+  e2max = wave_max_all(e2max);
+  tn = wave_max_all(tn);
+  if (lane == 0) {
+    red4[wave] = gl;
+    red4[NW + wave] = gu;
+    red4[2 * NW + wave] = e2max;
+    red4[3 * NW + wave] = tn;
+  }
+  __syncthreads();
+  for (int w2 = 0; w2 < NW; ++w2) {
+    gl = fmin(gl, red4[w2]);
+    gu = fmax(gu, red4[NW + w2]);
+    e2max = fmax(e2max, red4[2 * NW + w2]);
+    tn = fmax(tn, red4[3 * NW + w2]);
+  }
+  const double eps = DBL_EPSILON;
+  const double pivmin = DBL_MIN * fmax(1.0, e2max);
+  const double tnorm = fmax(fabs(gl), fabs(gu));
+  gl -= 2.1 * tnorm * eps * m + 2.1 * pivmin;
+  gu += 2.1 * tnorm * eps * m + 2.1 * pivmin;
+
+  const int groups = kRitzThreads / gs, g = tid / gs, t = tid - g * gs, wpg = gs >> 6;
+  const int na = min(k + 1, m);
+  for (int base = 0; base < nc; base += groups) {
+    const int c = base + g;
+    const bool active = c < nc;
+    const int want = active ? (c < na ? m - 1 - c : c - na) : 0;
+    double lo = gl, hi = gu;
+    bool done = !active;
+    for (int it = 0; it < 64; ++it) {
+      double cand_lo = lo, cand_hi = hi;
+      if (!done) {
+        const double x = lo + (hi - lo) * ((double)(t + 1) / (double)(gs + 1));
+        double qv = ds[0] - x;
+        if (fabs(qv) < pivmin) qv = -pivmin;
+        int cnt = (qv < 0.0) ? 1 : 0;
+        double dn = ds[1], en = e2s[0];
+        for (int i = 1; i < m; ++i) {
+          const double di = dn, ei = en;
+          dn = ds[i + 1];
+          en = e2s[i];
+          qv = di - x - ei / qv;
+          if (fabs(qv) < pivmin) qv = -pivmin;
+          cnt += (qv < 0.0) ? 1 : 0;
+        }
+        cand_lo = (cnt <= want) ? x : lo;
+        cand_hi = (cnt > want) ? x : hi;
+      }
+      cand_lo = wave_max_all(cand_lo);
+      cand_hi = wave_min_all(cand_hi);
+      if (lane == 0) {
+        red[wave] = cand_lo;
+        red[16 + wave] = cand_hi;
+      }
+      __syncthreads();
+      double nlo = red[g * wpg], nhi = red[16 + g * wpg];
+      for (int w2 = 1; w2 < wpg; ++w2) {
+        nlo = fmax(nlo, red[g * wpg + w2]);
+        nhi = fmin(nhi, red[16 + g * wpg + w2]);
+      }
+      if (!done) {
+        if (!(nlo > lo || nhi < hi) || !(nlo < nhi)) {
+          done = true;
+        } else {
+          lo = nlo;
+          hi = nhi;
+          if (hi - lo <= 2.0 * eps * fmax(fabs(lo), fabs(hi)) + 2.0 * pivmin) done = true;
+        }
+      }
+      if (__syncthreads_and(done ? 1 : 0)) break;
+    }
+    if (active && t == 0) cands[c] = 0.5 * (lo + hi);
+  }
+  __syncthreads();
+
+  const double ortol = 1e-3 * tn;
+  for (int c = tid; c < nc; c += kRitzThreads) {
+    const double vc = cands[c], fc = fabs(vc);
+    int rank = 0;
+    for (int o = 0; o < nc; ++o) {
+      const double vo = cands[o], fo = fabs(vo);
+      rank += (fo != fc) ? (fo > fc) : (vo != vc) ? (vo > vc) : (o < c);
+    }
+    if (rank < k) {
+      sels[rank] = vc;
+      sel[rank] = vc;
+    }
+    cand[c] = vc;
+  }
+  for (int s2 = nc + tid; s2 < k; s2 += kRitzThreads) {
+    sels[s2] = 0.0;
+    sel[s2] = 0.0;
+  }
+  __syncthreads();
+  if (tid == 0) {
+    bool clustered = false;
+    for (int a = 1; a < k; ++a)
+      for (int b = 0; b < a; ++b) clustered = clustered || fabs(sels[a] - sels[b]) <= ortol;
+    red[32] = clustered ? 1.0 : 0.0;
+  }
+  __syncthreads();
+
+  const bool parallel = par_fit && red[32] == 0.0;
+  if (wave >= (parallel ? k : 1)) return;
+  const double tiny = fmax(DBL_EPSILON * tn, DBL_MIN / DBL_EPSILON);
+  const int slot = parallel ? wave : 0;
+  double* dl = vec0 + (size_t)slot * 6 * m;
+  double* dd = dl + m;
+  double* du = dd + m;
+  double* du2 = du + m;
+  double* yv = du2 + m;
+  double* zc = yv + m;
+  int* ipiv = reinterpret_cast<int*>(vec0 + (size_t)(par_fit ? k : 1) * 6 * m) + (size_t)slot * m;
+  const int c_begin = parallel ? wave : 0, c_end = parallel ? wave + 1 : k;
+  for (int c = c_begin; c < c_end; ++c) {
+    const double lc = sels[c];
+    double* yc = y + (int64_t)c * m;
+    if (m == 1) {
+      if (lane == 0) {
+        yc[0] = 1.0;
+        if (beta_src) rec_beta[1 + c] = 1.0;
+      }
+      continue;
+    }
+    for (int i = lane; i < m; i += 64) {
+      uint32_t s = (uint32_t)(i + 1) * 2654435761u + (uint32_t)(c + 1) * 40503u;
+      s = s * 1103515245u + 12345u;
+      s ^= s >> 15;
+      s = s * 1103515245u + 12345u;
+      zc[i] = (double)(s >> 8) * (1.0 / 8388608.0) - 1.0;
+    }
+    wave_sync();
+    if (lane == 0) {
+      double ddi = ds[0] - lc, dui = es[0];
+      double dnext = ds[1], enext = es[1];
+      for (int i = 0; i < m - 1; ++i) {
+        const double dli = es[i], ddn = dnext - lc, en = enext;
+        dnext = ds[i + 2];
+        enext = es[i + 2];
+        if (fabs(ddi) >= fabs(dli)) {
+          double f = dli, nd = ddn;
+          if (ddi != 0.0) {
+            f = dli / ddi;
+            nd = ddn - f * dui;
+          }
+          dl[i] = f;
+          dd[i] = ddi;
+          du[i] = dui;
+          du2[i] = 0.0;
+          ipiv[i] = i;
+          ddi = nd;
+          dui = en;
+        } else {
+          const double f = ddi / dli;
+          dd[i] = dli;
+          dl[i] = f;
+          du[i] = ddn;
+          du2[i] = (i < m - 2) ? en : 0.0;
+          ipiv[i] = i + 1;
+          ddi = dui - f * ddn;
+          dui = -f * en;
+        }
+      }
+      dd[m - 1] = ddi;
+      du2[m - 1] = 0.0;
+      ipiv[m - 1] = m - 1;
+    }
+    wave_sync();
+    for (int i = lane; i < m; i += 64) {
+      double p = dd[i];
+      if (fabs(p) < tiny) p = (p < 0.0) ? -tiny : tiny;
+      dd[i] = 1.0 / p;
+    }
+    wave_sync();
+    for (int it = 0; it < 3; ++it) {
+      if (lane == 0) {
+        double yi = zc[0];
+        double zn = zc[1], ln = dl[0];
+        int pn = ipiv[0];
+        for (int i = 0; i < m - 1; ++i) {
+          const double znext = zn, dli = ln;
+          const bool keep = pn == i;
+          zn = zc[i + 2];
+          ln = dl[i + 1];
+          pn = ipiv[i + 1];
+          if (keep) {
+            yv[i] = yi;
+            yi = znext - dli * yi;
+          } else {
+            yv[i] = znext;
+            yi = yi - dli * znext;
+          }
+        }
+        double y1 = yi * dd[m - 1];
+        yv[m - 1] = y1;
+        double y2 = 0.0;
+        double yn = yv[m - 2], un = du[m - 2], u2n = 0.0, rn2 = dd[m - 2];
+        for (int i = m - 2; i >= 0; --i) {
+          const double yc0 = yn, ui = un, u2i = u2n, ri = rn2;
+          if (i > 0) {
+            yn = yv[i - 1];
+            un = du[i - 1];
+            u2n = du2[i - 1];
+            rn2 = dd[i - 1];
+          }
+          const double t0 = (yc0 - ui * y1 - u2i * y2) * ri;
+          yv[i] = t0;
+          y2 = y1;
+          y1 = t0;
+        }
+      }
+      wave_sync();
+      double mx = 0.0;
+      for (int i = lane; i < m; i += 64) mx = fmax(mx, fabs(yv[i]));
+      mx = wave_max_all(mx);
+      const double inv = (mx > 0.0) ? 1.0 / mx : 1.0;
+      for (int i = lane; i < m; i += 64) yv[i] *= inv;
+      wave_sync();
+      for (int p = 0; p < c; ++p) {
+        if (fabs(sels[p] - lc) <= ortol) {
+          const double* zp = y + (int64_t)p * m;
+          double dot = 0.0;
+          for (int i = lane; i < m; i += 64) dot += zp[i] * yv[i];
+          dot = __shfl(wave_sum(dot), 0, 64);
+          for (int i = lane; i < m; i += 64) yv[i] -= dot * zp[i];
+          wave_sync();
+        }
+      }
+      double nrm = 0.0;
+      for (int i = lane; i < m; i += 64) nrm += yv[i] * yv[i];
+      nrm = __shfl(wave_sum(nrm), 0, 64);
+      const double rn = (nrm > 0.0) ? 1.0 / sqrt(nrm) : 0.0;
+      for (int i = lane; i < m; i += 64) zc[i] = yv[i] * rn;
+      wave_sync();
+    }
+    for (int i = lane; i < m; i += 64) yc[i] = zc[i];
+    if (lane == 0 && beta_src) rec_beta[1 + c] = zc[m - 1];
+    wave_sync();
+  }
+  if (wave == 0 && lane == 0 && beta_src) rec_beta[0] = beta_src[m - 1];
+}
+
+inline int ritz_candidates(int m, int k) { return std::min(k + 1, m) + std::max(0, std::min(k + 1, m - 1 - k)); }
+
+hipError_t launch_ritz_tridiag(const double* d, const double* e, int m, int k, int nc, double* cand, double* sel, double* y,
+                               const double* beta_src, double* rec_beta, hipStream_t stream) {
+  bool par_fit = false;
+  const size_t lds = ritz_tridiag_lds_bytes(m, k, nc, &par_fit);
+  const int gs = nc > 6 ? 64 : nc > 3 ? 128 : 256;
+  hipLaunchKernelGGL(ritz_tridiag_kernel, dim3(1), dim3(kRitzThreads), lds, stream, d, e, m, k, nc, gs, par_fit ? 1 : 0, cand,
+                     sel, y, beta_src, rec_beta);
+  return hipGetLastError();
 }
 
 __global__ __launch_bounds__(256) void ritz_kernel(const double* __restrict__ v, int n, int m,
@@ -593,6 +959,10 @@
   return hipGetLastError();
 }
 void launch_centred_matvec(const EigWorkspace& ws, int32_t n, const double* x, double* y, hipStream_t stream) { launch_symv(ws, n, x, y, stream); }
+hipError_t ritz_tridiag(const double* d, const double* e, int32_t m, int32_t k, double* cand, double* sel, double* y, hipStream_t stream) {
+  return launch_ritz_tridiag(d, e, m, k, ritz_candidates(m, k), cand, sel, y, nullptr, nullptr, stream);
+}
+int32_t ritz_tridiag_candidates(int32_t m, int32_t k) { return ritz_candidates(m, k); }
 
 size_t lanczos_workspace_doubles(int32_t n, int32_t k, int32_t mmax) {
   const size_t nb = ((size_t)n + 255) / 256;
@@ -600,7 +970,11 @@
   const size_t pmax = 2 * ((size_t)k + 2);
   const size_t band = 2 * mcap * mcap + 12 * mcap + 2 * pmax * mcap + 4 * pmax + 32;
   return (size_t)(mmax + 1) * n + (size_t)n + (size_t)k * n + 4 * (size_t)(mmax + 2) + 4 * (size_t)k + 16 +
-         nb * (size_t)(mmax + 2) + band;
+         nb * (size_t)(mmax + 2) + band + (size_t)k * (mmax + 1);
+}
+
+size_t lanczos_fused_workspace_doubles(int32_t n, int32_t mmax) {
+  return (size_t)(mmax + 1) * n + (size_t)(mmax + 2) + ((size_t)n + 3) / 4 + 8;
 }
 
 namespace {
@@ -650,51 +1024,71 @@
   double* rec = h2 + (mmax + 2);
   double* part = rec + (4 * (size_t)k + 16);
   double* pnorm = part + (size_t)nb * (mmax + 1);
-
-  EigWorkspace small = ws;
-  small.d = alpha;
-  small.e = beta;
+  double* ybuf = pnorm + nb;
+  const bool one_kernel = ws.a || (ws.measure == PCOA_SIMILARITY_SHARED && !ws.comp_q32 && (ws.s64 || !(ws.sym_part && (n & 3) == 0)));
+  const bool fused = !mv && ws.lanczos_fused_room && one_kernel;
+  const unsigned rows4 = (unsigned)((n + 3) / 4);
+  double* h1b = ybuf + (size_t)k * (mmax + 1);
+  double* apart = h1b + (mmax + 2);
+  double* W = apart + rows4 + 8;
+  auto launch_fused_matvec = [&](int j, const double* x, const double* pn, const double* h1prev, double* h1out) {
+    const dim3 grid(rows4 + (unsigned)j), block(256);
+    double* vj = V + (size_t)j * n;
+    double* wj = W + (size_t)j * n;
+    if (ws.a)
+      hipLaunchKernelGGL(lanczos_matvec_fused_kernel<0>, grid, block, 0, stream, ws.a, ws.s32, ws.s64, n, ws.colmean, ws.stats,
+                         (int)rows4, j, x, pn, (int)nb, vj, W, wj, apart, h1prev, h2, h1out, alpha, beta);
+    else if (ws.s64)
+      hipLaunchKernelGGL(lanczos_matvec_fused_kernel<2>, grid, block, 0, stream, ws.a, ws.s32, ws.s64, n, ws.colmean, ws.stats,
+                         (int)rows4, j, x, pn, (int)nb, vj, W, wj, apart, h1prev, h2, h1out, alpha, beta);
+    else
+      hipLaunchKernelGGL(lanczos_matvec_fused_kernel<1>, grid, block, 0, stream, ws.a, ws.s32, ws.s64, n, ws.colmean, ws.stats,
+                         (int)rows4, j, x, pn, (int)nb, vj, W, wj, apart, h1prev, h2, h1out, alpha, beta);
+  };
 
   hipLaunchKernelGGL(lanczos_init_kernel, dim3(1), dim3(1024), 0, stream, V, n);
   int next_check = 12;
   if (next_check < k + 2) next_check = k + 2;
   if (next_check > mmax) next_check = mmax;
   std::vector<double> cand, pageable;
-  std::vector<int32_t> idx;
   double est_prev = 0.0;
+  bool normalised = true;
   for (int j = 0; j < mmax; ++j) {
     const double* vj = V + (size_t)j * n;
     const int cnt = j + 1;
-    {
+    const int m = j + 1;
+    const bool check = m == next_check || m == mmax;
+    if (fused) {
+      double* h1cur = (j & 1) ? h1b : h1;
+      const double* h1prev = (j & 1) ? h1 : h1b;
+      launch_fused_matvec(j, normalised ? vj : w, normalised ? nullptr : pnorm, h1prev, h1cur);
+      hipLaunchKernelGGL(cgs_update_dots_kernel<true>, dim3(nb), dim3(256), 0, stream, V, n, cnt, h1cur, W + (size_t)j * n, w, part,
+                         apart, (int)rows4);
+      hipLaunchKernelGGL(cgs_update_norm_kernel, dim3(nb), dim3(256), 0, stream, V, n, cnt, part, (int)nb, w, h2, pnorm);
+      if (check)
+        hipLaunchKernelGGL(lanczos_finish_kernel, dim3(1), dim3(1024), 0, stream, V, n, j, w, pnorm, (int)nb, h1cur, h2, alpha,
+                           beta);
+      normalised = check;
+    } else {
       const hipError_t em = matvec(vj, w);
       if (em != hipSuccess) return em;
-    }
-    hipLaunchKernelGGL(cgs_dots_kernel, dim3((unsigned)cnt), dim3(256), 0, stream, V, n, w, h1);
-    hipLaunchKernelGGL(cgs_update_dots_kernel, dim3(nb), dim3(256), 0, stream, V, n, cnt, h1, w, part);
-    hipLaunchKernelGGL(cgs_update_norm_kernel, dim3(nb), dim3(256), 0, stream, V, n, cnt, part, (int)nb, w, h2, pnorm);
-    hipLaunchKernelGGL(lanczos_finish_kernel, dim3(1), dim3(1024), 0, stream, V, n, j, w, pnorm, (int)nb, h1, h2, alpha,
-                       beta);
-    const int m = j + 1;
-    if (m != next_check && m != mmax) continue;
+      hipLaunchKernelGGL(cgs_dots_kernel, dim3((unsigned)cnt), dim3(256), 0, stream, V, n, w, h1);
+      hipLaunchKernelGGL(cgs_update_dots_kernel<false>, dim3(nb), dim3(256), 0, stream, V, n, cnt, h1, w, w, part, nullptr, 0);
+      hipLaunchKernelGGL(cgs_update_norm_kernel, dim3(nb), dim3(256), 0, stream, V, n, cnt, part, (int)nb, w, h2, pnorm);
+      hipLaunchKernelGGL(lanczos_finish_kernel, dim3(1), dim3(1024), 0, stream, V, n, j, w, pnorm, (int)nb, h1, h2, alpha,
+                         beta);
+    }
+    if (!check) continue;
     next_check = (m < 24) ? m + 4 : (m < 64) ? m + 8 : m + m / 2;
     if (next_check > mmax) next_check = mmax;
     if (steps_out) *steps_out = m;
 
-    idx.clear();
-    for (int t = 0; t <= k && t < m; ++t) idx.push_back(m - 1 - t);
-    for (int t = 0; t <= k; ++t)
-      if (t < m - 1 - k) idx.push_back(t);
-    const int nc = (int)idx.size();
+    const int nc = ritz_candidates(m, k);
     double* rec_beta = rec + nc;
     double* rec_res = rec_beta + 1 + k;
-    hipError_t e = launch_bisect(small, m, idx.data(), nc, rec, stream);
+    hipError_t e = launch_ritz_tridiag(alpha, beta, m, k, nc, rec, ws.lam, ybuf, beta, rec_beta, stream);
     if (e != hipSuccess) return e;
-    hipLaunchKernelGGL(ritz_select_kernel, dim3(1), dim3(64), 0, stream, rec, nc, k, ws.lam);
-    if ((e = launch_inverse_iteration_dev(small, m, k, stream)) != hipSuccess) return e;
-    hipLaunchKernelGGL(ritz_collect_kernel, dim3(1), dim3(64), 0, stream, beta, ws.z, m, k, rec_beta);
-    hipLaunchKernelGGL(ritz_kernel, dim3(nb, (unsigned)k), dim3(256), 0, stream, V, n, m, ws.z, bu);
-    if ((e = hipMemcpyAsync(ws.z, bu, sizeof(double) * (size_t)k * n, hipMemcpyDeviceToDevice, stream)) != hipSuccess)
-      return e;
+    hipLaunchKernelGGL(ritz_kernel, dim3(nb, (unsigned)k), dim3(256), 0, stream, V, n, m, ybuf, ws.z);
     for (int t = 0; t < k; ++t) {
       const hipError_t em = matvec(ws.z + (size_t)t * n, bu + (size_t)t * n);
       if (em != hipSuccess) return em;
@@ -825,7 +1219,7 @@
   for (int t = 1; t < bw0; ++t) {
     hipLaunchKernelGGL(lanczos_init_kernel, dim3(1), dim3(1024), 0, stream, w, n, (uint32_t)t);
     hipLaunchKernelGGL(cgs_dots_kernel, dim3((unsigned)cnt), dim3(256), 0, stream, V, n, w, h1);
-    hipLaunchKernelGGL(cgs_update_dots_kernel, dim3(nb), dim3(256), 0, stream, V, n, cnt, h1, w, part);
+    hipLaunchKernelGGL(cgs_update_dots_kernel<false>, dim3(nb), dim3(256), 0, stream, V, n, cnt, h1, w, w, part, nullptr, 0);
     hipLaunchKernelGGL(cgs_update_norm_kernel, dim3(nb), dim3(256), 0, stream, V, n, cnt, part, (int)nb, w, h2, pnorm);
     hipLaunchKernelGGL(lanczos_finish_kernel, dim3(1), dim3(1024), 0, stream, V, n, cnt - 1, w, pnorm, (int)nb, h1, h2, alpha, beta);
     cnt += 1;
@@ -833,7 +1227,6 @@
   double anorm = 0.0;
   int next_check = std::max(12, 3 * bw0);
   std::vector<double> cand;
-  std::vector<int32_t> idx;
   const int cap = mmax - pk;
   const int64_t budget = 40LL * mmax;
   int64_t columns = 0;
@@ -845,7 +1238,7 @@
     }
     columns += 1;
     hipLaunchKernelGGL(cgs_dots_kernel, dim3((unsigned)cnt), dim3(256), 0, stream, V, n, w, h1);
-    hipLaunchKernelGGL(cgs_update_dots_kernel, dim3(nb), dim3(256), 0, stream, V, n, cnt, h1, w, part);
+    hipLaunchKernelGGL(cgs_update_dots_kernel<false>, dim3(nb), dim3(256), 0, stream, V, n, cnt, h1, w, w, part, nullptr, 0);
     hipLaunchKernelGGL(cgs_update_norm_kernel, dim3(nb), dim3(256), 0, stream, V, n, cnt, part, (int)nb, w, h2, pnorm);
     const bool room = cnt < cap;
     hipLaunchKernelGGL(band_finish_kernel, dim3(1), dim3(1024), 0, stream, V, n, cnt, w, pnorm, (int)nb, h1, h2, cnt,
@@ -872,15 +1265,9 @@
     if ((e = launch_tridiagonalize(hs, J, stream)) != hipSuccess) return e;
     const int kk = std::min(k, J);
     const int pw = full ? std::min(pk, J - 1) : kk;
-    idx.clear();
-    for (int t = 0; t <= pw && t < J; ++t) idx.push_back(J - 1 - t);
-    for (int t = 0; t <= pw; ++t)
-      if (t < J - 1 - pw) idx.push_back(t);
-    const int nc = (int)idx.size();
+    const int nc = ritz_candidates(J, pw);
     double* rec_res = rec + nc;
-    if ((e = launch_bisect(hs, J, idx.data(), nc, rec, stream)) != hipSuccess) return e;
-    hipLaunchKernelGGL(ritz_select_kernel, dim3(1), dim3(64), 0, stream, rec, nc, pw, hlam);
-    if ((e = launch_inverse_iteration_dev(hs, J, pw, stream)) != hipSuccess) return e;
+    if ((e = launch_ritz_tridiag(hd, he, J, pw, nc, rec, hlam, hz, nullptr, nullptr, stream)) != hipSuccess) return e;
     if ((e = launch_backtransform(hs, J, pw, 0, 1, hout, stream)) != hipSuccess) return e;
     hipLaunchKernelGGL(ritz_kernel, dim3(nb, (unsigned)kk), dim3(256), 0, stream, V, n, J, hout, bu);
     if ((e = hipMemcpyAsync(ws.z, bu, sizeof(double) * (size_t)kk * n, hipMemcpyDeviceToDevice, stream)) != hipSuccess) return e;
diff --git a/spark-examples_amd/csrc/pcoa_capi.hip b/spark-examples_amd/csrc/pcoa_capi.hip
--- a/spark-examples_amd/csrc/pcoa_capi.hip
+++ b/spark-examples_amd/csrc/pcoa_capi.hip
@@ -275,7 +275,8 @@
     if ((rc = ensure_workspace(c, num_pc)) != PCOA_OK) return rc;
     if (c->n >= 32 && !(c->flags & PCOA_FLAG_EIG_HOUSEHOLDER)) {
       const int32_t mmax = std::min<int32_t>(c->n, 512);
-      if ((rc = ensure(c, &c->lanczos_ws, &c->lanczos_cap, (int64_t)lanczos_workspace_doubles(c->n, num_pc, mmax))) != PCOA_OK)
+      const size_t fused = c->n < 16384 ? lanczos_fused_workspace_doubles(c->n, mmax) : 0;
+      if ((rc = ensure(c, &c->lanczos_ws, &c->lanczos_cap, (int64_t)(lanczos_workspace_doubles(c->n, num_pc, mmax) + fused))) != PCOA_OK)
         return rc;
     } else if ((rc = ensure_b(c)) != PCOA_OK) {
       return rc;
diff --git a/spark-examples_amd/csrc/pcoa_internal.h b/spark-examples_amd/csrc/pcoa_internal.h
--- a/spark-examples_amd/csrc/pcoa_internal.h
+++ b/spark-examples_amd/csrc/pcoa_internal.h
@@ -259,6 +259,7 @@
   const double* colmean;
   const double* stats;
   double* sym_part = nullptr;
+  bool lanczos_fused_room = false;
   bool band_only = false;
   int measure = 0;
   const int64_t* diag = nullptr;
@@ -299,12 +300,15 @@
                          double* lam_out_dev, hipStream_t stream, int32_t* form = nullptr);
 hipError_t launch_inverse_iteration(const EigWorkspace& ws, int32_t n, const double* lam_sel_host, int32_t k,
                                     hipStream_t stream, int32_t* form = nullptr);
-hipError_t launch_inverse_iteration_dev(const EigWorkspace& ws, int32_t n, int32_t k, hipStream_t stream);
 size_t wy_workspace_doubles(int32_t n, int32_t k);
 hipError_t launch_backtransform(const EigWorkspace& ws, int32_t n, int32_t k, int sign_normalize,
                                 int apply_reflectors, double* out_dev, hipStream_t stream, int32_t* form = nullptr);
 
 size_t lanczos_workspace_doubles(int32_t n, int32_t k, int32_t mmax);
+size_t lanczos_fused_workspace_doubles(int32_t n, int32_t mmax);
+int32_t ritz_tridiag_candidates(int32_t m, int32_t k);
+hipError_t ritz_tridiag(const double* d, const double* e, int32_t m, int32_t k, double* cand, double* sel, double* y,
+                        hipStream_t stream);
 typedef std::function<int(const double*, double*)> LanczosMatvec;
 hipError_t lanczos_topk(const EigWorkspace& ws, double* lz, int32_t n, int32_t k, int32_t mmax, double tol,
                         double* lam_sel_host, int* converged, int* steps_out, hipStream_t stream,
diff --git a/spark-examples_amd/engine.py b/spark-examples_amd/engine.py
--- a/spark-examples_amd/engine.py
+++ b/spark-examples_amd/engine.py
@@ -323,6 +323,19 @@
         self._check(self._lib.pcoa_debug_centred_matvec(self._ctx, _ptr(x), _ptr(y), int(form)))
         return y
 
+    def debug_ritz_tridiag(self, d, e, k):
+        d = np.ascontiguousarray(d, dtype=np.float64)
+        e = np.ascontiguousarray(e, dtype=np.float64)
+        m = int(d.shape[0])
+        if e.shape[0] != m - 1:
+            raise ValueError("e must have len(d) - 1 entries")
+        nc = int(self._lib.pcoa_debug_ritz_candidates(m, int(k)))
+        cand = np.zeros(max(nc, 1), dtype=np.float64)
+        sel = np.zeros(int(k), dtype=np.float64)
+        y = np.zeros((int(k), m), dtype=np.float64)
+        self._check(self._lib.pcoa_debug_ritz_tridiag(self._ctx, _ptr(d), _ptr(e), m, int(k), _ptr(cand), _ptr(sel), _ptr(y)))
+        return cand[:nc], sel, y
+
     def reduce_from(self, other):
         self._check(self._lib.pcoa_gram_reduce_from(self._ctx, other._ctx))
 
```

Result: slower. 455.8 million (-2.5%).
